# ictnlp/StreamSpeech

Measured on AMD Instinct MI355X. Metric: real-time factor (RTFx = audio seconds / wall seconds) + utterances/sec, offline S2ST fr-en, higher is better.
Workload: dtype f32

## Files before the change

include/streamspeech_hip.h:

```cpp
#ifndef STREAMSPEECH_HIP_H
#define STREAMSPEECH_HIP_H

#include <stddef.h>
#include <stdint.h>

#ifdef __cplusplus
extern "C" {
#endif

#define SS_ABI_VERSION 2

typedef struct ss_model ss_model;
typedef struct ss_vocoder ss_vocoder;
typedef struct ss_scratch ss_scratch;
typedef struct ss_stream_pool ss_stream_pool;

typedef struct ss_config {
  int32_t input_feat, conv_channels, conv_kernel;
  int32_t enc_dim, enc_ffn, enc_heads, enc_layers, dw_kernel;
  int32_t src_vocab, tgt_vocab;
  int32_t mt_layers, dec_dim, dec_ffn, dec_heads;
  int32_t t2u_layers, unit_layers, unit_vocab, ctc_upsample;
  int32_t pad, eos, unk;
  int32_t max_rel_pos;
// ... 214 lines not shown
  float* powers;
  int64_t hist_first;
  int64_t n_hist;
  int64_t first_frame;
  int32_t n_frames;
  int32_t H, W;
  float p_abs, p_min, snr, rise;
  int32_t min_speech, end_silence, post_roll, max_frames;
  int32_t reserved;
} ss_vad_seg;

typedef struct ss_vad_result {
  int64_t consumed;
  int64_t start_frame;
  int64_t cut_sample;
  int64_t last_speech;
  int32_t events;
  int32_t mode;
} ss_vad_result;

int ss_vad_scan(void* stream, const ss_vad_seg* h_segs, int n_segs, ss_vad_result* d_results);
int ss_vad_scan_host(const ss_vad_seg* h_segs, int n_segs, ss_vad_result* h_results);

int ss_row_max_logprob(void* stream, const float* d_logits, int rows, int vocab, int mask0, int mask1, int mask2,
                       float* d_out);

int ss_log_softmax(void* stream, const float* d_logits, int rows, int vocab, int mask0, int mask1, int as_probs,
                   float* d_out);

int ss_encoder_out_len(int T);
int ss_encoder_forward(ss_model* m, void* stream, const float* d_fbank, int T, int attn_chunk,
                       int conv_chunk, float* d_enc_out);

int ss_encoder_stream_reset(ss_model* m);
int ss_encoder_stream_set_tail(ss_model* m, int unsettled_fbank_frames);
int ss_encoder_stream_forward(ss_model* m, void* stream, const float* d_fbank, int T, int attn_chunk,
                              int conv_chunk, float* d_enc_out, int32_t* n_final, int32_t* n_computed);
int ss_encoder_stream_set_deferred(ss_model* m, int on);
int ss_encoder_stream_status(ss_model* m, void* stream, int32_t* repeat);

int ss_stream_pool_create(ss_model* m, int max_sessions, int max_rows, ss_stream_pool** out);
void ss_stream_pool_destroy(ss_stream_pool* p);
int ss_stream_pool_reset(ss_stream_pool* p, int slot);
int ss_stream_pool_set_tail(ss_stream_pool* p, int slot, int unsettled_fbank_frames);
int ss_encoder_stream_forward_batch(ss_model* m, void* stream, ss_stream_pool* p, int n, const int32_t* h_slots,
                                    const float* const* h_fbank, const int32_t* h_T, const int32_t* h_attn_chunk,
                                    const int32_t* h_conv_chunk, float* d_enc_packed, int32_t* h_n_final, int32_t* h_n_computed);
int ss_stream_pool_ctc(ss_model* m, void* stream, ss_stream_pool* p, int head, int n, const int32_t* h_slots,
                       const float* d_enc_packed, int32_t* d_raw, int32_t* d_tokens, int32_t* d_index, int32_t* d_counts);
int ss_stream_pool_set_scores(ss_stream_pool* p, int on);
int ss_stream_pool_ctc_scored(ss_model* m, void* stream, ss_stream_pool* p, int head, int n, const int32_t* h_slots,
                              const float* d_enc_packed, int32_t* d_raw, int32_t* d_tokens, int32_t* d_index, int32_t* d_counts,
                              float* d_lprob, int32_t* d_last, float* d_tok_lprob);
int ss_stream_pool_stats(ss_stream_pool* p, int64_t* launches, int64_t* head_rows);

int ss_ctc_greedy(ss_model* m, void* stream, int head, const float* d_enc_out, int Tp,
                  int32_t* d_raw, int32_t* d_tokens, int32_t* d_index, int32_t* d_count,
                  float* d_logits);

int ss_ctc_greedy_scored(ss_model* m, void* stream, int head, const float* d_enc_out, int Tp,
                         int32_t* d_raw, int32_t* d_tokens, int32_t* d_index, int32_t* d_count,
                         float* d_logits, float* d_lprob, int32_t* d_last, float* d_tok_lprob);

int ss_mt_set_persistent(ss_model* m, int workgroups);
int ss_mt_get_persistent(ss_model* m);

int ss_mt_begin(ss_model* m, void* stream, const float* d_enc_out, int Tp);
int ss_mt_append(ss_model* m, void* stream, const int32_t* d_tokens, int n, int pos0, int ban_eos,
                 int force_eos, float* d_feats, int32_t* d_next, int n_tail_pad);
int ss_mt_greedy(ss_model* m, void* stream, const float* d_enc_out, int Tp, const int32_t* h_prefix,
                 int n_prefix, int max_len, int min_len, int32_t* h_out_tokens, int* h_n_out,
                 float* d_feats, int* h_n_feats);
int ss_mt_truncate(ss_model* m, int len);

int ss_t2u_units(ss_model* m, void* stream, const float* d_mt_feats, int n, int t2u_causal,
                 int mask_eos, int32_t* d_raw, int32_t* d_tokens, int32_t* d_count, float* d_logits,
                 int n_tail_pad);

int ss_vocoder_create(const ss_vocoder_config* cfg, const float* d_blob, size_t blob_floats,
                      const char* const* names, const int64_t* offsets, const int64_t* numels,
                      int n_slots, ss_vocoder** out);
void ss_vocoder_destroy(ss_vocoder* v);
int ss_vocoder_set_bf16x3(ss_vocoder* v, int on);
int ss_vocoder_set_f16(ss_vocoder* v, int on);
int ss_vocoder_forward(ss_vocoder* v, void* stream, const int32_t* d_codes, int K, int dur_prediction,
                       const int32_t* d_forced_dur, float* d_wav, int64_t wav_capacity,
                       int32_t* d_dur, int64_t* h_n_samples);
int ss_vocoder_num_speakers(const ss_vocoder* v);
int ss_vocoder_forward_spkr(ss_vocoder* v, void* stream, const int32_t* d_codes, int K, int dur_prediction,
                            const int32_t* d_forced_dur, float* d_wav, int64_t wav_capacity,
                            int32_t* d_dur, int64_t* h_n_samples, int32_t spkr);

int ss_batch_fbank_cmvn(ss_model* m, void* stream, int B, const float* d_pcm, const int64_t* h_pcm_start,
                        const int32_t* h_n_samples, float pcm_scale, float* d_feat, int32_t* h_T);
int ss_batch_cmvn(ss_model* m, void* stream, const float* d_in, int64_t rows, float* d_out);
int ss_batch_encoder_forward(ss_model* m, void* stream, int B, const float* d_fbank, const int32_t* h_T,
                             int attn_chunk, int conv_chunk, float* d_enc_out, int32_t* h_Tp);
int ss_batch_ctc_greedy(ss_model* m, void* stream, int head, int B, const float* d_enc_out,
                        const int32_t* h_Tp, int32_t* d_raw, int32_t* d_tokens, int32_t* d_index,
                        int32_t* d_counts);
int ss_batch_ctc_greedy_scored(ss_model* m, void* stream, int head, int B, const float* d_enc_out,
                               const int32_t* h_Tp, int32_t* d_raw, int32_t* d_tokens, int32_t* d_index,
                               int32_t* d_counts, float* d_lprob, int32_t* d_last, float* d_tok_lprob);
typedef struct ss_ctc_align_result {
  double score;
  double viterbi;
  int32_t status;
  int32_t n_tokens;
} ss_ctc_align_result;
#define SS_CTC_ALIGN_MAX_FRAMES 1500
#define SS_CTC_ALIGN_MAX_LABELS 1500
int ss_batch_ctc_align(ss_model* m, void* stream, int head, int B, const float* d_enc_out, const int32_t* h_Tp,
                       const int32_t* h_targets, const int32_t* h_n_targets, ss_ctc_align_result* d_results, int32_t* d_path,
                       int32_t* d_first, int32_t* d_last, float* d_tok_lprob);
int ss_ctc_align_host(const float* h_logits, int ld, int V, int pad, int B, const int32_t* h_T, const int32_t* h_targets,
                      const int32_t* h_n_targets, ss_ctc_align_result* h_results, int32_t* h_path, int32_t* h_first, int32_t* h_last,
                      float* h_tok_lprob, float* h_frame_lprob);
int ss_batch_mt_greedy(ss_model* m, void* stream, int B, const float* d_enc_out, const int32_t* h_Tp,
                       const int32_t* h_max_len, int min_len, int32_t* h_out_tokens, int out_stride,
                       int32_t* h_n_out, float* d_feats, int feat_rows);
int ss_batch_mt_beam(ss_model* m, void* stream, int B, int beam, const float* d_enc_out, const int32_t* h_Tp,
                     const int32_t* h_max_len, int min_len, float unk_penalty, int normalize, int32_t* h_out_tokens,
                     int out_stride, int32_t* h_n_out, float* h_scores, float* h_pos_scores, float* d_feats, int feat_rows);
int ss_batch_mt_continue(ss_model* m, void* stream, int B, const float* d_enc_out, const int32_t* h_Tp, const int32_t* h_prefix,
                         const int32_t* h_n_prefix, const int32_t* h_max_len, int min_len, int32_t* h_out_tokens, int out_stride,
                         int32_t* h_n_out, float* d_feats, int feat_rows, int32_t* h_n_feats);
int ss_batch_mt_continue_plan(int B, const int32_t* h_Tp, const int32_t* h_prefix, const int32_t* h_n_prefix, const int32_t* h_max_len,
                              int min_len, int out_stride, int feat_rows, int max_tgt_pos, int vocab, int eos, int32_t* h_dims,
                              int32_t* h_tables, int64_t tables_cap, int64_t* h_n_tables);
int ss_batch_mt_beam_continue(ss_model* m, void* stream, int B, int beam, const float* d_enc_out, const int32_t* h_Tp,
                              const int32_t* h_prefix, const int32_t* h_n_prefix, const int32_t* h_max_len, int min_len,
                              float unk_penalty, int normalize, int32_t* h_out_tokens, int out_stride, int32_t* h_n_out,
                              float* h_scores, float* h_pos_scores, float* d_feats, int feat_rows);
int ss_batch_mt_beam_continue_plan(int B, int beam, const int32_t* h_Tp, const int32_t* h_prefix, const int32_t* h_n_prefix,
                                   const int32_t* h_max_len, int min_len, int out_stride, int feat_rows, int max_tgt_pos, int vocab,
                                   int eos, int pad, int32_t* h_dims, int32_t* h_tables, int64_t tables_cap, int64_t* h_n_tables);
typedef struct ss_mt_search_opts {
  int32_t size;
  int32_t no_repeat_ngram;
  float len_penalty;
  float temperature;
} ss_mt_search_opts;
int ss_batch_mt_beam_opts(ss_model* m, void* stream, int B, int beam, const float* d_enc_out, const int32_t* h_Tp,
                          const int32_t* h_max_len, int min_len, float unk_penalty, int normalize, int32_t* h_out_tokens,
                          int out_stride, int32_t* h_n_out, float* h_scores, float* h_pos_scores, float* d_feats, int feat_rows,
                          const ss_mt_search_opts* opts);
int ss_batch_mt_beam_continue_opts(ss_model* m, void* stream, int B, int beam, const float* d_enc_out, const int32_t* h_Tp,
                                   const int32_t* h_prefix, const int32_t* h_n_prefix, const int32_t* h_max_len, int min_len,
                                   float unk_penalty, int normalize, int32_t* h_out_tokens, int out_stride, int32_t* h_n_out,
                                   float* h_scores, float* h_pos_scores, float* d_feats, int feat_rows,
                                   const ss_mt_search_opts* opts);
int ss_batch_mt_beam_continue_plan_opts(int B, int beam, const int32_t* h_Tp, const int32_t* h_prefix, const int32_t* h_n_prefix,
                                        const int32_t* h_max_len, int min_len, int out_stride, int feat_rows, int max_tgt_pos,
                                        int vocab, int eos, int pad, int32_t* h_dims, int32_t* h_tables, int64_t tables_cap,
                                        int64_t* h_n_tables, const ss_mt_search_opts* opts);
int ss_batch_fbank_frames(ss_model* m, void* stream, int B, const float* const* h_pcm, const int32_t* h_first, const int32_t* h_n,
                          float pcm_scale, float* const* h_feat);
int ss_batch_fbank_frames_sr(ss_model* m, void* stream, int B, const float* const* h_pcm, const int32_t* h_n_in, const int32_t* h_up,
                             const int32_t* h_down, const float* const* h_taps, const int32_t* h_half_len, const int32_t* h_first,
                             const int32_t* h_n, float pcm_scale, float* const* h_feat);
int ss_fbank_sr_rows(int64_t n_in, int up, int down, int half_len, int32_t* h_n_rows, int32_t* h_n_final);
int ss_batch_t2u_units(ss_model* m, void* stream, int B, const float* d_feats, int feat_rows,
                       const int32_t* h_n, int t2u_causal, int mask_eos, int32_t* d_raw, int32_t* d_tokens,
                       int32_t* d_counts);
int ss_batch_vocoder_forward(ss_vocoder* v, void* stream, int B, const int32_t* d_codes, const int32_t* h_K,
                             int dur_prediction, const int32_t* d_forced_dur, float* d_wav,
// ... 10 lines not shown
                         const int32_t* h_n_tokens, const int32_t* h_n_tail_pad, float* d_feats, int feat_rows);
int ss_batch_mt_attention(ss_model* m, void* stream, int B, const float* d_enc_out, const int32_t* h_Tp, const int32_t* h_tokens,
                          const int32_t* h_n_tokens, const int32_t* h_first, float* d_feats, int feat_rows, float* d_attn,
                          int64_t* h_attn_off, int64_t attn_capacity, int32_t* d_peak, float* d_stat);
int ss_batch_mt_score(ss_model* m, void* stream, int U, const float* d_enc_out, const int32_t* h_Tp, int B, const int32_t* h_src,
                      const int32_t* h_tokens, const int32_t* h_n_tokens, float* d_feats, int feat_rows, float* d_stat,
                      int32_t* d_idx);
int ss_batch_vocoder_tail(ss_vocoder* v, void* stream, int B, const int32_t* d_codes, const int32_t* h_K, const int32_t* h_n_new,
                          const int32_t* h_ctx, const int32_t* h_rf, int dur_prediction, float* d_out, int64_t out_capacity,
                          int32_t* h_win_first, int32_t* h_dur, int64_t* h_out_start, int64_t* h_n_out);
int ss_batch_vocoder_tail_spkr(ss_vocoder* v, void* stream, int B, const int32_t* d_codes, const int32_t* h_K, const int32_t* h_n_new,
                               const int32_t* h_ctx, const int32_t* h_rf, int dur_prediction, float* d_out, int64_t out_capacity,
                               int32_t* h_win_first, int32_t* h_dur, int64_t* h_out_start, int64_t* h_n_out,
                               const int32_t* h_spkr );

int ss_batch_unit_spans(ss_model* m, void* stream, int B, const int32_t* d_raw, const int32_t* h_n, const int32_t* h_K,
                        const int32_t* h_dur_first, const int32_t* h_unit0, const int32_t* d_dur, const int32_t* h_dur,
                        int32_t* h_spans, int32_t* h_K_out);
int ss_unit_spans_host(int B, const int32_t* h_raw, const int32_t* h_n, const int32_t* h_K, const int32_t* h_dur_first,
                       const int32_t* h_unit0, const int32_t* h_dur, int up, int blank, int pad, int bos, int eos, int32_t* h_spans,
                       int32_t* h_K_out);

int ss_prof_enable(int cls_mask);
int ss_prof_enable_hi(int cls_mask);
int ss_prof_reset(void);
int ss_prof_read(int cls, double* h_ms_total, double* h_flops_total, int64_t* h_launches,
                 double* h_bytes_total);
int ss_prof_totals(int cls, double* h_flops_total, double* h_bytes_total, int64_t* h_launches);
int ss_prof_read_issued(int cls, double* h_issued_flops_total);
int ss_prof_shape_log(int on);
int ss_prof_shape_dump(char* buf, int cap);
int ss_prof_num_classes(void);
const char* ss_prof_class_name(int cls);

int ss_model_set_pack_invariant(ss_model* m, int on);
int ss_model_get_pack_invariant(ss_model* m);
int ss_debug_canon(int mode);

int ss_debug_last_logits(ss_model* m, void* stream, float* d_out, int64_t cap_floats, int* h_rows, int* h_cols);

int ss_op_ffn_fused(void* stream, const float* dX, int ldx, float* dY, int ldy, const float* ln_g, const float* ln_b,
                    const float* dW1, const float* db1, const float* dW2, const float* db2, float alpha,
                    const float* ln2_g, const float* ln2_b, int M, int D, int F);
int ss_debug_ffn(int grid, int row_tiles_per_wave, int enable);
int ss_debug_rtlin(int grid, int enable);
int ss_debug_rtlin_kb(int uw, int order);
int ss_debug_rtlin_kb_last(int32_t out[4]);
int ss_debug_conv_c64(int enable);
int ss_debug_conv_c256_rows(int rows);
int ss_debug_conv_c32(int enable);
int ss_debug_conv_c16(int enable);
int64_t ss_debug_enc_step_launches(void);
int ss_op_ln_linear(void* stream, const float* dX, int ldx, const float* ln_g, const float* ln_b, const float* dW,
                    const float* dbias, const float* dR, int ldr, float* dC, int ldc, int M, int N, int K, int act, float alpha,
                    int glu);
int ss_op_ln_linear_ex(void* stream, const float* dX, int ldx, const float* ln_g, const float* ln_b, float* ln_out, const float* dW,
                       const float* dbias, const float* dR, int ldr, float* dC, int ldc, int M, int N, int K, int act, float alpha,
                       int glu, int canon);

int ss_debug_force_tile(int bm, int bn, int ks);
int ss_debug_sk_errors(void);
int ss_debug_attention_split(int v);
int ss_debug_attention_q16(int v);
int ss_debug_enc_step_inject_timeout(ss_model* m);
int ss_debug_scratch_audit(ss_scratch* sc, size_t* booked, size_t* held);
int ss_debug_mt_inject_timeout(ss_model* m);

int ss_op_conv_gemm(void* stream, const float* dA, int lda, const float* dW, const float* dbias,
                    const float* dR, int ldr, const float* dR2, int ldr2, float* dC, int ldc,
                    int M, int N, int Cin, int taps, int dil, int stride, int pad, int in_len,
                    int chunk, int in_act, float in_slope, int act, float alpha, float div, int glu);
typedef struct ss_op_conv_args {
  const float* A; const float* W; const float* bias; const float* R; const float* R2; float* C; float* C2;
  int32_t lda, ldc, ldr, ldr2, ldc2;
  int32_t M, N, Cin, taps, dil, stride, pad, in_len, chunk;
  int32_t in_act; float in_slope;
  int32_t act; float act_slope, alpha, div, c2_slope;
  int32_t glu;
  const int32_t* segs; int32_t nseg, max_seg_out;
  int32_t same_rows;
} ss_op_conv_args;
int ss_op_conv_gemm_ex(void* stream, const ss_op_conv_args* a);
int ss_op_conv_gemm_rows(void* stream, const ss_op_conv_args* a, int m_begin, const int32_t* seg_mb, const float* const* seg_A, int canon);
int ss_op_conv_pair(void* stream, const float* dA, int lda, const float* dW1, const float* db1, const float* dW2, const float* db2,
                    float* dC, int ldc, const float* dR2, int ldr2, float div, float* dC2, int ldc2, float c2_slope, int C, int taps,
                    int dil, int M, int in_len, float slope, const int32_t* d_segs, int nseg);
int ss_op_resblock_fused(void* stream, const float* dX, int ldx, const float* const* dW1, const float* const* dB1,
                         const float* const* dW2, const float* const* dB2, const int32_t* dil, float* dY, int ldy, const float* dR2,
                         int ldr2, float div, int C, int taps, int M, float slope, const int32_t* d_segs, int nseg);
int ss_debug_slab(int grid, long long min_rows);
int ss_op_conv_f16(void* stream, const float* dA, const float* dW, const float* dbias, const float* dR, const float* dR2,
                   float* dC, float* dC2, int M, int C, int taps, int dil, int in_act, float in_slope, int act, float div,
                   const int32_t* d_segs, int nseg);
int ss_op_layernorm(void* stream, const float* dx, int ldx, float* dy, int ldy, const float* dg,
                    const float* db, int M, int D, float eps);
int ss_op_attention(void* stream, const float* dQ, int ldq, const float* dK, int ldk, const float* dV,
                    int ldv, float* dO, int ldo, int Tq, int Tk, int H, float scale, int causal,
                    int chunk, const float* dP, int ldp, const float* du, const float* dv);
typedef struct ss_op_attn_args {
  const float* Q; const float* K; const float* V; float* O;
  int32_t ldq, ldk, ldv, ldo;
  int32_t Tq, Tk, H;
  float scale;
  int32_t causal, chunk, q0, k_mask_tail;
  const float* P; int32_t ldp;
  const float* bias_u; const float* bias_v;
  const int32_t* segs; int32_t nseg, max_q, p_tmax;
  const int32_t* seg_tail;
  int32_t no_decode_kernel;
  const int32_t* anc; int32_t anc_ld, anc_slots;
  int32_t use_split;
} ss_op_attn_args;
int ss_op_attention_ex(void* stream, const ss_op_attn_args* a);
typedef struct ss_op_attn_probs_args {
  const float* Q; const float* K;
  int32_t ldq, ldk, H;
  float scale;
  const int32_t* segs; int32_t nseg;
  const int32_t* q_first; const int32_t* row_off; const int64_t* p_off;
  float* P; int32_t* peak; float* stat;
  int32_t max_rows;
} ss_op_attn_probs_args;
int ss_op_attention_probs(void* stream, const ss_op_attn_probs_args* a);
typedef struct ss_op_pool_attn_args {
  const float* Qs; float* cache; float* O;
  int32_t ld, ldo, slot_rows;
  const float* P; int32_t ldp, p_tmax;
  const float* bias_u; const float* bias_v;
  const int32_t* sess; const int32_t* qt_pre;
  int32_t nsess, qtiles, H;
  float scale;
} ss_op_pool_attn_args;
int ss_op_attention_pool(void* stream, const ss_op_pool_attn_args* a);
int ss_debug_attention_no_mfma(int v);
int ss_op_dwconv_bn_silu(void* stream, const float* dx, int ldx, float* dy, int ldy, const float* dwt,
                         int K, const float* mean, const float* var, const float* gamma,
                         const float* beta, float eps, int T, int C, int chunk);
int ss_op_dwconv_bn_silu_ex(void* stream, const float* dx, int ldx, float* dy, int ldy, const float* dwt, int K, const float* mean,
                            const float* var, const float* gamma, const float* beta, float eps, int T, int C, int chunk,
                            const int32_t* segs, int nseg, int t_begin);
int ss_op_pool_dwconv(void* stream, const float* gs, float* cache, int slot_rows, float* y, const float* wt, int K, const float* bn_mean,
                      const float* bn_var, const float* bn_gamma, const float* bn_beta, float bn_eps, int C, const int32_t* sess,
                      int nsess, int max_n);
int ss_op_pool_gather_rows(void* stream, float* out, const float* stk, float* cache, int slot_rows, int W, const int32_t* tab,
                           const int32_t* pre, int nsess, int total);
int ss_op_pool_gather_ids(void* stream, int32_t* out, const int32_t* stk, int32_t* cache, int slot_rows, const int32_t* tab,
                          const int32_t* pre, int nsess, int total);
int ss_op_pool_stack_rows(void* stream, float* out, const float* enc, int W, const int32_t* src, const int32_t* pre, int nsess,
                          int total);

int ss_op_masked_argmax(void* stream, const float* logits, int ld, int M, int N, int mask0, int mask1, int mask2, int force,
                        int32_t* ids, const int32_t* row_max_len, int step, int force_id, const int32_t* row_min_len, int ban_id);
int ss_op_ctc_collapse(void* stream, const int32_t* raw, int T, int blank, int pad, int32_t* tokens, int32_t* index, int32_t* count,
                       const int32_t* segs, int nseg);
int ss_op_masked_argmax_lprob(void* stream, const float* logits, int ld, int M, int N, int mask0, int mask1, int mask2, int32_t* ids,
                              float* lprob);
int ss_op_ctc_collapse_spans(void* stream, const int32_t* raw, const float* lprob, int T, int blank, int pad, int32_t* tokens,
                             int32_t* index, int32_t* last, float* tok_lprob, int32_t* count, const int32_t* segs, int nseg);
int ss_op_mt_token_scores(void* stream, const float* d_logits, int ld, int rows, int V, const int32_t* d_target, float* d_stat,
                          int32_t* d_idx);
int ss_debug_mt_score_form(int force_strided);
int ss_op_ctc_align(void* stream, const float* d_logits, int ld, int V, int pad, int B, const int32_t* h_T, const int32_t* h_targets,
                    const int32_t* h_n_targets, ss_ctc_align_result* d_results, int32_t* d_path, int32_t* d_first, int32_t* d_last,
                    float* d_tok_lprob, float* d_frame_lprob);
int ss_op_unit_spans(void* stream, int B, const int32_t* d_raw, const int32_t* h_n, const int32_t* h_K, const int32_t* h_dur_first,
                     const int32_t* h_unit0, const int32_t* d_dur, int up, int blank, int pad, int bos, int eos, int32_t* d_spans,
// ... 49 lines not shown
```

streamspeech_amd/csrc/conv_c64.hip:

```cpp
#include "slab_common.hpp"

#ifndef C64_FENCE
#define C64_FENCE 1
#endif
#if C64_FENCE
#define C64_STEP_FENCE __builtin_amdgcn_sched_barrier(0)
#else
#define C64_STEP_FENCE do { } while (0)
#endif

namespace ss {

using u32x4 = __attribute__((ext_vector_type(4))) unsigned;

namespace {
constexpr int C6_C = 64;
constexpr int C6_BM_MAX = 256;
constexpr int C6_LDA = C6_C + 4;
constexpr int C6_MAXHALO = 64;
constexpr int C6_MAXSEG = 256;
[[maybe_unused]] constexpr int C6_RING = 8;
[[maybe_unused]] constexpr int C6_NUM_RECORDS = 0x7ffffff0;
[[maybe_unused]] constexpr int C6_NP = ((C6_BM_MAX + C6_MAXHALO) * (C6_C / 4) + 255) / 256;
}

template <bool LRELU, int WM>
__global__ __launch_bounds__(256, 2) void conv_c64_kernel(const GemmArgs p, const int slab_rows) {
#if __HIP_DEVICE_COMPILE__
  constexpr int C = C6_C, BM = 64 * WM, LDA = C6_LDA, NP = C6_NP;
  extern __shared__ __attribute__((aligned(16))) float smem[];
  float* sA = smem;
  int* s_blk = reinterpret_cast<int*>(smem + ((slab_rows * LDA + 3) & ~3));

  const int t = threadIdx.x, lane = t & 63;
  const int wave = __builtin_amdgcn_readfirstlane(t >> 6);
  const int r = lane & 15, g = lane >> 4;
  const int K = p.taps * C;

  SlabWalk<GemmArgs> w(p, s_blk, BM);
  __syncthreads();
  const int nblocks = w.nblocks();
  const float slope = p.in_slope;

  const __amdgpu_buffer_rsrc_t rsW = __builtin_amdgcn_make_buffer_rsrc((void*)p.W, 0, C6_NUM_RECORDS, 0x00020000);
  const int vo = (r * K + 4 * g) * 4;
  auto wload = [&](int tap, int f) -> f32x4 {
    const int so = __builtin_amdgcn_readfirstlane((((f & 3) * 16) * K + tap * C + (f >> 2) * 16) * 4);
    const u32x4 v = __builtin_amdgcn_raw_buffer_load_b128(rsW, vo, so, 0);
    return f32x4{__uint_as_float(v[0]), __uint_as_float(v[1]), __uint_as_float(v[2]), __uint_as_float(v[3])};
  };

  int blk = blockIdx.x;
  if (blk >= nblocks) return;
  f32x4 ring[C6_RING];
#pragma unroll
  for (int f = 0; f < C6_RING; ++f) ring[f] = wload(0, f);

  for (; blk < nblocks; blk += gridDim.x) {
    w.locate(blk, p.in_len);
    const int m0 = w.m0, seg_lo = w.seg_lo, seg_hi = w.seg_hi;
    const int m_hi = p.nseg > 0 ? seg_hi : min(seg_hi, p.M);
    const bool edge = (m0 - p.pad < seg_lo) || (m0 - p.pad + slab_rows > seg_hi);
    __syncthreads();
    {
      f32x4 pre[NP];
#pragma unroll
      for (int u = 0; u < NP; ++u) {
        const int rho = (t >> 4) + 16 * u;
        const int gc = min(max(m0 - p.pad + rho, seg_lo), seg_hi - 1);
        pre[u] = *reinterpret_cast<const f32x4*>(p.A + (size_t)gc * p.lda + (t & 15) * 4);
      }
      float* dst = sA + (t >> 4) * LDA + (t & 15) * 4;
#pragma unroll
      for (int u = 0; u < NP; ++u) {
        const int rho = (t >> 4) + 16 * u;
        f32x4 v = pre[u];
        if (edge) {
          const int gin = m0 - p.pad + rho;
          const bool ok = gin >= seg_lo && gin < seg_hi;
#pragma unroll
          for (int e = 0; e < 4; ++e) v[e] = ok ? v[e] : 0.f;
        }
        if (LRELU) {
#pragma unroll
          for (int e = 0; e < 4; ++e) v[e] = fmaxf(v[e], v[e] * slope);
        }
        if (rho < slab_rows) *reinterpret_cast<f32x4*>(dst + u * 16 * LDA) = v;
      }
    }
    __syncthreads();

    f32x4 acc[WM][4];
#pragma unroll
    for (int i = 0; i < WM; ++i)
#pragma unroll
      for (int j = 0; j < 4; ++j) acc[i][j] = f32x4{0.f, 0.f, 0.f, 0.f};

    const float* pa = sA + (wave * 16 * WM + r) * LDA + 4 * g;
    const int a_step = p.dil * LDA;
    f32x4 xa[WM];
#pragma unroll
    for (int i = 0; i < WM; ++i) xa[i] = *reinterpret_cast<const f32x4*>(pa + i * 16 * LDA);
#pragma unroll 1
    for (int tap = 0; tap < p.taps; ++tap) {
      const int tap_next = tap + 1 < p.taps ? tap + 1 : 0;
      const float* pa_next = tap + 1 < p.taps ? pa + a_step : pa;
#pragma unroll
      for (int cc = 0; cc < 4; ++cc) {
        f32x4 xb[WM];
#pragma unroll
        for (int i = 0; i < WM; ++i)
          xb[i] = *reinterpret_cast<const f32x4*>((cc < 3 ? pa : pa_next) + i * 16 * LDA + (cc < 3 ? (cc + 1) * 16 : 0));
        f32x4 wf[4];
#pragma unroll
        for (int j = 0; j < 4; ++j) {
          const int f = cc * 4 + j;
          wf[j] = ring[f % C6_RING];
          ring[f % C6_RING] = wload(f + C6_RING < 16 ? tap : tap_next, (f + C6_RING) & 15);
        }
#pragma unroll
        for (int e = 0; e < 4; ++e)
#pragma unroll
          for (int i = 0; i < WM; ++i)
#pragma unroll
            for (int j = 0; j < 4; ++j)
              acc[i][j] = __builtin_amdgcn_mfma_f32_16x16x4f32(wf[j][e], xa[i][e], acc[i][j], 0, 0, 0);
#pragma unroll
        for (int i = 0; i < WM; ++i) xa[i] = xb[i];
        C64_STEP_FENCE;
      }
      pa = pa_next;
    }

    int le = lane;
    asm volatile("" : "+v"(le));
    const int r_e = le & 15, g_e = le >> 4;
    f32x4 bb[4];
#pragma unroll
    for (int j = 0; j < 4; ++j) bb[j] = f32x4{0.f, 0.f, 0.f, 0.f};
    if (p.bias) {
#pragma unroll
      for (int j = 0; j < 4; ++j) bb[j] = *reinterpret_cast<const f32x4*>(p.bias + j * 16 + g_e * 4);
    }
    f32x4 y[WM * 4];
#pragma unroll
    for (int i = 0; i < WM; ++i)
#pragma unroll
      for (int j = 0; j < 4; ++j) y[i * 4 + j] = acc[i][j];
    const int mw = m0 + wave * 16 * WM + r_e;
    slab_epi_batch(p, y, bb, [&](int q, int n) -> size_t {
      return (size_t)min(mw + (n / 4) * 16, m_hi - 1) * (q == 0 ? p.ldr : p.ldr2) + (n % 4) * 16 + g_e * 4;
    });
#pragma unroll
    for (int i = 0; i < WM; ++i) {
      if (mw + i * 16 < m_hi) {
#pragma unroll
        for (int j = 0; j < 4; ++j) slab_epi_store(p, mw + i * 16, j * 16 + g_e * 4, y[i * 4 + j]);
      }
    }
  }
#endif
}

void conv_c64_debug(int enable) { if (enable >= 0) dispatch_edit([enable](Dispatch& d) { d.c64_off = enable ? 0 : 1; }); }
bool conv_c64_enabled() { return !disp().c64_off; }

bool conv_c64_eligible(const GemmArgs& a) {
  return !disp().c64_off && slab_conv_ok(a, C6_C) && a.taps >= 1 && a.dil >= 1 && (a.taps - 1) * a.dil <= C6_MAXHALO && a.pad >= 0 &&
         a.pad <= (a.taps - 1) * a.dil && a.nseg <= C6_MAXSEG && a.M >= disp().c64_min_rows && slab_rows_ok(a.M) &&
         (size_t)a.taps * C6_C * C6_C * 4 < 0x7ff00000ull;
}

static size_t c64_lds(int bm, const GemmArgs& a) { return slab_lds_bytes(bm + (a.taps - 1) * a.dil, C6_LDA, C6_MAXSEG); }
template <bool LRELU, int WM>
static int launch_c64_t(const GemmArgs& a, hipStream_t stream) {
  constexpr int BM = 64 * WM;
  const int slab_rows = BM + (a.taps - 1) * a.dil;
  const size_t lds = c64_lds(BM, a);
  SS_MAX_LDS_ONCE((&conv_c64_kernel<LRELU, WM>), 96 * 1024);
  SkWorkspace* st = nullptr;
  int rc = sk_workspace_acquire(stream, &st);
  if (rc != SS_OK) return rc;
  const int occ = lds * 2 <= 158 * 1024 ? 2 : 1;
  const int grid = slab_grid(occ, st->cus, a.M, BM, a.nseg);
  ProfRec rec{}; bool prof = false;
  rc = prof_begin(a, stream, PROF_CONV_C64, rec, prof);
  if (rc != SS_OK) return rc;
  hipLaunchKernelGGL((conv_c64_kernel<LRELU, WM>), dim3(grid), dim3(256), lds, stream, a, slab_rows);
  SS_LAUNCH_CHECK();
  return prof_end(stream, rec, prof);
}

int launch_conv_c64(const GemmArgs& a, hipStream_t stream) {
  if (!conv_c64_eligible(a)) return SS_ERR_ARG;
  const bool wm4 = 2 * c64_lds(256, a) <= 158 * 1024;
  if (a.in_act == ACT_LRELU) return wm4 ? launch_c64_t<true, 4>(a, stream) : launch_c64_t<true, 3>(a, stream);
  return wm4 ? launch_c64_t<false, 4>(a, stream) : launch_c64_t<false, 3>(a, stream);
}

}
```

streamspeech_amd/csrc/conv_sk2.hip:

```cpp
#include "gemm.hpp"

#include <cstdlib>

namespace ss {

using f32x4 = __attribute__((ext_vector_type(4))) float;
using u32x4 = __attribute__((ext_vector_type(4))) unsigned;
using f32x2 = __attribute__((ext_vector_type(2))) float;
using s16x4 = __attribute__((ext_vector_type(4))) short;
typedef __bf16 bf16x2_t __attribute__((ext_vector_type(2)));
typedef __attribute__((address_space(3))) void* lds_ptr_t;

constexpr int K2_BM = 256, K2_BK = 32;
[[maybe_unused]] constexpr int K2_SC1 = 16;
constexpr int K2_MAXG = 512;
[[maybe_unused]] constexpr int K2_WORD0 = 16;
[[maybe_unused]] constexpr unsigned K2_SPIN_LIMIT = 1u << 22;
[[maybe_unused]] constexpr int K2_NUM_RECORDS = 0x7ffffff0;
[[maybe_unused]] constexpr unsigned K2_OOB = 0x80000000u;
constexpr int k2_stage_floats(int BN) { return (K2_BM + BN) * K2_BK; }
constexpr size_t k2_lds_bytes(int BN) { return 3 * (size_t)k2_stage_floats(BN) * sizeof(float) + (2 * K2_BM + 4) * sizeof(int); }

struct Sk2Args {
  float* ws;
  unsigned* sync;
  unsigned base;
  unsigned epoch;
  int G;
  unsigned long long* dbg;
};

#define K2_WAIT_VMCNT(n) asm volatile("s_waitcnt vmcnt(" #n ")" ::: "memory")
#ifdef K2_DIAGNOSTIC_BUILD
#include "../../tools/src/conv_sk2_diag.hpp"
#else
#define K2D_SKIP_DMA(in_loop) false
#define K2D_SKIP_A_PIECE(in_loop, j) false
#define K2D_SKIP_WAIT_BARRIER 0
#define K2D_SKIP_DS_READ(in_loop) false
#define K2D_SKIP_TAIL false
#define K2D_SKIP_MFMA false
#define K2D_SKIP_HANDOFF false
#define K2D_SKIP_STORES false
#define K2D_SKIP_R_LOADS false
#define K2D_ONE_A_PIECE 0
#define K2D_TIMING 0
#define K2D_TIMING_DECL
#define K2_STAMP(slot) do { } while (0)
#define K2D_COUNT_STEPS(n) do { } while (0)
#define K2D_TIMING_FLUSH do { } while (0)
#endif
#ifndef K2_RPREF
#define K2_RPREF 1
#endif

__device__ __attribute__((noinline)) float k2_act_slow(float v, int act) {
  if (act == ACT_SILU) return v / (1.0f + expf(-v));
  if (act == ACT_TANH) return tanhf(v);
  return v;
}

__device__ __forceinline__ f32x4 k2_split_bf16(f32x4 x) {
  const bf16x2_t h01 = __builtin_convertvector((f32x2){x[0], x[1]}, bf16x2_t);
  const bf16x2_t h23 = __builtin_convertvector((f32x2){x[2], x[3]}, bf16x2_t);
  const unsigned u01 = __builtin_bit_cast(unsigned, h01), u23 = __builtin_bit_cast(unsigned, h23);
  const bf16x2_t l01 = __builtin_convertvector((f32x2){x[0] - __uint_as_float(u01 << 16), x[1] - __uint_as_float(u01 & 0xffff0000u)}, bf16x2_t);
  const bf16x2_t l23 = __builtin_convertvector((f32x2){x[2] - __uint_as_float(u23 << 16), x[3] - __uint_as_float(u23 & 0xffff0000u)}, bf16x2_t);
  return f32x4{__uint_as_float(u01), __uint_as_float(u23), __uint_as_float(__builtin_bit_cast(unsigned, l01)),
               __uint_as_float(__builtin_bit_cast(unsigned, l23))};
}
__device__ __forceinline__ s16x4 k2_half(f32x4 v, int lo) {
  const unsigned long long w = (unsigned long long)__float_as_uint(v[2 * lo]) | ((unsigned long long)__float_as_uint(v[2 * lo + 1]) << 32);
  return __builtin_bit_cast(s16x4, w);
}

template <int BN, bool LRELU, bool X3>
__global__ __launch_bounds__(256, 1) void conv_sk2_kernel(const GemmArgs p, const Sk2Args q) {
#if __HIP_DEVICE_COMPILE__
  constexpr int BM = K2_BM, BK = K2_BK, STAGE = k2_stage_floats(BN);
  constexpr int TN = 4, TM = BN == 128 ? 8 : 4;
  constexpr int NWP = BN / 32;
  constexpr int PIECES = 8 + NWP;
  constexpr int NFR = TM + TN;
  constexpr int HG = TM / 2;
  static_assert(BN == 128 || BN == 64, "tile widths");
  extern __shared__ __attribute__((aligned(16))) float smem[];
  int* s_lo = reinterpret_cast<int*>(smem + 3 * STAGE);
  int* s_hi = s_lo + BM;
  int* s_misc = s_hi + BM;

  const int t = threadIdx.x, lane = t & 63;
  const int wave = __builtin_amdgcn_readfirstlane(t >> 6);
  const int wrow = BN == 128 ? (wave >> 1) * 128 : wave * 64;
  const int wcol = BN == 128 ? (wave & 1) * 64 : 0;
  const int r = lane & 15, g = lane >> 4;
  if (t == 0) s_misc[0] = (int)(atomicAdd(q.sync, 1u) - q.base);
  __syncthreads();
  const int w = __builtin_amdgcn_readfirstlane(s_misc[0]);
  if ((unsigned)w >= (unsigned)q.G) { if (t == 0) atomicAdd(q.sync + 8, 1u); return; }
  K2D_TIMING_DECL

  const int kpt = p.Cin / BK;
  const int nk = p.taps * kpt;
  const int Ktot = p.taps * p.Cin;
  const int tiles_n = p.N / BN;
  const int tiles_m = (p.M + BM - 1) / BM;
  const long long U = (long long)tiles_m * tiles_n * nk;
  const long long u0 = (long long)w * U / q.G, u1 = (long long)(w + 1) * U / q.G;
  if (u1 <= u0) return;
  const int t_first = (int)(u0 / nk), t_last = (int)((u1 - 1) / nk);

  const float slope = p.in_slope;
  const __amdgpu_buffer_rsrc_t rsA = __builtin_amdgcn_make_buffer_rsrc(
      (void*)(reinterpret_cast<uintptr_t>(p.A) - (uintptr_t)p.pad * p.lda * sizeof(float)), 0, K2_NUM_RECORDS, 0x00020000);
  const __amdgpu_buffer_rsrc_t rsW = __builtin_amdgcn_make_buffer_rsrc((void*)p.W, 0, K2_NUM_RECORDS, 0x00020000);

  const int swz = (r >> 1) & 7;
  const int rdA0 = (wrow + r) * BK + ((g ^ swz) << 2);
  const int rdA1 = (wrow + r) * BK + (((4 + g) ^ swz) << 2);
  const int rdW0 = BM * BK + (wcol + r) * BK + ((g ^ swz) << 2);
  const int rdW1 = BM * BK + (wcol + r) * BK + (((4 + g) ^ swz) << 2);
  const int st_row = lane >> 3, st_pos = lane & 7;

  struct Part { int ka, kb, n, m0, n0, tm; };
  const int nparts = t_last - t_first + 1;
  auto part_of = [&](int ip) {
    const int tile = t_last - ip;
    const long long ut0 = (long long)tile * nk;
    Part P;
    P.ka = (int)(max(u0, ut0) - ut0);
    P.kb = (int)(min(u1, ut0 + nk) - ut0);
    P.n = P.kb - P.ka;
    P.tm = tile / tiles_n;
    P.m0 = P.tm * BM;
    P.n0 = (tile - P.tm * tiles_n) * BN;
    return P;
  };
  int a_base[8], a_len[8];
  unsigned a_off[8], w_off[NWP];
  int nci = 0, ntap = 0;
  int soffA = 0, soffW = 0, shift = 0;
  int cur_tm = -1;
  auto lds_barrier = [&]() {
    asm volatile("s_waitcnt lgkmcnt(0)" ::: "memory");
    __builtin_amdgcn_s_barrier();
  };
  auto stage_setup = [&](const Part& P) {
    lds_barrier();
    if (P.tm != cur_tm) {
      cur_tm = P.tm;
      const int m = P.m0 + t;
      int lo = 0, hi = 0;
      if (m < p.M) {
        if (p.nseg > 0) {
          int a = 0, bsz = p.nseg;
          while (bsz > 1) {
            const int half = bsz >> 1;
            if (p.segs[4 * (a + half)] <= m) a += half;
            bsz -= half;
          }
          const int sst = p.segs[4 * a], ln = p.segs[4 * a + 1];
          if (m >= sst && m < sst + ln) { lo = sst; hi = sst + ln; }
        } else {
          hi = p.in_len;
        }
      }
      s_lo[t] = lo; s_hi[t] = hi;
      lds_barrier();
    }
#pragma unroll
    for (int j = 0; j < 8; ++j) {
      const int row = wave * 64 + j * 8 + st_row;
      a_base[j] = P.m0 + row - p.pad - s_lo[row];
      a_len[j] = s_hi[row] - s_lo[row];
      a_off[j] = (unsigned)(((P.m0 + row) * p.lda + ((st_pos ^ ((row >> 1) & 7)) << 2)) * 4);
    }
#pragma unroll
    for (int j = 0; j < NWP; ++j) {
      const int nrow = wave * (BN / 4) + j * 8 + st_row;
      w_off[j] = (unsigned)(((P.n0 + nrow) * Ktot + ((st_pos ^ ((nrow >> 1) & 7)) << 2)) * 4);
    }
    nci = (P.ka / p.taps) * BK;
    ntap = P.ka - (P.ka / p.taps) * p.taps;
  };
  int shift_l = 0;
  auto step_begin = [&](bool live) {
    const int tapv = __builtin_amdgcn_readfirstlane(ntap);
    const int nciv = __builtin_amdgcn_readfirstlane(nci);
    shift = tapv * p.dil;
    shift_l = live ? shift : 0x40000000;
    soffA = (shift * p.lda + nciv) * 4;
    soffW = (tapv * p.Cin + nciv) * 4;
  };
  auto step_advance = [&](bool adv = true) {
    const int nt = ntap + (adv ? 1 : 0);
    const bool wrap = nt >= p.taps;
    ntap = wrap ? 0 : nt;
    nci += wrap ? BK : 0;
  };
  [[maybe_unused]] bool in_loop = false;
  auto issueA = [&](int stage, int j, bool live) {
    if (K2D_SKIP_DMA(in_loop) || K2D_SKIP_A_PIECE(in_loop, j)) return;
    float* sA = smem + stage * STAGE + (wave * 64) * BK;
    const bool ok = (unsigned)(a_base[j] + shift_l) < (unsigned)a_len[j];
    __builtin_amdgcn_raw_ptr_buffer_load_lds(rsA, (lds_ptr_t)(sA + j * 8 * BK), 16, ok ? a_off[j] : K2_OOB,
                                             __builtin_amdgcn_readfirstlane(soffA), 0, 0);
  };
  auto issueW = [&](int stage, int j, bool live) {
    if (K2D_SKIP_DMA(in_loop)) return;
    float* sW = smem + stage * STAGE + BM * BK + (wave * (BN / 4)) * BK;
    __builtin_amdgcn_raw_ptr_buffer_load_lds(rsW, (lds_ptr_t)(sW + j * 8 * BK), 16, live ? w_off[j] : K2_OOB,
                                             __builtin_amdgcn_readfirstlane(soffW), 0, 0);
  };
  auto issue_step = [&](int stage, bool live) {
    step_begin(live);
#pragma unroll
    for (int j = 0; j < 8; ++j) issueA(stage, j, live);
#pragma unroll
    for (int j = 0; j < NWP; ++j) issueW(stage, j, live);
    step_advance(live);
  };
  auto wait_newest_step_only = [&]() {
    if constexpr (K2D_ONE_A_PIECE != 0) { if constexpr (BN == 128) K2_WAIT_VMCNT(5); else K2_WAIT_VMCNT(3); }
    else if constexpr (BN == 128) K2_WAIT_VMCNT(12); else K2_WAIT_VMCNT(10);
  };
  int stage_ip = 0, stage_left = 0;
  auto stager_next_part = [&]() {
    const Part P = part_of(stage_ip);
    stage_setup(P);
    stage_left = P.n;
  };
  auto stager_advance = [&]() {
    if (stage_left == 0 && stage_ip + 1 < nparts) { ++stage_ip; stager_next_part(); }
  };

  int st = 0;
  stager_next_part();
  issue_step(0, true);
  --stage_left;
  stager_advance();
  issue_step(1, stage_left > 0);
  stage_left -= stage_left > 0 ? 1 : 0;
  wait_newest_step_only();
  __builtin_amdgcn_s_barrier();
  K2_STAMP(0);
  for (int ip = 0; ip < nparts; ++ip) {
    const Part cur = part_of(ip);
    const int n = cur.n, m0 = cur.m0, n0 = cur.n0;
    K2D_COUNT_STEPS(n);
    f32x4 acc[TM][TN];
#pragma unroll
    for (int i = 0; i < TM; ++i)
#pragma unroll
      for (int j = 0; j < TN; ++j) acc[i][j] = f32x4{0.f, 0.f, 0.f, 0.f};

    auto load_frag = [&](const float* S, int half, int u, f32x4 (&af)[TM], f32x4 (&bf)[TN]) {
      if (K2D_SKIP_DS_READ(in_loop)) return;
      if (u < TN) {
        bf[u] = *reinterpret_cast<const f32x4*>(S + (half ? rdW1 : rdW0) + u * 16 * BK);
        if (X3) bf[u] = k2_split_bf16(bf[u]);
      } else {
        const int i = u - TN;
        af[i] = *reinterpret_cast<const f32x4*>(S + (half ? rdA1 : rdA0) + i * 16 * BK);
        if (LRELU) {
#pragma unroll
          for (int e = 0; e < 4; ++e) af[i][e] = fmaxf(af[i][e], af[i][e] * slope);
        }
        if (X3) af[i] = k2_split_bf16(af[i]);
      }
    };
    auto mma8 = [&](const f32x4 (&af)[TM], const f32x4 (&bf)[TN], int e, int qd) {
      if (K2D_SKIP_MFMA) return;
      if (X3 && e == 3) return;
#pragma unroll
      for (int i = 2 * qd; i < 2 * qd + 2; ++i)
#pragma unroll
        for (int j = 0; j < TN; ++j) {
          if constexpr (X3)
            acc[i][j] = __builtin_amdgcn_mfma_f32_16x16x16bf16_1k(k2_half(bf[j], e == 2), k2_half(af[i], e == 1), acc[i][j], 0, 0, 0);
          else
            acc[i][j] = __builtin_amdgcn_mfma_f32_16x16x4f32(bf[j][e], af[i][e], acc[i][j], 0, 0, 0);
        }
    };

    f32x4 ax[TM], bx[TN], ay[TM], by[TN];
#pragma unroll
    for (int u = 0; u < NFR; ++u) load_frag(smem + st * STAGE, 0, u, ax, bx);
#if K2_RPREF
    constexpr int PT = BN == 128 ? 2 : TM;
    f32x4 rall[PT][TN];
    const bool want_r = p.R != nullptr && cur.kb == nk;
#endif
    in_loop = true;
    K2_STAMP(1);
    for (int i = 0; i < n; ++i) {
#if K2_RPREF
      if (i == n - 1 && want_r) {
        int lp = lane;
        asm volatile("" : "+v"(lp));
#pragma unroll
        for (int ii = 0; ii < PT; ++ii) {
          const int m = min(m0 + wrow + ii * 16 + (lp & 15), p.M - 1);
#pragma unroll
          for (int j = 0; j < TN; ++j)
            rall[ii][j] = *reinterpret_cast<const f32x4*>(p.R + (size_t)m * p.ldr + n0 + wcol + j * 16 + (lp >> 4) * 4);
        }
      }
#endif
      stager_advance();
      const float* S = smem + st * STAGE;
      const int st1 = st == 2 ? 0 : st + 1, st2 = st1 == 2 ? 0 : st1 + 1;
      const bool live = stage_left > 0;
      stage_left -= live ? 1 : 0;
      const float* S1 = smem + st1 * STAGE;
      step_begin(live);
#pragma unroll
      for (int u = 0; u < (NFR > PIECES ? NFR : PIECES); ++u) {
        if (u < NFR) load_frag(S, 1, u, ay, by);
        if (u < 8) issueA(st2, u, live); else if (u < PIECES) issueW(st2, u - 8, live);
      }
      step_advance(live);
#pragma unroll
      for (int sl = 0; sl < 4 * HG; ++sl) mma8(ax, bx, sl / HG, sl % HG);
#pragma unroll
      for (int sl = 0; sl < 2 * HG; ++sl) mma8(ay, by, sl / HG, sl % HG);
#if !K2D_SKIP_WAIT_BARRIER
      wait_newest_step_only();
      __builtin_amdgcn_s_barrier();
#endif
#pragma unroll
      for (int u = 0; u < NFR; ++u) load_frag(S1, 0, u, ax, bx);
#pragma unroll
      for (int sl = 0; sl < 2 * HG; ++sl) mma8(ay, by, 2 + sl / HG, sl % HG);
      st = st1;
    }
    in_loop = false;
    K2_STAMP(2);
    const bool has_begin = cur.ka == 0, has_end = cur.kb == nk;
    if (K2D_SKIP_TAIL && acc[0][0][0] != 12345.f) continue;

    int le = lane;
    asm volatile("" : "+v"(le));
    const int r_e = le & 15, g_e = le >> 4;
    if (!K2D_SKIP_HANDOFF && !has_end) {
      const __amdgpu_buffer_rsrc_t rsP = __builtin_amdgcn_make_buffer_rsrc((void*)(q.ws + (size_t)w * (BM * BN)), 0, BM * BN * 4, 0x00020000);
#pragma unroll
      for (int i = 0; i < TM; ++i)
#pragma unroll
        for (int j = 0; j < TN; ++j) {
          u32x4 v;
#pragma unroll
          for (int e = 0; e < 4; ++e) v[e] = __float_as_uint(acc[i][j][e]);
          __builtin_amdgcn_raw_buffer_store_b128(v, rsP, (((wave * TM + i) * TN + j) * 64 + le) * 16, 0, K2_SC1);
        }
      K2_WAIT_VMCNT(0);
      __syncthreads();
      if (t == 0) __hip_atomic_store(q.sync + K2_WORD0 + w, q.epoch, __ATOMIC_RELAXED, __HIP_MEMORY_SCOPE_AGENT);
      K2_STAMP(3);
      continue;
    }
    if (!K2D_SKIP_HANDOFF && !has_begin) {
      const long long ut0 = (long long)(t_last - ip) * nk;
      const int wf = (int)(((ut0 + 1) * q.G - 1) / U);
      if (t == 0) {
        for (int ww = wf; ww < w; ++ww) {
          unsigned spins = 0;
          while (__hip_atomic_load(q.sync + K2_WORD0 + ww, __ATOMIC_RELAXED, __HIP_MEMORY_SCOPE_AGENT) != q.epoch) {
            __builtin_amdgcn_s_sleep(8);
            if (++spins > K2_SPIN_LIMIT) { atomicAdd(q.sync + 8, 1u); break; }
          }
        }
      }
      __syncthreads();
      for (int ww = wf; ww < w; ++ww) {
        const __amdgpu_buffer_rsrc_t rsP = __builtin_amdgcn_make_buffer_rsrc((void*)(q.ws + (size_t)ww * (BM * BN)), 0, BM * BN * 4, 0x00020000);
#pragma unroll
        for (int qq = 0; qq < HG; ++qq) {
          __builtin_amdgcn_sched_barrier(0);
          u32x4 o[2][TN];
#pragma unroll
          for (int i = 0; i < 2; ++i)
#pragma unroll
            for (int j = 0; j < TN; ++j)
              o[i][j] = __builtin_amdgcn_raw_buffer_load_b128(rsP, (((wave * TM + qq * 2 + i) * TN + j) * 64 + le) * 16, 0, K2_SC1);
          __builtin_amdgcn_sched_barrier(0);
#pragma unroll
          for (int i = 0; i < 2; ++i)
#pragma unroll
            for (int j = 0; j < TN; ++j)
#pragma unroll
              for (int e = 0; e < 4; ++e) acc[qq * 2 + i][j][e] += __uint_as_float(o[i][j][e]);
        }
        __builtin_amdgcn_sched_barrier(0);
      }
    }

    K2_STAMP(3);
    if (m0 + wrow >= p.M) continue;
    f32x4 bb[TN];
#pragma unroll
    for (int j = 0; j < TN; ++j) {
      bb[j] = f32x4{0.f, 0.f, 0.f, 0.f};
      if (p.bias) bb[j] = *reinterpret_cast<const f32x4*>(p.bias + n0 + wcol + j * 16 + g_e * 4);
    }
#pragma unroll
    for (int qq = 0; qq < HG; ++qq) {
      __builtin_amdgcn_sched_barrier(0);
      f32x4 rr[2][TN], rr2[2][TN];
#pragma unroll
      for (int i = 0; i < 2; ++i) {
        const int m = min(m0 + wrow + (qq * 2 + i) * 16 + r_e, p.M - 1);
#pragma unroll
        for (int j = 0; j < TN; ++j) {
          const int nn = n0 + wcol + j * 16 + g_e * 4;
#if K2_RPREF
          if (p.R && !K2D_SKIP_R_LOADS) {
            if (qq * 2 + i < PT) rr[i][j] = rall[qq * 2 + i < PT ? qq * 2 + i : 0][j];
            else rr[i][j] = *reinterpret_cast<const f32x4*>(p.R + (size_t)m * p.ldr + nn);
          }
#else
          if (p.R && !K2D_SKIP_R_LOADS) rr[i][j] = *reinterpret_cast<const f32x4*>(p.R + (size_t)m * p.ldr + nn);
#endif
          if (p.R2 && !K2D_SKIP_R_LOADS) rr2[i][j] = *reinterpret_cast<const f32x4*>(p.R2 + (size_t)m * p.ldr2 + nn);
        }
      }
      __builtin_amdgcn_sched_barrier(0);
      f32x4 v[2][TN];
#pragma unroll
      for (int i = 0; i < 2; ++i)
#pragma unroll
        for (int j = 0; j < TN; ++j) {
          v[i][j] = acc[qq * 2 + i][j];
#pragma unroll
          for (int e = 0; e < 4; ++e) v[i][j][e] += bb[j][e];
        }
      if (p.act == ACT_LRELU) {
#pragma unroll
        for (int i = 0; i < 2; ++i)
#pragma unroll
          for (int j = 0; j < TN; ++j)
#pragma unroll
            for (int e = 0; e < 4; ++e) v[i][j][e] = v[i][j][e] > 0.f ? v[i][j][e] : v[i][j][e] * p.act_slope;
      } else if (p.act == ACT_RELU) {
#pragma unroll
        for (int i = 0; i < 2; ++i)
// ... 3 lines not shown
            for (int e = 0; e < 4; ++e) v[i][j][e] = fmaxf(v[i][j][e], 0.f);
      } else if (p.act != ACT_NONE) {
#pragma unroll
        for (int i = 0; i < 2; ++i)
#pragma unroll
          for (int j = 0; j < TN; ++j)
#pragma unroll
            for (int e = 0; e < 4; ++e) v[i][j][e] = k2_act_slow(v[i][j][e], p.act);
      }
#pragma unroll
      for (int i = 0; i < 2; ++i)
#pragma unroll
        for (int j = 0; j < TN; ++j)
#pragma unroll
          for (int e = 0; e < 4; ++e) v[i][j][e] *= p.alpha;
      if (p.R && !K2D_SKIP_R_LOADS) {
#pragma unroll
        for (int i = 0; i < 2; ++i)
#pragma unroll
          for (int j = 0; j < TN; ++j)
#pragma unroll
            for (int e = 0; e < 4; ++e) v[i][j][e] += rr[i][j][e];
      }
      if (p.R2 && !K2D_SKIP_R_LOADS) {
#pragma unroll
        for (int i = 0; i < 2; ++i)
#pragma unroll
          for (int j = 0; j < TN; ++j)
#pragma unroll
            for (int e = 0; e < 4; ++e) v[i][j][e] = rr2[i][j][e] + v[i][j][e];
      }
      if (p.div > 0.f) {
#pragma unroll
        for (int i = 0; i < 2; ++i)
#pragma unroll
          for (int j = 0; j < TN; ++j)
#pragma unroll
            for (int e = 0; e < 4; ++e) v[i][j][e] = v[i][j][e] / p.div;
      }
#pragma unroll
      for (int i = 0; i < 2; ++i) {
        const int m = m0 + wrow + (qq * 2 + i) * 16 + r_e;
        if (m >= p.M) continue;
#pragma unroll
        for (int j = 0; j < TN; ++j) {
          const int nn = n0 + wcol + j * 16 + g_e * 4;
          if (!K2D_SKIP_STORES || v[i][j][0] == 12345.f) *reinterpret_cast<f32x4*>(p.C + (size_t)m * p.ldc + nn) = v[i][j];
          if (p.C2 && !K2D_SKIP_STORES) {
            f32x4 w2;
#pragma unroll
            for (int e = 0; e < 4; ++e) w2[e] = v[i][j][e] > 0.f ? v[i][j][e] : v[i][j][e] * p.c2_slope;
            *reinterpret_cast<f32x4*>(p.C2 + (size_t)m * p.ldc2 + nn) = w2;
          }
        }
      }
    }
    __builtin_amdgcn_sched_barrier(0);
    K2_STAMP(4);
  }
  K2D_TIMING_FLUSH;
#endif
}

#if K2D_TIMING
static unsigned long long* g_k2_last_dbg = nullptr;
static int g_k2_last_G = 0;
extern "C" int ss_debug_sk2_timing(unsigned long long* h_out, int cap_wgs) {
  if (!g_k2_last_dbg || cap_wgs < g_k2_last_G) return -1;
  if (hipMemcpy(h_out, g_k2_last_dbg, (size_t)g_k2_last_G * 8 * sizeof(unsigned long long), hipMemcpyDeviceToHost) != hipSuccess) return -1;
  return g_k2_last_G;
}
#endif

bool conv_sk2_eligible(const GemmArgs& a) {
  return a.canon != CANON_SEQ && a.same_rows && a.stride == 1 && a.chunk == 0 && !a.glu && !a.ln_g && a.Cin % K2_BK == 0 && (a.lda & 3) == 0 &&
         a.N % 64 == 0 && a.M > 0 && (a.ldc & 3) == 0 && (!a.R || (a.ldr & 3) == 0) && (!a.R2 || (a.ldr2 & 3) == 0) &&
         (!a.C2 || (a.ldc2 & 3) == 0) && ((size_t)(a.M + a.pad + 256) * a.lda + a.Cin) * 4 < 0x7ff00000ull &&
         (size_t)a.N * a.taps * a.Cin * 4 < 0x7ff00000ull &&
         (a.in_act == ACT_NONE || (a.in_act == ACT_LRELU && a.in_slope > 0.f && a.in_slope < 1.f));
}

int conv_sk2_error_count() { return 0; }

template <int BN, bool LRELU, bool X3>
static int launch_sk2(const GemmArgs& a, hipStream_t stream, int g_force) {
  constexpr size_t kLds = k2_lds_bytes(BN);
  SS_MAX_LDS_ONCE((&conv_sk2_kernel<BN, LRELU, X3>), kLds);
  SkWorkspace* st = nullptr;
  int rc = sk_workspace_acquire(stream, &st);
  if (rc != SS_OK) return rc;
  int cus = st->cus > K2_MAXG ? K2_MAXG : st->cus;
  if (const int spare = disp().sk2_spare_cus; spare > 0 && spare < cus) cus -= spare;
  const long long nk = (long long)a.taps * (a.Cin / K2_BK);
  const long long U = (long long)cdiv(a.M, K2_BM) * (a.N / BN) * nk;
  long long G = g_force > 0 ? g_force : cus;
  if (G > cus) G = cus;
  if (G > U / 4) G = U / 4;
  if (G < 1) G = 1;
  Sk2Args q;
  q.ws = st->ws; q.sync = st->sync2; q.G = (int)G; q.dbg = nullptr;
#if K2D_TIMING
  if (!st->dbg) SS_HIP_CHECK(hipMalloc(&st->dbg, (size_t)K2_MAXG * 8 * sizeof(unsigned long long)));
  SS_HIP_CHECK(hipMemsetAsync(st->dbg, 0, (size_t)K2_MAXG * 8 * sizeof(unsigned long long), stream));
  q.dbg = st->dbg;
  g_k2_last_dbg = st->dbg; g_k2_last_G = (int)G;
#endif
  unsigned epoch = st->epoch2 + 1;
  if (epoch == 0) epoch = 1;
  q.base = st->base2;
  q.epoch = epoch;
  ProfRec rec{}; bool prof = false;
  rc = prof_begin(a, stream, X3 ? PROF_CONV_SK2_BF16X3 : PROF_CONV_SK2, rec, prof);
  if (rc != SS_OK) return rc;
  hipLaunchKernelGGL((conv_sk2_kernel<BN, LRELU, X3>), dim3((unsigned)G), dim3(256), kLds, stream, a, q);
  SS_LAUNCH_CHECK();
  st->base2 += (unsigned)G;
  st->epoch2 = epoch;
  return prof_end(stream, rec, prof);
}

int launch_conv_sk2(const GemmArgs& a, hipStream_t stream, int g_force) {
  if (!conv_sk2_eligible(a)) return SS_ERR_ARG;
  const bool lr = a.in_act == ACT_LRELU;
  if (a.x3) {
    if (a.N % 128 == 0) return lr ? launch_sk2<128, true, true>(a, stream, g_force) : launch_sk2<128, false, true>(a, stream, g_force);
    return lr ? launch_sk2<64, true, true>(a, stream, g_force) : launch_sk2<64, false, true>(a, stream, g_force);
  }
  if (a.N % 128 == 0) return lr ? launch_sk2<128, true, false>(a, stream, g_force) : launch_sk2<128, false, false>(a, stream, g_force);
  return lr ? launch_sk2<64, true, false>(a, stream, g_force) : launch_sk2<64, false, false>(a, stream, g_force);
}

}
```

streamspeech_amd/csrc/debug_ops.hip:

```cpp
#include "model_internal.hpp"
#include "ctc_align.hpp"

static int op_bind_wino(GemmArgs& a, void* stream) {
  static thread_local std::map<hipStream_t, DevBuf> wino_tmps;
  DevBuf& wino_tmp = wino_tmps[(hipStream_t)stream];
  const int N = a.N, Cin = a.Cin, taps = a.taps;
  if ((conv_c64w_enabled() && N == 64 && Cin == 64 && taps >= 3 && conv_c64_eligible(a)) ||
      (conv_c128w_enabled() && N == 128 && Cin == 128 && taps >= 3 && a.same_rows && !a.glu) ||
      (conv_c256w_enabled() && N == 256 && Cin == 256 && taps >= 3 && a.same_rows && !a.glu) ||
      (conv_c32w_enabled() && N == 32 && Cin == 32 && taps >= 3 && conv_c32_eligible(a))) {
    RET(wino_tmp.ensure((size_t)N * ((taps + 2) / 3) * 4 * N * sizeof(float)));
    RET(launch_wino_pack(a.W, wino_tmp.f(), N, taps, (hipStream_t)stream));
    a.Wwino = wino_tmp.f();
  }
  return SS_OK;
}

extern "C" int ss_op_conv_gemm(void* stream, const float* dA, int lda, const float* dW, const float* dbias,
                               const float* dR, int ldr, const float* dR2, int ldr2, float* dC, int ldc, int M,
                               int N, int Cin, int taps, int dil, int stride, int pad, int in_len, int chunk,
                               int in_act, float in_slope, int act, float alpha, float div, int glu) {
  GemmArgs a;
  a.A = dA; a.lda = lda; a.W = dW; a.bias = dbias; a.R = dR; a.ldr = ldr; a.R2 = dR2; a.ldr2 = ldr2; a.C = dC; a.ldc = ldc;
  a.M = M; a.N = N; a.Cin = Cin; a.taps = taps; a.dil = dil; a.stride = stride; a.pad = pad; a.in_len = in_len;
  a.chunk = chunk; a.in_act = in_act; a.in_slope = in_slope; a.act = act; a.alpha = alpha; a.div = div; a.glu = glu;
  a.same_rows = (stride == 1 && M == in_len) ? 1 : 0;
  RET(op_bind_wino(a, stream));
  return launch_conv_gemm(a, (hipStream_t)stream);
}

static void op_fill_conv(GemmArgs& a, const ss_op_conv_args* x) {
  a.A = x->A; a.W = x->W; a.bias = x->bias; a.R = x->R; a.R2 = x->R2; a.C = x->C; a.C2 = x->C2;
  a.lda = x->lda; a.ldc = x->ldc; a.ldr = x->ldr; a.ldr2 = x->ldr2; a.ldc2 = x->ldc2;
  a.M = x->M; a.N = x->N; a.Cin = x->Cin; a.taps = x->taps; a.dil = x->dil; a.stride = x->stride; a.pad = x->pad;
  a.in_len = x->in_len; a.chunk = x->chunk;
  a.in_act = x->in_act; a.in_slope = x->in_slope; a.act = x->act; a.act_slope = x->act_slope; a.alpha = x->alpha; a.div = x->div;
  a.c2_slope = x->c2_slope; a.glu = x->glu;
  a.segs = x->segs; a.nseg = x->nseg; a.max_seg_out = x->max_seg_out; a.same_rows = x->same_rows;
}
extern "C" int ss_op_conv_gemm_ex(void* stream, const ss_op_conv_args* x) {
  if (!x) return SS_ERR_ARG;
  GemmArgs a;
  op_fill_conv(a, x);
  if (a.W && a.N > 0 && a.taps > 0) RET(op_bind_wino(a, stream));
  return launch_conv_gemm(a, (hipStream_t)stream);
}
extern "C" int ss_op_conv_gemm_rows(void* stream, const ss_op_conv_args* x, int m_begin, const int32_t* seg_mb,
                                    const float* const* seg_A, int canon) {
  if (!x || canon < 0 || canon > 2) return SS_ERR_ARG;
  GemmArgs a;
  op_fill_conv(a, x);
  a.m_begin = m_begin; a.seg_mb = seg_mb; a.seg_A = seg_A; a.canon = canon;
  if (a.W && a.N > 0 && a.taps > 0) RET(op_bind_wino(a, stream));
  return launch_conv_gemm(a, (hipStream_t)stream);
}
extern "C" int ss_op_conv_pair(void* stream, const float* dA, int lda, const float* dW1, const float* db1, const float* dW2,
                               const float* db2, float* dC, int ldc, const float* dR2, int ldr2, float div, float* dC2, int ldc2,
                               float c2_slope, int Cch, int taps, int dil, int M, int in_len, float slope, const int32_t* d_segs,
                               int nseg) {
  return launch_conv_pair(dA, lda, dW1, db1, dW2, db2, dC, ldc, dR2, ldr2, div, dC2, ldc2, c2_slope, Cch, taps, dil, M, in_len, slope,
                          d_segs, nseg, (hipStream_t)stream);
}
extern "C" int ss_op_resblock_fused(void* stream, const float* dX, int ldx, const float* const* dW1, const float* const* dB1,
                                    const float* const* dW2, const float* const* dB2, const int32_t* dil, float* dY, int ldy,
                                    const float* dR2, int ldr2, float div, int Cch, int taps, int M, float slope,
                                    const int32_t* d_segs, int nseg) {
  if (!dW1 || !dB1 || !dW2 || !dB2 || !dil) return SS_ERR_ARG;
  return launch_resblock_fused(dX, ldx, dW1, dB1, dW2, dB2, dil, dY, ldy, dR2, ldr2, div, Cch, taps, M, slope, d_segs, nseg,
                               (hipStream_t)stream);
}
extern "C" int ss_debug_slab(int grid, long long min_rows) {
  if (grid < 0) return SS_ERR_ARG;
  slab_debug(grid, min_rows);
  return SS_OK;
}

extern "C" int ss_op_conv_f16(void* stream, const float* dA, const float* dW, const float* dbias, const float* dR, const float* dR2,
                              float* dC, float* dC2, int M, int Cch, int taps, int dil, int in_act, float in_slope, int act, float div,
                              const int32_t* d_segs, int nseg) {
  if (!dA || !dW || !dC || M <= 0 || taps < 1 || dil < 1 || nseg < 0 || (nseg > 0 && !d_segs)) return SS_ERR_ARG;
  if (!(Cch == 64 || Cch == 128 || Cch == 256)) return SS_ERR_ARG;
  static thread_local std::map<hipStream_t, DevBuf> f16_tmps;
  DevBuf& wh = f16_tmps[(hipStream_t)stream];
  RET(wh.ensure(f16_pack_halves(Cch, taps) * sizeof(uint16_t)));
  RET(launch_f16_pack(dW, wh.p, Cch, taps, (hipStream_t)stream));
  GemmArgs a;
  a.A = dA; a.lda = Cch; a.W = dW; a.Wf16 = wh.p; a.bias = dbias; a.R = dR; a.ldr = Cch; a.R2 = dR2; a.ldr2 = Cch;
  a.C = dC; a.ldc = Cch; a.C2 = dC2; a.ldc2 = Cch; a.c2_slope = 0.1f;
  a.M = M; a.N = Cch; a.Cin = Cch; a.taps = taps; a.dil = dil; a.stride = 1; a.pad = dil * (taps - 1) / 2; a.in_len = M;
  a.same_rows = 1; a.in_act = in_act; a.in_slope = in_slope; a.act = act; a.act_slope = 0.1f; a.div = div;
  a.segs = d_segs; a.nseg = nseg;
  return launch_conv_f16(a, (hipStream_t)stream);
}

extern "C" int ss_debug_last_logits(ss_model* m, void* stream, float* d_out, int64_t cap_floats, int* h_rows, int* h_cols) {
  if (!m || !h_rows || !h_cols) return SS_ERR_ARG;
  *h_rows = m->sc->dbg_rows; *h_cols = m->sc->dbg_cols;
  if (!d_out) return SS_OK;
  if (!m->sc->dbg_logits || cap_floats < (int64_t)m->sc->dbg_rows * m->sc->dbg_cols) return SS_ERR_CAPACITY;
  SS_HIP_CHECK(hipMemcpyAsync(d_out, m->sc->dbg_logits, (size_t)m->sc->dbg_rows * m->sc->dbg_cols * sizeof(float), hipMemcpyDeviceToDevice,
                              (hipStream_t)stream));
  return SS_OK;
}

extern "C" int ss_op_ffn_fused(void* stream, const float* dX, int ldx, float* dY, int ldy, const float* ln_g, const float* ln_b,
                               const float* dW1, const float* db1, const float* dW2, const float* db2, float alpha,
                               const float* ln2_g, const float* ln2_b, int M, int D, int F) {
  return launch_ffn_fused(dX, ldx, dY, ldy, ln_g, ln_b, dW1, db1, dW2, db2, alpha, ln2_g, ln2_b, M, D, F, (hipStream_t)stream,
                          canon_mode() == CANON_SEQ);
}
extern "C" int ss_debug_canon(int mode) {
  if (mode < 0 || mode > 2) return SS_ERR_ARG;
  canon_debug_set(mode);
  return SS_OK;
}
extern "C" int ss_op_ln_linear(void* stream, const float* dX, int ldx, const float* ln_g, const float* ln_b, const float* dW,
                               const float* dbias, const float* dR, int ldr, float* dC, int ldc, int M, int N, int K, int act,
                               float alpha, int glu) {
  GemmArgs a;
  a.A = dX; a.lda = ldx; a.W = dW; a.bias = dbias; a.R = dR; a.ldr = ldr; a.C = dC; a.ldc = ldc;
  a.M = M; a.N = N; a.Cin = K; a.in_len = M; a.act = act; a.alpha = alpha; a.glu = glu; a.same_rows = 1;
  a.ln_g = ln_g; a.ln_b = ln_b;
  return launch_conv_gemm(a, (hipStream_t)stream);
}
extern "C" int ss_op_ln_linear_ex(void* stream, const float* dX, int ldx, const float* ln_g, const float* ln_b, float* ln_out,
                                  const float* dW, const float* dbias, const float* dR, int ldr, float* dC, int ldc, int M, int N, int K,
                                  int act, float alpha, int glu, int canon) {
  if (canon < 0 || canon > 2 || (ln_g == nullptr) != (ln_b == nullptr) || (ln_out && !ln_g)) return SS_ERR_ARG;
  GemmArgs a;
  a.A = dX; a.lda = ldx; a.W = dW; a.bias = dbias; a.R = dR; a.ldr = ldr; a.C = dC; a.ldc = ldc;
  a.M = M; a.N = N; a.Cin = K; a.in_len = M; a.act = act; a.alpha = alpha; a.glu = glu; a.same_rows = 1;
  a.ln_g = ln_g; a.ln_b = ln_b; a.ln_out = ln_out; a.canon = canon;
  return launch_conv_gemm(a, (hipStream_t)stream);
}
extern "C" int ss_debug_conv_c64(int enable) {
  if (enable == 4 || enable == 5) { conv_c64w_debug(enable == 5); return SS_OK; }
  if (enable == 6 || enable == 7) { conv_c128w_debug(enable == 7); return SS_OK; }
  if (enable == 8 || enable == 9) { conv_c256w_debug(enable == 9); return SS_OK; }
// ... 238 lines not shown
```

streamspeech_amd/csrc/dispatch.hip:

```cpp
#include "gemm.hpp"

#include <atomic>
#include <cstdlib>
#include <map>
#include <mutex>
#include <utility>
#include <vector>

namespace ss {

namespace {
std::mutex g_disp_mu;
std::atomic<unsigned> g_disp_gen{1};
Dispatch env_defaults() {
  Dispatch d;
  auto I = [](const char* k, int dflt) { const char* e = getenv(k); return e ? atoi(e) : dflt; };
  auto L = [](const char* k, long long dflt) { const char* e = getenv(k); return e ? atoll(e) : dflt; };
  d.attn_split = I("SS_ATTN_NO_SPLIT", 0) ? -1 : 0; d.attn_q16 = I("SS_ATTN_Q16", d.attn_q16);
  d.c16_off = I("SS_NO_CONV_C16", 0) ? 1 : 0; d.c32_off = I("SS_NO_CONV_C32", 0) ? 1 : 0; d.c64_off = I("SS_NO_CONV_C64", 0) ? 1 : 0;
  d.c16_min_rows = L("SS_CONV_C16_MIN_ROWS", d.c16_min_rows); d.c32_min_rows = L("SS_CONV_C32_MIN_ROWS", d.c32_min_rows);
  d.c64_min_rows = L("SS_CONV_C64_MIN_ROWS", d.c64_min_rows);
  d.c64w_on = I("SS_CONV_C64_WINOGRAD", 1); d.c128w_on = I("SS_CONV_C128_WINOGRAD", 1); d.c256w_on = I("SS_CONV_C256_WINOGRAD", 1);
  d.c32w_on = I("SS_CONV_C32_WINOGRAD", 1); d.c64w_min_k = I("SS_CONV_C64_WINOGRAD_MIN_K", 3);
  d.c128w_min_rows = L("SS_CONV_C128_MIN_ROWS", d.c128w_min_rows); d.c256w_min_rows = L("SS_CONV_C256_MIN_ROWS", d.c256w_min_rows);
  if (const int r = I("SS_CONV_C256_ROWS", d.c256w_rows); r == 128 || r == 256) d.c256w_rows = r;
  if (getenv("SS_FFN_WM")) { d.ffn_wm = I("SS_FFN_WM", 3); d.ffn_wm_forced = 1; d.ffn_wm_env = d.ffn_wm; }
  d.ffn_fusion = I("SS_NO_FFN_FUSION", 0) ? 0 : 1; d.ffn_min_rows = I("SS_FFN_MIN_ROWS", d.ffn_min_rows);
  if (getenv("SS_SK_MIN_GFLOP")) d.sk_min_flops = 1e9 * atof(getenv("SS_SK_MIN_GFLOP"));
  d.no_resblock_fusion = I("SS_NO_RESBLOCK_FUSION", 0); d.no_pair_fusion = I("SS_NO_PAIR_FUSION", 0);
  d.rt_off = I("SS_NO_RTLIN", 0) ? 1 : 0; d.rt_min_rows = I("SS_RTLIN_MIN_ROWS", d.rt_min_rows); d.rt_min_units = L("SS_RTLIN_MIN_UNITS", d.rt_min_units);
  d.rt_kb_min_units = L("SS_RTLIN_KB_MIN_UNITS", d.rt_kb_min_units); d.rt_kb_uw = I("SS_RTLIN_KB_UW", d.rt_kb_uw); d.rt_kb_xmap = I("SS_RTLIN_KB_XMAP", d.rt_kb_xmap);
  d.smallm_max_rows = I("SS_SMALLM_MAX_ROWS", d.smallm_max_rows); d.sk_min_units = L("SS_SK_MIN_UNITS", d.sk_min_units);
  d.no_sk2 = I("SS_NO_SK2", 0) ? 1 : 0; d.sk2_min_k64 = I("SS_SK2_MINK64", d.sk2_min_k64); d.sk2_spare_cus = I("SS_SK2_SPARE_CUS", 0);
  d.rt_wg_per_cu = I("SS_RTLIN_WG_PER_CU", 0); d.c32_min_k = I("SS_CONV_C32_MIN_K", d.c32_min_k); d.c16_min_k = I("SS_CONV_C16_MIN_K", d.c16_min_k);
  return d;
}
Dispatch& process_settings() { static Dispatch d = env_defaults(); return d; }
thread_local const Dispatch* t_disp = nullptr;
thread_local CtxDispatch t_disp_own;
}
void dispatch_edit(const std::function<void(Dispatch&)>& fn) {
  std::lock_guard<std::mutex> lk(g_disp_mu);
  fn(process_settings());
  g_disp_gen.fetch_add(1, std::memory_order_release);
}
void slab_debug(int grid, long long min_rows) {
  const Dispatch dflt = env_defaults();
  dispatch_edit([=](Dispatch& d) {
    d.slab_grid_cap = grid > 0 ? grid : 0;
    const bool set = min_rows >= 0;
    d.c16_min_rows = set ? min_rows : dflt.c16_min_rows; d.c32_min_rows = set ? min_rows : dflt.c32_min_rows;
    d.c64_min_rows = set ? min_rows : dflt.c64_min_rows;
    d.c128w_min_rows = set ? min_rows : dflt.c128w_min_rows; d.c256w_min_rows = set ? min_rows : dflt.c256w_min_rows;
  });
}
int conv_c256w_rows_debug(int rows) {
  if (rows != 0 && rows != 128 && rows != 256) return SS_ERR_ARG;
  const int dflt = env_defaults().c256w_rows;
  dispatch_edit([=](Dispatch& d) { d.c256w_rows = rows ? rows : dflt; });
  return SS_OK;
}
const Dispatch* CtxDispatch::refresh() {
  const unsigned now = g_disp_gen.load(std::memory_order_acquire);
  if (gen != now) {
    std::lock_guard<std::mutex> lk(g_disp_mu);
    d = process_settings();
    gen = g_disp_gen.load(std::memory_order_relaxed);
  }
  return &d;
}
const Dispatch& disp() { return t_disp ? *t_disp : *t_disp_own.refresh(); }
DispatchScope::DispatchScope(const Dispatch* d) : prev(t_disp) { t_disp = d; }
DispatchScope::~DispatchScope() { t_disp = prev; }

void debug_force_tile(int bm, int bn, int ks) {
  dispatch_edit([=](Dispatch& d) { d.force_bm = bm; d.force_bn = bn; d.force_ks = ks; d.sk_groups = (bm == 1 && bn == 8); });
}
bool debug_tile_forced() { return disp().force_bm != 0; }

static thread_local int t_canon = CANON_NONE;
CanonScope::CanonScope(int mode) : prev(t_canon) { t_canon = mode; }
CanonScope::~CanonScope() { t_canon = prev; }
int canon_mode() { return t_canon; }
void canon_debug_set(int mode) { t_canon = mode; }

constexpr size_t SKW_SYNC_BYTES = (16 + 1024) * sizeof(unsigned) + 256;
static std::mutex g_skw_mu;
static std::vector<SkWorkspace*> g_skw_live;
static std::map<std::pair<int, hipStream_t>, SkWorkspace*> g_skw_fallback;
static thread_local SkWorkspace* t_skw = nullptr;

SkWorkspace* sk_workspace_new() {
  SkWorkspace* w = new SkWorkspace();
  std::lock_guard<std::mutex> lk(g_skw_mu);
  g_skw_live.push_back(w);
  return w;
}
void sk_workspace_free(SkWorkspace* w) {
  if (!w) return;
  {
    std::lock_guard<std::mutex> lk(g_skw_mu);
    for (size_t i = 0; i < g_skw_live.size(); ++i)
      if (g_skw_live[i] == w) { g_skw_live.erase(g_skw_live.begin() + i); break; }
  }
  if (w->ws) (void)hipFree(w->ws);
  if (w->sync1) (void)hipFree(w->sync1);
  if (w->sync2) (void)hipFree(w->sync2);
  if (w->sync3) (void)hipFree(w->sync3);
  if (w->dbg) (void)hipFree(w->dbg);
  delete w;
}
SkScope::SkScope(SkWorkspace* w) : prev(t_skw), prev_disp(t_disp) { t_skw = w; t_disp = w ? w->disp.refresh() : nullptr; }
SkScope::~SkScope() { t_skw = prev; t_disp = prev_disp; }

int sk_workspace_acquire(hipStream_t stream, SkWorkspace** out) {
  *out = nullptr;
// ... 59 lines not shown
```

streamspeech_amd/csrc/dispatch.hpp:

```cpp
#pragma once
#include <functional>

namespace ss {

struct Dispatch {
  int attn_no_mfma = 0;
  int attn_q16 = 1;
  int attn_split = 0;
  int c16_off = 0, c32_off = 0, c64_off = 0;
  long long c16_min_rows = 131072, c32_min_rows = 65536, c64_min_rows = 32768;
  int c64w_on = 1, c128w_on = 1, c256w_on = 1, c32w_on = 1;
  int c64w_min_k = 3;
  long long c128w_min_rows = 65536, c256w_min_rows = 32768;
  int c256w_rows = 128;
  int c32_min_k = 7, c16_min_k = 11;
  int slab_grid_cap = 0;
  int sk_groups = 0;
  int sk2_spare_cus = 0;
  int ffn_force_g = 0;
  int ffn_wm = 3, ffn_wm_forced = 0;
  int ffn_wm_env = 0;
  int ffn_fusion = 1;
  int ffn_min_rows = 1000;
  int force_bm = 0, force_bn = 0, force_ks = 0;
  double sk_min_flops = 4e9;
  int smallm_max_rows = 192;
  long long sk_min_units = 12 * 512;
  int no_sk2 = 0;
  int sk2_min_k64 = 192;
  int no_resblock_fusion = 0, no_pair_fusion = 0;
  int rt_off = 0, rt_min_rows = 193, rt_force_g = 0;
  long long rt_min_units = 4000;
  int rt_wg_per_cu = 0;
  long long rt_kb_min_units = 256;
  int rt_kb_xmap = 1;
  int rt_kb_uw = 0;
  int rt_kb_order = 1;
};

const Dispatch& disp();
void dispatch_edit(const std::function<void(Dispatch&)>& fn);

struct CtxDispatch {
  Dispatch d;
  unsigned gen = 0xffffffffu;
  const Dispatch* refresh();
};
struct DispatchScope {
  explicit DispatchScope(const Dispatch* d);
  ~DispatchScope();
  const Dispatch* prev;
};

}
```

streamspeech_amd/csrc/gemm.hpp:

```cpp
#pragma once
#include "common.hpp"
#include "dispatch.hpp"
#include "prof.hpp"

namespace ss {

struct GemmArgs {
  const float* A = nullptr;
  const float* W = nullptr;
  const float* Wwino = nullptr;
  const void* Wf16 = nullptr;
  const float* bias = nullptr;
  const float* R = nullptr;
  const float* R2 = nullptr;
  float* C = nullptr;
  int lda = 0, ldc = 0, ldr = 0, ldr2 = 0;
  int M = 0, N = 0, Cin = 0;
  int taps = 1, dil = 1, stride = 1, pad = 0;
  int in_len = 0;
  int chunk = 0;
  int m_begin = 0;
  int in_act = ACT_NONE;
  float in_slope = 0.1f;
  int act = ACT_NONE;
  float alpha = 1.0f;
  float div = 0.0f;
  float act_slope = 0.1f;
  float* C2 = nullptr;
  int ldc2 = 0;
  float c2_slope = 0.1f;
  int glu = 0;
  const int* segs = nullptr;
  int nseg = 0;
  int max_seg_out = 0;
  const int* seg_mb = nullptr;
  const float* const* seg_A = nullptr;
  double algo_flops = 0.0;
  double algo_bytes = 0.0;
  const float* ln_g = nullptr;
  const float* ln_b = nullptr;
  float* ln_out = nullptr;
  int same_rows = 0;
  int x3 = 0;
  int canon = 0;
};
constexpr int CANON_NONE = 0, CANON_SEQ = 1, CANON_SMALLM = 2;
constexpr int CANON_KBLOCK = 64;
struct CanonScope {
  explicit CanonScope(int mode);
  ~CanonScope();
  int prev;
};
int canon_mode();
void canon_debug_set(int mode);

struct SkWorkspace {
  int dev = -1, cus = 0;
  float* ws = nullptr;
  unsigned* sync1 = nullptr;
  unsigned* sync2 = nullptr;
  unsigned* sync3 = nullptr;
  unsigned base1[8] = {0, 0, 0, 0, 0, 0, 0, 0}, epoch1 = 0;
  unsigned base2 = 0, epoch2 = 0;
  unsigned long long* dbg = nullptr;
  CtxDispatch disp;
};
SkWorkspace* sk_workspace_new();
void sk_workspace_free(SkWorkspace* w);
struct SkScope {
  explicit SkScope(SkWorkspace* w);
  ~SkScope();
  SkWorkspace* prev;
  const Dispatch* prev_disp;
};
int sk_workspace_acquire(hipStream_t stream, SkWorkspace** out);
int sk_workspace_error_count();

bool conv_sk_eligible(const GemmArgs& a);
int launch_conv_sk(const GemmArgs& a, hipStream_t stream, int g_force = 0);
int conv_sk_error_count();
void conv_sk_set_groups(int on);

bool conv_sk2_eligible(const GemmArgs& a);
int launch_conv_sk2(const GemmArgs& a, hipStream_t stream, int g_force = 0);
int conv_sk2_error_count();

inline bool slab_rows_ok(long long rows) { return rows > 0 && rows < (1ll << 30); }

inline size_t slab_lds_bytes(int slab_rows, int lda, int maxseg) {
  return (size_t)((slab_rows * lda + 3) & ~3) * sizeof(float) + (maxseg + 2) * sizeof(int);
}
inline long long slab_max_blocks(int M, int bm, int nseg) { return (long long)cdiv(M, bm) + (nseg > 0 ? nseg : 1); }
inline int slab_grid(int occ, int cus, int M, int bm, int nseg) {
  const long long g = std::min<long long>((long long)occ * cus, std::max<long long>(1, slab_max_blocks(M, bm, nseg)));
  const int cap = disp().slab_grid_cap;
  return (int)(cap > 0 ? std::min<long long>(g, cap) : g);
}
void slab_debug(int grid, long long min_rows);
bool slab_layout_ok(const GemmArgs& a);
bool slab_conv_ok(const GemmArgs& a, int c);
int device_cus(int& cus);

bool conv_slab_eligible(const GemmArgs& a);
int launch_conv_slab(const GemmArgs& a, hipStream_t stream);

bool conv_pair_eligible(int C, int taps, int dil, int lda, int ldc, int nseg, long long M);
int launch_conv_pair(const float* A, int lda, const float* W1, const float* b1, const float* W2, const float* b2, float* C,
                     int ldc, const float* R2, int ldr2, float div, float* C2, int ldc2, float c2_slope, int Cch, int taps,
                     int dil, int M, int in_len, float slope, const int* segs, int nseg, hipStream_t stream);

bool resblock_fused_eligible(int C, int taps, const int* dil, int ldx, int ldy, int nseg, long long M);
int launch_resblock_fused(const float* X, int ldx, const float* const* W1, const float* const* B1, const float* const* W2,
                          const float* const* B2, const int* dil, float* Y, int ldy, const float* R2, int ldr2, float div, int C,
                          int taps, int M, float slope, const int* segs, int nseg, hipStream_t stream);

bool conv_c64_eligible(const GemmArgs& a);
bool conv_c64_enabled();
int launch_conv_c64(const GemmArgs& a, hipStream_t stream);
bool conv_c64w_eligible(const GemmArgs& a);
int launch_conv_c64w(const GemmArgs& a, hipStream_t stream);
int launch_wino_pack(const float* W, float* WW, int C, int taps, hipStream_t stream);
void conv_c64w_debug(int enable);
bool conv_c64w_enabled();
bool conv_wide_winograd_eligible(const GemmArgs& a, int ch);
int launch_conv_c128w(const GemmArgs& a, hipStream_t stream);
void conv_c128w_debug(int enable);
bool conv_c128w_enabled();
int launch_conv_c256w(const GemmArgs& a, hipStream_t stream);
void conv_c256w_debug(int enable);
int conv_c256w_rows_debug(int rows);
bool conv_c256w_enabled();
bool conv_c32w_eligible(const GemmArgs& a);
int launch_conv_c32w(const GemmArgs& a, hipStream_t stream);
void conv_c32w_debug(int enable);
bool conv_c32w_enabled();
void conv_c64_debug(int enable);

bool conv_c32_eligible(const GemmArgs& a);
bool conv_c32_enabled();
int launch_conv_c32(const GemmArgs& a, hipStream_t stream);
void conv_c32_debug(int enable);

bool conv_c16_eligible(const GemmArgs& a);
bool conv_c16_enabled();
int launch_conv_c16(const GemmArgs& a, hipStream_t stream);
void conv_c16_debug(int enable);

bool conv_f16_eligible(const GemmArgs& a);
bool conv_f16_geometry_ok(int C, int taps, int dil);
int launch_conv_f16(const GemmArgs& a, hipStream_t stream);
size_t f16_pack_halves(int C, int taps);
int launch_f16_pack(const float* W, void* Wf, int C, int taps, hipStream_t stream);

bool rtlin_eligible(const GemmArgs& a);
bool rtlin_shape_ok(const GemmArgs& a);
int launch_rtlin(const GemmArgs& a, hipStream_t stream);
void rtlin_debug(int grid, int enable);
bool rtlin_kb_shape_ok(const GemmArgs& a);
bool rtlin_kb_eligible(const GemmArgs& a);
int launch_rtlin_kb(const GemmArgs& a, hipStream_t stream);
void rtlin_kb_debug(int uw, int order);
void rtlin_kb_last(int out[4]);

bool ffn_fused_eligible(int D, int F, int act, int M, int ldx, int ldy, bool canon = false);
int launch_ffn_fused(const float* X, int ldx, float* Y, int ldy, const float* ln_g, const float* ln_b, const float* W1,
                     const float* b1, const float* W2, const float* b2, float alpha, const float* ln2_g, const float* ln2_b,
                     int M, int D, int F, hipStream_t stream, int canon = 0);
void ffn_fused_debug_grid(int g);
void ffn_fused_debug_rows(int wm);

bool gemv_eligible(const GemmArgs& a);
bool smallm_eligible(const GemmArgs& a);

void debug_force_tile(int bm, int bn, int ks);
bool debug_tile_forced();

int launch_conv_gemm(const GemmArgs& a, hipStream_t stream);

}
```

streamspeech_amd/csrc/model_internal.hpp:

```cpp
#pragma once
#include <algorithm>
#include <atomic>
#include <map>
#include <mutex>
#include <string>
#include <tuple>
#include <unordered_map>
#include <vector>

#include "../../include/streamspeech_hip.h"
#include "attention.hpp"
#include "attn_probs.hpp"
#include "common.hpp"
#include "elementwise.hpp"
#include "fbank.hpp"
#include "gemm.hpp"
#include "mt_step.hpp"
#include "enc_step.hpp"

using namespace ss;

namespace {

struct Slot { const float* p = nullptr; int64_t n = 0; };
// ... 314 lines not shown
}

[[maybe_unused]] static void subsampler_args(const ss_model* m, const float* fbank, float* h1, float* out, GemmArgs& a, GemmArgs& b) {
  const ss_config& c = m->cfg;
  const int k = c.conv_kernel, C1 = c.conv_channels / 2;
  a.A = fbank; a.lda = c.input_feat; a.W = m->sub0.w; a.bias = m->sub0.b; a.C = h1; a.ldc = C1;
  a.N = c.conv_channels; a.Cin = c.input_feat; a.taps = k; a.stride = 2; a.pad = k / 2; a.glu = 1;
  b.A = h1; b.lda = C1; b.W = m->sub1.w; b.bias = m->sub1.b; b.C = out; b.ldc = c.enc_dim;
  b.N = 2 * c.enc_dim; b.Cin = C1; b.taps = k; b.stride = 2; b.pad = k / 2; b.glu = 1;
}

[[maybe_unused]] static int enc_ffn_half(hipStream_t s, const ss_config& c, float* x, int n, const LN& ln, const Lin& w1, const Lin& w2,
                                         const LN* fin, bool fused, bool canon, float* h, float* ff) {
  const int d = c.enc_dim, f = c.enc_ffn;
  if (fused)
    return launch_ffn_fused(x, d, x, d, ln.g, ln.b, w1.w, w1.b, w2.w, w2.b, 0.5f, fin ? fin->g : nullptr, fin ? fin->b : nullptr,
                            n, d, f, s, canon);
  RET(ln_linear(s, x, n, ln, w1, f, d, ff, f, h, ACT_SILU));
  RET(linear(s, ff, f, n, w2, d, f, x, d, ACT_NONE, 0.5f, x, d));
  return fin ? layernorm(s, x, x, *fin, n, d) : SS_OK;
}

template <typename Attention, typename DwConv>
static int enc_layer_ex(hipStream_t s, const ss_config& c, const EncLayer& e, float* x, int n, float* h, float* ff, float* qkv_rows,
                        float* glu_rows, const float* dw_rows, bool ffn_fused, bool canon, Attention&& attention, DwConv&& dwconv) {
  const int d = c.enc_dim;
  RET(enc_ffn_half(s, c, x, n, e.ffn1_ln, e.ffn1_w1, e.ffn1_w2, nullptr, ffn_fused, canon, h, ff));
  RET(ln_linear(s, x, n, e.attn_ln, e.qkv, 3 * d, d, qkv_rows, 3 * d, h));
  RET(attention());
  RET(linear(s, h, d, n, e.out, d, d, x, d, ACT_NONE, 1.f, x, d));
  RET(ln_linear(s, x, n, e.conv_ln, e.pw1, 2 * d, d, glu_rows, d, h, ACT_NONE, 1.f, 1));
  RET(dwconv());
  RET(linear(s, dw_rows, d, n, e.pw2, d, d, x, d, ACT_NONE, 1.f, x, d));
  return enc_ffn_half(s, c, x, n, e.ffn2_ln, e.ffn2_w1, e.ffn2_w2, &e.final_ln, ffn_fused, canon, h, ff);
}

int mt_prefix_pass(ss_model* m, hipStream_t s, int B, int Np, int np_max, int n_enc, const int* d_ptok, const int* d_ppos,
                   const int* d_pself, const int* d_pcross, const int* d_ptail, const int* d_pcache, int cache_rows, const float** out);

int mt_cross_kv(ss_model* m, hipStream_t s, const float* d_enc_out, int n_rows);

struct MtRowsWs {
  float *x, *h, *q2, *ff, *logits;
  static size_t floats(int rows, int D, int F, int V, size_t gap = 0) { return (size_t)rows * (3 * D + F + V) + gap; }
  MtRowsWs(float* base, int rows, int D, int F, size_t gap = 0)
      : x(base), h(x + (size_t)rows * D), q2(h + (size_t)rows * D), ff(q2 + (size_t)rows * D), logits(ff + (size_t)rows * F + gap) {}
};

struct MtRowsStep {
  int rows = 0;
  int cache_ld = 0, ci = 0;
  const int* tok = nullptr;
  const int* row_pos = nullptr;
  int row_pad = -1;
  const int* self_segs = nullptr;
  const int* cross_segs = nullptr;
  int n_enc = 0;
  const int* anc = nullptr; int anc_ld = 0, anc_slots = 0;
  float* states = nullptr; int states_ld = 0;
};
int mt_decode_rows(ss_model* m, hipStream_t s, const MtRowsWs& w, const MtRowsStep& a);

extern std::atomic<int> g_mt_timeouts;

struct ConvW { const float* w = nullptr; const float* b = nullptr; const float* ww = nullptr;
               const void* wh = nullptr; };
struct ss_vocoder {
  ss_vocoder_config cfg;
  WeightTable wt;
  ss_scratch* sc = nullptr;
  const float* dict = nullptr;
  ConvW dur_c1, dur_c2, dur_proj, pre, post;
  LN dur_ln1, dur_ln2;
  std::vector<ConvW> ups;
  std::vector<ConvW> rb_c1, rb_c2;
  float* wino = nullptr;
  const float* wino_key = nullptr;
  int x3 = 0;
  int f16 = 0;
  const float* blob = nullptr;
  void* f16w = nullptr;
  const float* spk_table = nullptr;
  int n_spk = 0;
};

namespace {

[[maybe_unused]] int upload(hipStream_t s, int* dst, const std::vector<int>& v) {
  SS_HIP_CHECK(hipMemcpyAsync(dst, v.data(), v.size() * sizeof(int), hipMemcpyHostToDevice, s));
  return SS_OK;
}

struct Offsets { std::vector<int> off; int total = 0, mx = 0; };
[[maybe_unused]] Offsets prefix(const int* len, int B) {
  Offsets o; o.off.resize(B + 1); o.off[0] = 0;
  for (int b = 0; b < B; ++b) { o.off[b + 1] = o.off[b] + len[b]; o.mx = std::max(o.mx, len[b]); }
  o.total = o.off[B];
  return o;
}

}
```

streamspeech_amd/csrc/vocoder.hip:

```cpp
#include "model_internal.hpp"

#include <cstdint>
#include <tuple>


namespace {
struct WinoShared { DevBuf buf; size_t floats = 0; int refs = 0; };
struct WinoKey {
  int dev; const float* blob; uint64_t sig;
  bool operator<(const WinoKey& o) const { return std::tie(dev, blob, sig) < std::tie(o.dev, o.blob, o.sig); }
};
std::mutex g_wino_mu;
std::map<WinoKey, WinoShared> g_wino;
inline uint64_t fnv(uint64_t h, uint64_t v) { for (int i = 0; i < 8; ++i) { h ^= (v >> (8 * i)) & 0xff; h *= 1099511628211ull; } return h; }
uint64_t blob_sig(const ss_vocoder* v, const float* d_blob) {
  const ss_vocoder_config* cfg = &v->cfg;
  uint64_t sig = fnv(fnv(fnv(14695981039346656037ull, (uint64_t)cfg->upsample_initial_channel), (uint64_t)cfg->n_up), (uint64_t)cfg->n_res);
  for (int j = 0; j < cfg->n_res; ++j) sig = fnv(sig, (uint64_t)cfg->resblock_kernel_sizes[j]);
  for (size_t i = 0; i < v->rb_c1.size(); ++i) sig = fnv(fnv(sig, (uint64_t)(v->rb_c1[i].w - d_blob)), (uint64_t)(v->rb_c2[i].w - d_blob));
  return sig;
}
std::mutex g_f16_mu;
std::map<WinoKey, WinoShared> g_f16;
bool f16_stage(int ch) { return ch == 64 || ch == 128 || ch == 256; }
// ... 23 lines not shown
  for (int i = 0; i < cfg->n_up; ++i) {
    const int Co = C / 2, st = cfg->upsample_rates[i];
    v->ups.push_back({w.get("voc.up" + std::to_string(i) + ".w", (int64_t)st * Co * 3 * C),
                      w.get("voc.up" + std::to_string(i) + ".b", (int64_t)st * Co)});
    for (int j = 0; j < cfg->n_res; ++j) {
      const int kr = cfg->resblock_kernel_sizes[j];
      for (int dd = 0; dd < 3; ++dd) {
        const std::string p = "voc.rb" + std::to_string(i * cfg->n_res + j);
        v->rb_c1.push_back({w.get(p + ".c1." + std::to_string(dd) + ".w", (int64_t)Co * kr * Co),
                            w.get(p + ".c1." + std::to_string(dd) + ".b", Co)});
        v->rb_c2.push_back({w.get(p + ".c2." + std::to_string(dd) + ".w", (int64_t)Co * kr * Co),
                            w.get(p + ".c2." + std::to_string(dd) + ".b", Co)});
      }
    }
    C = Co;
  }
  v->post = {w.get("voc.post.w", (int64_t)7 * C), w.get("voc.post.b", 1)};
  {
    auto it = w.map.find("voc.spkr.table");
    if (it != w.map.end()) {
      const int64_t per = (int64_t)16 * C0;
      if (it->second.n <= 0 || it->second.n % per || it->second.n / per > INT32_MAX || (C0 & 3)) { scratch_unref(v->sc); delete v; return SS_ERR_ARG; }
      v->spk_table = it->second.p;
      v->n_spk = (int)(it->second.n / per);
    }
  }
  if (!w.missing.empty()) { scratch_unref(v->sc); delete v; return SS_ERR_MISSING_WEIGHT; }
  {
    auto wino_stage = [](int ch) { return ch == 32 || ch == 64 || ch == 128 || ch == 256; };
    size_t need = 0;
    int Cs = C0;
    for (int i = 0; i < cfg->n_up; ++i) {
      Cs /= 2;
      if (wino_stage(Cs)) for (int j = 0; j < cfg->n_res; ++j) need += 6 * (size_t)Cs * ((cfg->resblock_kernel_sizes[j] + 2) / 3) * 4 * Cs;
    }
    if (need) {
      int dev = 0;
      if (hipGetDevice(&dev) != hipSuccess) { scratch_unref(v->sc); delete v; return SS_ERR_HIP; }
      std::lock_guard<std::mutex> lk(g_wino_mu);
      const WinoKey key{dev, d_blob, blob_sig(v, d_blob)};
      WinoShared& sh = g_wino[key];
      const bool fresh = sh.refs == 0;
      if (!fresh && sh.floats != need) { scratch_unref(v->sc); delete v; return SS_ERR_ARG; }
      if (fresh) {
        rc = sh.buf.ensure(need * sizeof(float));
        if (rc != SS_OK) { g_wino.erase(key); scratch_unref(v->sc); delete v; return rc; }
        sh.floats = need;
      }
      float* dst = sh.buf.f();
      Cs = C0;
      for (int i = 0; i < cfg->n_up && rc == SS_OK; ++i) {
        Cs /= 2;
        if (!wino_stage(Cs)) continue;
        for (int j = 0; j < cfg->n_res && rc == SS_OK; ++j) {
          const int kr = cfg->resblock_kernel_sizes[j];
          const size_t n = (size_t)Cs * ((kr + 2) / 3) * 4 * Cs;
          for (int dd = 0; dd < 3 && rc == SS_OK; ++dd) {
            const int idx = (i * cfg->n_res + j) * 3 + dd;
            if (fresh) rc = launch_wino_pack(v->rb_c1[idx].w, dst, Cs, kr, nullptr);
            v->rb_c1[idx].ww = dst; dst += n;
            if (fresh && rc == SS_OK) rc = launch_wino_pack(v->rb_c2[idx].w, dst, Cs, kr, nullptr);
            v->rb_c2[idx].ww = dst; dst += n;
          }
        }
      }
      if (fresh && rc == SS_OK && hipDeviceSynchronize() != hipSuccess) rc = SS_ERR_HIP;
      if (rc != SS_OK) {
        if (fresh) { sh.buf.release(); g_wino.erase(key); }
        scratch_unref(v->sc); delete v; return rc;
      }
      ++sh.refs;
      v->wino = sh.buf.f(); v->wino_key = d_blob;
    }
  }
  *out = v;
  return SS_OK;
}

extern "C" int ss_vocoder_num_speakers(const ss_vocoder* v) { return v ? v->n_spk : 0; }

extern "C" int ss_vocoder_set_bf16x3(ss_vocoder* v, int on) {
  if (!v) return SS_ERR_ARG;
  v->x3 = on ? 1 : 0;
  return SS_OK;
}

static int f16_take(ss_vocoder* v) {
  const ss_vocoder_config& c = v->cfg;
  size_t need = 0;
  for (int i = 0, Cs = c.upsample_initial_channel; i < c.n_up; ++i) {
    Cs /= 2;
    if (f16_stage(Cs)) for (int j = 0; j < c.n_res; ++j) need += 6 * f16_pack_halves(Cs, c.resblock_kernel_sizes[j]);
  }
  if (!need) return SS_OK;
  for (int i = 0, Cs = c.upsample_initial_channel; i < c.n_up; ++i) {
    Cs /= 2;
    if (!f16_stage(Cs)) continue;
    for (int j = 0; j < c.n_res; ++j)
      for (int dd = 0; dd < 3; ++dd)
        if (!conv_f16_geometry_ok(Cs, c.resblock_kernel_sizes[j], c.resblock_dilations[j][dd]) ||
            !conv_f16_geometry_ok(Cs, c.resblock_kernel_sizes[j], 1))
          return SS_ERR_ARG;
  }
  int dev = 0;
  if (hipGetDevice(&dev) != hipSuccess) return SS_ERR_HIP;
  std::lock_guard<std::mutex> lk(g_f16_mu);
  const WinoKey key{dev, v->blob, blob_sig(v, v->blob)};
  WinoShared& sh = g_f16[key];
  const bool fresh = sh.refs == 0;
  if (!fresh && sh.floats != need) return SS_ERR_ARG;
  int rc = SS_OK;
  if (fresh) {
    rc = sh.buf.ensure(need * sizeof(uint16_t));
    if (rc != SS_OK) { g_f16.erase(key); return rc; }
    sh.floats = need;
  }
  char* dst = static_cast<char*>(sh.buf.p);
  std::vector<ConvW> rb1 = v->rb_c1, rb2 = v->rb_c2;
  for (int i = 0, Cs = c.upsample_initial_channel; i < c.n_up && rc == SS_OK; ++i) {
    Cs /= 2;
    if (!f16_stage(Cs)) continue;
    for (int j = 0; j < c.n_res && rc == SS_OK; ++j) {
      const int kr = c.resblock_kernel_sizes[j];
      const size_t n = f16_pack_halves(Cs, kr) * sizeof(uint16_t);
      for (int dd = 0; dd < 3 && rc == SS_OK; ++dd) {
        const int idx = (i * c.n_res + j) * 3 + dd;
        if (fresh) rc = launch_f16_pack(rb1[idx].w, dst, Cs, kr, nullptr);
        rb1[idx].wh = dst; dst += n;
        if (fresh && rc == SS_OK) rc = launch_f16_pack(rb2[idx].w, dst, Cs, kr, nullptr);
        rb2[idx].wh = dst; dst += n;
      }
    }
  }
  if (fresh && rc == SS_OK && hipDeviceSynchronize() != hipSuccess) rc = SS_ERR_HIP;
  if (rc != SS_OK) {
    if (fresh) { sh.buf.release(); g_f16.erase(key); }
    return rc;
  }
  ++sh.refs;
  v->rb_c1.swap(rb1); v->rb_c2.swap(rb2);
  v->f16w = sh.buf.p;
  return SS_OK;
}

extern "C" int ss_vocoder_set_f16(ss_vocoder* v, int on) {
  if (!v) return SS_ERR_ARG;
  if (on && !v->f16w) RET(f16_take(v));
  v->f16 = on ? 1 : 0;
  return SS_OK;
}

extern "C" void ss_vocoder_destroy(ss_vocoder* v) {
  if (!v) return;
  if (v->f16w) {
    std::lock_guard<std::mutex> lk(g_f16_mu);
    for (auto it = g_f16.begin(); it != g_f16.end(); ++it)
      if (it->first.blob == v->blob && it->second.buf.p == v->f16w) {
        if (--it->second.refs == 0) { it->second.buf.release(); g_f16.erase(it); }
        break;
      }
  }
  if (v->wino_key) {
    std::lock_guard<std::mutex> lk(g_wino_mu);
    for (auto it = g_wino.begin(); it != g_wino.end(); ++it)
      if (it->first.blob == v->wino_key && it->second.buf.f() == v->wino) {
        if (--it->second.refs == 0) { it->second.buf.release(); g_wino.erase(it); }
// ... 11 lines not shown
    scratch_unref(v->sc);
    v->sc = sc;
  }
  return SS_OK;
}

struct GenBufs { float *bx, *bt, *br, *bs, *bxa, *bra, *bsa, *br2; };
struct SpkSel { const int* seg = nullptr; int one = 0; int max_frames = 0; };

template <class ConvFn, class StageFn, class GeomFn>
static int hifigan_stack(const ss_vocoder* v, hipStream_t s, ConvFn&& conv, StageFn&& on_stage, GeomFn&& geom,
                         const float* frames, int Ft, const GenBufs& b, int* out_scale, int* out_C, const SpkSel* spk = nullptr) {
  const ss_vocoder_config& c = v->cfg;
  const bool f16 = v->f16 && v->f16w;
  const bool x3 = v->x3 && !f16;
  auto slab_stage = [&](int channels) {
    if (x3 || !(channels == 64 ? conv_c64_enabled() : channels == 32 ? conv_c32_enabled() : channels == 16 ? conv_c16_enabled() : false)) return false;
    long long rows = Ft; int ch = c.upsample_initial_channel; bool found = false;
    for (int i = 0; i < c.n_up && !found; ++i) { rows *= c.upsample_rates[i]; ch /= 2; found = ch == channels; }
    if (!found || rows >= (1ll << 30)) return false;
    GemmArgs probe;
    probe.same_rows = 1; probe.Cin = probe.N = probe.lda = probe.ldc = channels; probe.taps = 3; probe.dil = 1; probe.pad = 1;
    probe.M = probe.in_len = (int)rows; probe.in_act = ACT_LRELU;
    return channels == 64 ? conv_c64_eligible(probe) : channels == 32 ? conv_c32_eligible(probe) : conv_c16_eligible(probe);
  };
  const bool c64 = slab_stage(64), c32 = slab_stage(32), c16 = slab_stage(16);
  auto wino_slab_stage = [&](int channels) {
    if (f16 || x3 || !(channels == 128 ? conv_c128w_enabled() : conv_c256w_enabled())) return false;
    long long rows = Ft; int ch = c.upsample_initial_channel, stage = -1;
    for (int i = 0; i < c.n_up && stage < 0; ++i) { rows *= c.upsample_rates[i]; ch /= 2; if (ch == channels) stage = i; }
    if (stage < 0 || rows >= (1ll << 30)) return false;
    int sc = 1, gM = 0, gnseg = 0; const int* gsegs = nullptr;
    for (int i = 0; i <= stage; ++i) sc *= c.upsample_rates[i];
    geom(sc, gM, gsegs, gnseg);
    for (int j = 0; j < c.n_res; ++j)
      for (int dd = 0; dd < 3; ++dd)
        for (int which = 0; which < 2; ++which) {
          const int idx = (stage * c.n_res + j) * 3 + dd;
          GemmArgs probe;
          probe.same_rows = 1; probe.Cin = probe.N = probe.lda = probe.ldc = probe.ldr = probe.ldr2 = probe.ldc2 = channels;
          probe.taps = c.resblock_kernel_sizes[j]; probe.dil = which ? 1 : c.resblock_dilations[j][dd];
          probe.pad = probe.dil * (probe.taps - 1) / 2; probe.M = probe.in_len = gM; probe.nseg = gnseg; probe.in_act = ACT_LRELU;
          probe.Wwino = which ? v->rb_c2[idx].ww : v->rb_c1[idx].ww;
          if (!conv_wide_winograd_eligible(probe, channels)) return false;
        }
    return true;
  };
  const bool c128 = wino_slab_stage(128), c256 = wino_slab_stage(256);
  auto preact = [c64, c128, c256, f16](int channels) {
    return channels >= 64 && !(c64 && channels == 64) && !(c128 && channels == 128) && !(c256 && channels == 256) && !(f16 && f16_stage(channels));
  };
  auto up_preact = [c64](int channels) { return channels >= 64 && !(c64 && channels == 64); };
  auto mk = [x3, f16](const float* A, int Cin, const ConvW& cw, int Cout, int k, int dil, float* Cc, int ldc) {
    GemmArgs a;
    a.A = A; a.lda = Cin; a.W = cw.w; a.Wwino = cw.ww; a.bias = cw.b; a.C = Cc; a.ldc = ldc; a.ldr = ldc; a.ldr2 = ldc; a.ldc2 = ldc;
    a.N = Cout; a.Cin = Cin; a.taps = k; a.dil = dil; a.stride = 1; a.pad = dil * (k - 1) / 2; a.same_rows = 1;
    a.x3 = x3;
    if (f16) a.Wf16 = cw.wh;
    return a;
  };
  int scale = 1, C = c.upsample_initial_channel;
  RET(on_stage(scale));
  {
    GemmArgs a = mk(frames, c.model_in_dim, v->pre, C, 7, 1, b.bx, C);
    if (up_preact(C) && !spk) a.C2 = b.bxa;
    if (f16) a.canon = CANON_SEQ;
    RET(conv(a, scale));
    if (spk) {
      int gM = 0, gnseg = 0; const int* gsegs = nullptr;
      geom(scale, gM, gsegs, gnseg);
      const bool pa0 = up_preact(C);
      RET(launch_spkr_pre_add(b.bx, pa0 ? b.bxa : b.bx, C, C, v->spk_table, spk->seg, spk->one, gsegs, gnseg, spk->max_frames, gM, pa0 ? 1 : 0,
                              0.1f, s));
    }
  }
  for (int i = 0; i < c.n_up; ++i) {
    const int st = c.upsample_rates[i], Co = C / 2;
    const bool pa_in = up_preact(C), pa = preact(Co);
    {
      GemmArgs a = mk(pa_in ? b.bxa : b.bx, C, v->ups[i], st * Co, 3, 1, b.bs, st * Co);
      if (!pa_in) { a.in_act = ACT_LRELU; a.in_slope = 0.1f; }
      if (pa) a.C2 = b.bsa;
      a.algo_flops = 2.0 * Ft * scale * C * Co * c.upsample_kernel_sizes[i];
      if (f16 && Co >= 64) a.canon = CANON_SEQ;
      RET(conv(a, scale));
    }
    scale *= st; C = Co;
    RET(on_stage(scale));
    const bool pa_next = (i + 1 < c.n_up) && up_preact(C);
    for (int j = 0; j < c.n_res; ++j) {
      const int kr = c.resblock_kernel_sizes[j];
      int gM = 0, gnseg = 0; const int* gsegs = nullptr;
      geom(scale, gM, gsegs, gnseg);
      const bool per_conv = (c32 && C == 32 && kr >= disp().c32_min_k) || (c16 && C == 16 && kr >= disp().c16_min_k);
      if (!pa && !per_conv && !disp().no_resblock_fusion && resblock_fused_eligible(C, kr, c.resblock_dilations[j], C, C, gnseg, gM)) {
        const float *W1[3], *B1[3], *W2[3], *B2[3];
        for (int dd = 0; dd < 3; ++dd) {
          const int idx = (i * c.n_res + j) * 3 + dd;
          W1[dd] = v->rb_c1[idx].w; B1[dd] = v->rb_c1[idx].b; W2[dd] = v->rb_c2[idx].w; B2[dd] = v->rb_c2[idx].b;
        }
        RET(launch_resblock_fused(b.bs, C, W1, B1, W2, B2, c.resblock_dilations[j], b.bx, C, j > 0 ? b.bx : nullptr, C,
                                  j == c.n_res - 1 ? (float)c.n_res : 0.f, C, kr, gM, 0.1f, gsegs, gnseg, s));
        continue;
      }
      const bool fuse = !pa && !per_conv && !disp().no_pair_fusion && kr == 3 &&
                        conv_pair_eligible(C, kr, c.resblock_dilations[j][2], C, C, gnseg, gM);
      const float* cur = b.bs;
      for (int dd = 0; dd < 3; ++dd) {
        const int idx = (i * c.n_res + j) * 3 + dd;
        if (fuse) {
          float* out = dd == 0 ? b.br : dd == 1 ? b.br2 : b.bx;
          const float* R2 = (dd == 2 && j > 0) ? b.bx : nullptr;
          const float div = (dd == 2 && j == c.n_res - 1) ? (float)c.n_res : 0.f;
          RET(launch_conv_pair(cur, C, v->rb_c1[idx].w, v->rb_c1[idx].b, v->rb_c2[idx].w, v->rb_c2[idx].b, out, C, R2, C, div,
                               nullptr, C, 0.1f, C, kr, c.resblock_dilations[j][dd], gM, gM, 0.1f, gsegs, gnseg, s));
          cur = out;
          continue;
        }
        const float* rin = dd == 0 ? b.bs : b.br;
        const float* rin_act = dd == 0 ? b.bsa : b.bra;
        GemmArgs a1 = mk(pa ? rin_act : rin, C, v->rb_c1[idx], C, kr, c.resblock_dilations[j][dd], b.bt, C);
        if (pa) { a1.act = ACT_LRELU; a1.act_slope = 0.1f; }
        else { a1.in_act = ACT_LRELU; a1.in_slope = 0.1f; }
        RET(conv(a1, scale));
        GemmArgs a2 = mk(b.bt, C, v->rb_c2[idx], C, kr, 1, dd < 2 ? b.br : b.bx, C);
        if (!pa) { a2.in_act = ACT_LRELU; a2.in_slope = 0.1f; }
        a2.R = rin;
        if (dd < 2) {
          if (pa) a2.C2 = b.bra;
        } else {
          a2.R2 = j == 0 ? nullptr : b.bx;
          a2.div = (j == c.n_res - 1) ? (float)c.n_res : 0.f;
          if (pa_next && j == c.n_res - 1) a2.C2 = b.bxa;
        }
        RET(conv(a2, scale));
      }
    }
  }
  *out_scale = scale; *out_C = C;
  return SS_OK;
}

static int conv1d(hipStream_t s, const float* A, int T, int Cin, const ConvW& cw, int Cout, int k, int dil,
                  float* C, int in_act, float slope, int act, const float* R, const float* R2, float div) {
  GemmArgs a;
  a.A = A; a.lda = Cin; a.W = cw.w; a.bias = cw.b; a.C = C; a.ldc = Cout; a.R = R; a.ldr = Cout; a.R2 = R2; a.ldr2 = Cout;
  a.M = T; a.N = Cout; a.Cin = Cin; a.taps = k; a.dil = dil; a.stride = 1; a.pad = dil * (k - 1) / 2; a.in_len = T;
  a.in_act = in_act; a.in_slope = slope; a.act = act; a.div = div; a.same_rows = 1;
  return launch_conv_gemm(a, s);
}

static bool spkr_args_ok(const ss_vocoder* v, bool have, const int32_t* h_spkr, int B) {
  if (!have) return v->n_spk == 0;
  if (v->n_spk == 0 || !h_spkr) return false;
  for (int b = 0; b < B; ++b)
    if (h_spkr[b] < 0 || h_spkr[b] >= v->n_spk) return false;
  return true;
}

static int vocoder_forward(ss_vocoder* v, void* stream, const int32_t* d_codes, int K, int dur_prediction,
                           const int32_t* d_forced_dur, float* d_wav, int64_t wav_capacity,
                           int32_t* d_dur, int64_t* h_n_samples, const int32_t* h_spkr) {
  if (!v || K <= 0 || !d_codes || !d_wav || !d_dur) return SS_ERR_ARG;
  if (!spkr_args_ok(v, h_spkr != nullptr, h_spkr, 1)) return SS_ERR_ARG;
  SkScope sk_scope(v->sc->skws);
  hipStream_t s = (hipStream_t)stream;
// ... 402 lines not shown
```

streamspeech_amd/engine.py:

```python
import ctypes as C
import os
from typing import List, NamedTuple, Optional, Tuple

import numpy as np
import torch

from . import lib as L
from .config import ModelConfig, VocoderConfig
from .weights import pack_model, pack_vocoder


def _ptr(t: Optional[torch.Tensor]):
    return None if t is None else C.c_void_p(t.data_ptr())


def _stream():
    return C.c_void_p(torch.cuda.current_stream().cuda_stream)


def _require_gpu(device):
    if not torch.cuda.is_available():
        raise L.StreamSpeechHipError(
            "streamspeech_amd needs an AMD GPU (torch.cuda.is_available() is False); "
            "there is no CPU fallback for the product path")
    return torch.device(device)


def _slots(names, offsets, numels):
    n = len(names)
    c_names = (C.c_char_p * n)(*[s.encode() for s in names])
    c_off = (C.c_int64 * n)(*offsets)
    c_num = (C.c_int64 * n)(*numels)
    return c_names, c_off, c_num, n


def _i32(vals):
    return (C.c_int32 * len(vals))(*[int(v) for v in vals])


def _unpack_scored(host, T: List[int], return_raw: bool = False):
    tot, fl = sum(T), host.view(np.float32)
    out, off = [], 0
    for b, t in enumerate(T):
        n = int(host[6 * tot + b])
        rec = (host[tot + off: tot + off + n].tolist(), host[2 * tot + off: 2 * tot + off + n].tolist(),
               host[3 * tot + off: 3 * tot + off + n].tolist(), fl[5 * tot + off: 5 * tot + off + n].copy(),
               fl[4 * tot + off: 4 * tot + off + t].copy())
        out.append(rec + (host[off: off + t].tolist(),) if return_raw else rec)
        off += t
    return out


class CtcAlignment(NamedTuple):
    score: float
    viterbi_score: float
    status: int
    path: Optional[List[int]]
    first: List[int]
    last: List[int]
    tok_lprob: np.ndarray


def resample_ratio(sr_in: int, sr_out: int = 16000) -> Tuple[int, int, int]:
    import math
    from .frontend import filter_half_len
    g = math.gcd(int(sr_in), int(sr_out))
    up, down = int(sr_out) // g, int(sr_in) // g
    return up, down, (0 if up == down else filter_half_len(up, down))


def fbank_sr_rows(n_in: int, up: int, down: int, half_len: int, lib=None) -> Optional[Tuple[int, int]]:
    lib = lib or L.load()
    rows, fin = C.c_int32(0), C.c_int32(0)
    rc = lib.ss_fbank_sr_rows(int(n_in), int(up), int(down), int(half_len), C.byref(rows), C.byref(fin))
    if rc == L.SS_ERR_ARG:
        return None
    L.check(rc, "ss_fbank_sr_rows")
    return rows.value, fin.value


MT_BEAM_MAX_ROWS = 256
MT_BEAM_MAX = 32


def check_search_options(len_penalty: float = 1.0, temperature: float = 1.0, no_repeat_ngram_size: int = 0):
    n, p, t = int(no_repeat_ngram_size), float(len_penalty), float(temperature)
    if n != no_repeat_ngram_size or (n != 0 and not 2 <= n <= 32):
        raise ValueError(f"no_repeat_ngram_size {no_repeat_ngram_size} outside {{0, 2..32}}")
    if not np.isfinite(p):
        raise ValueError(f"len_penalty {len_penalty} is not finite")
    if not (np.isfinite(t) and t > 0):
        raise ValueError(f"temperature {temperature} is not a finite positive number")
# ... 904 lines not shown
            _i32([min(int(a), 1 << 30) for a in attn_chunks]), _i32([min(int(c), 1 << 30) for c in conv_chunks]),
            _ptr(out), nf, nc), "ss_encoder_stream_forward_batch")
        views = [out[o:o + t2] for o, t2 in zip(plan["off"], plan["T2"])]
        self._last = (list(int(s) for s in slots), plan["T2"], out)
        return out, views, list(nf), list(nc)

    def ctc(self, head: int, slots: Optional[List[int]] = None, enc_packed: Optional[torch.Tensor] = None, return_raw: bool = False):
        if self._last is None:
            raise ValueError("ctc() before any forward()")
        lslots, T2, lout = self._last
        if slots is not None and [int(s) for s in slots] != lslots:
            raise ValueError("ctc() takes the slots of the last forward(), in its order")
        enc = lout if enc_packed is None else enc_packed
        if enc.shape[0] != sum(T2):
            raise ValueError("packed output of another step")
        n, tot = len(lslots), sum(T2)
        if self.scores:
            ibuf = torch.empty((6 * tot + n,), dtype=torch.int32, device=self.device)
            self._ctc_scored(head, n, lslots, enc, ibuf, tot)
            return _unpack_scored(ibuf.cpu().numpy(), T2, return_raw)
        ibuf = torch.empty((3 * tot + n,), dtype=torch.int32, device=self.device)
        raw, toks, idx, cnt = ibuf[:tot], ibuf[tot:2 * tot], ibuf[2 * tot:3 * tot], ibuf[3 * tot:]
        L.check(self.lib.ss_stream_pool_ctc(self.model.h, _stream(), self.h, int(head), n, _i32(lslots), _ptr(enc), _ptr(raw),
                                            _ptr(toks), _ptr(idx), _ptr(cnt)), "ss_stream_pool_ctc")
        host = ibuf.cpu().numpy()
        res, off = [], 0
        for b in range(n):
            k = int(host[3 * tot + b])
            rec = (host[tot + off: tot + off + k].tolist(), host[2 * tot + off: 2 * tot + off + k].tolist())
            res.append(rec + (host[off: off + T2[b]].tolist(),) if return_raw else rec)
            off += T2[b]
        return res

    def ctc_both(self):
        if self._last is None:
            raise ValueError("ctc_both() before any forward()")
        lslots, T2, enc = self._last
        n, tot = len(lslots), sum(T2)
        if self.scores:
            per = 6 * tot + n
            ibuf = torch.empty((2 * per,), dtype=torch.int32, device=self.device)
            for hd in (0, 1):
                self._ctc_scored(hd, n, lslots, enc, ibuf[hd * per:(hd + 1) * per], tot)
            host = ibuf.cpu().numpy()
            return _unpack_scored(host[:per], T2), _unpack_scored(host[per:], T2)
        per = 3 * tot + n
        ibuf = torch.empty((2 * per,), dtype=torch.int32, device=self.device)
        for hd in (0, 1):
            b = ibuf[hd * per:(hd + 1) * per]
            L.check(self.lib.ss_stream_pool_ctc(self.model.h, _stream(), self.h, hd, n, _i32(lslots), _ptr(enc), _ptr(b[:tot]),
                                                _ptr(b[tot:2 * tot]), _ptr(b[2 * tot:3 * tot]), _ptr(b[3 * tot:])), "ss_stream_pool_ctc")
        host = ibuf.cpu().numpy()
        res = []
        for hd in (0, 1):
            h = host[hd * per:(hd + 1) * per]
            out, off = [], 0
            for b in range(n):
                k = int(h[3 * tot + b])
                out.append((h[tot + off: tot + off + k].tolist(), h[2 * tot + off: 2 * tot + off + k].tolist()))
                off += T2[b]
            res.append(out)
        return res[0], res[1]

    def stats(self) -> Tuple[int, int]:
        a, b = C.c_int64(0), C.c_int64(0)
        L.check(self.lib.ss_stream_pool_stats(self.h, C.byref(a), C.byref(b)), "ss_stream_pool_stats")
        return int(a.value), int(b.value)

    def __del__(self):
        try:
            if getattr(self, "h", None):
                self.lib.ss_stream_pool_destroy(self.h)
                self.h = None
        except Exception:
            pass


class HipVocoder:

    def __init__(self, generator_state_dict, cfg: VocoderConfig = None, device="cuda:0", _share=None, scratch: "Scratch" = None):
        self.lib = L.load()
        self.cfg = cfg or VocoderConfig()
        self.device = _require_gpu(device)
        if _share is not None:
            names, offsets, numels, self.blob = _share
        else:
            names, offsets, numels, blob = pack_vocoder(generator_state_dict, self.cfg)
            self.blob = blob.to(self.device)
        self._packed = (names, offsets, numels, self.blob)
        c = self.cfg
        cc = L.SSVocoderConfig()
        c.validate()
        cc.num_embeddings, cc.embedding_dim, cc.model_in_dim = c.num_embeddings, c.embedding_dim, c.embedding_dim
        cc.upsample_initial_channel = c.upsample_initial_channel
        cc.n_up = len(c.upsample_rates)
        for i, (u, k) in enumerate(zip(c.upsample_rates, c.upsample_kernel_sizes)):
            cc.upsample_rates[i] = u
            cc.upsample_kernel_sizes[i] = k
        cc.n_res = len(c.resblock_kernel_sizes)
        for j, (k, dil) in enumerate(zip(c.resblock_kernel_sizes, c.resblock_dilation_sizes)):
            cc.resblock_kernel_sizes[j] = k
            for t, dv in enumerate(dil):
                cc.resblock_dilations[j][t] = dv
        cc.dur_hidden, cc.dur_kernel = c.dur_hidden, c.dur_kernel
        self.c_cfg = cc
        cn, co, cm, n = _slots(names, offsets, numels)
        h = C.c_void_p()
        with torch.cuda.device(self.device):
            L.check(self.lib.ss_vocoder_create(C.byref(cc), _ptr(self.blob), self.blob.numel(), cn, co, cm, n,
                                               C.byref(h)), "ss_vocoder_create")
        self.h = h
        self.num_speakers = int(self.lib.ss_vocoder_num_speakers(self.h))
        self.scratch = None
        if scratch is not None:
            self.bind_scratch(scratch)
        self.hop = int(np.prod(c.upsample_rates))
        self.max_dur = 64

    def bind_scratch(self, scratch: "Scratch"):
        L.check(self.lib.ss_vocoder_bind_scratch(self.h, scratch.h), "ss_vocoder_bind_scratch")
        self.scratch = scratch

    def new_context(self, scratch: "Scratch" = None) -> "HipVocoder":
        v = HipVocoder(None, self.cfg, device=str(self.device), _share=self._packed, scratch=scratch)
        if getattr(self, "bf16x3", False):
            v.set_bf16x3(True)
        if getattr(self, "fp16", False):
            v.set_fp16(True)
        return v

    def set_fp16(self, on: bool):
        with torch.cuda.device(self.device):
            L.check(self.lib.ss_vocoder_set_f16(self.h, int(bool(on))), "ss_vocoder_set_f16")
        self.fp16 = bool(on)

    def set_bf16x3(self, on: bool):
        L.check(self.lib.ss_vocoder_set_bf16x3(self.h, int(bool(on))), "ss_vocoder_set_bf16x3")
        self.bf16x3 = bool(on)

    def _check_units(self, ids: torch.Tensor):
        if ids.numel() and (int(ids.min()) < 0 or int(ids.max()) >= self.cfg.num_embeddings):
            raise IndexError(f"unit id outside the vocoder's {self.cfg.num_embeddings} codes")

    def _check_speakers(self, speakers, n: int) -> Optional[List[int]]:
        if not self.num_speakers:
            if speakers is not None:
                raise ValueError("this vocoder is single-speaker: it takes no speaker")
            return None
        if speakers is None:
            raise ValueError('require a speaker for a multi-speaker vocoder (the reference: require "spkr" input)')
        ids = [int(x) for x in speakers]
        if len(ids) != n:
            raise ValueError(f"{len(ids)} speakers for {n} rows")
        if any(x < 0 or x >= self.num_speakers for x in ids):
            raise IndexError(f"speaker id outside the vocoder's {self.num_speakers} speakers")
        return ids

    def batch_forward(self, codes: List[List[int]], dur_prediction=True, forced_dur: Optional[List[List[int]]] = None,
                      speakers: Optional[List[int]] = None):
        B = len(codes)
        spk = self._check_speakers(speakers, B)
        K = [len(c) for c in codes]
        flat = torch.tensor([u for c in codes for u in c], dtype=torch.int32)
        self._check_units(flat)
        flat = flat.to(self.device)
        fd = None
        if forced_dur is not None:
            fd = torch.tensor([d for ds in forced_dur for d in ds], dtype=torch.int32).to(self.device)
            cap = int(sum(sum(ds) for ds in forced_dur)) * self.hop
        else:
            cap = sum(K) * (self.max_dur if dur_prediction else 1) * self.hop
        wav = torch.empty((cap,), dtype=torch.float32, device=self.device)
        dur = torch.empty((sum(K),), dtype=torch.int32, device=self.device)
        st, ns = (C.c_int64 * B)(), (C.c_int64 * B)()
        if spk is None:
            L.check(self.lib.ss_batch_vocoder_forward(self.h, _stream(), B, _ptr(flat), _i32(K), int(dur_prediction), _ptr(fd),
                                                      _ptr(wav), cap, _ptr(dur), st, ns), "ss_batch_vocoder_forward")
        else:
            L.check(self.lib.ss_batch_vocoder_forward_spkr(self.h, _stream(), B, _ptr(flat), _i32(K), int(dur_prediction), _ptr(fd),
                                                           _ptr(wav), cap, _ptr(dur), st, ns, _i32(spk)),
                    "ss_batch_vocoder_forward_spkr")
        wavs = [wav[st[b]: st[b] + ns[b]] for b in range(B)]
        return wavs, dur, K

    def batch_tail(self, codes: List[List[int]], n_new: List[int], ctx: List[int], rf: List[int], dur_prediction: bool = True,
                   speakers: Optional[List[int]] = None):
        B = len(codes)
        if not (len(n_new) == len(ctx) == len(rf) == B) or B == 0:
            raise ValueError("one unit list, n_new, ctx and rf per row")
        spk = self._check_speakers(speakers, B)
        K = [len(c) for c in codes]
        flat = torch.tensor([u for c in codes for u in c], dtype=torch.int32)
        self._check_units(flat)
        flat = flat.to(self.device)
        cap = sum(int(n) for n in n_new) * (self.max_dur if dur_prediction else 1) * self.hop
        out = torch.empty((max(cap, 1),), dtype=torch.float32, device=self.device)
        first = (C.c_int32 * B)()
        dur = (C.c_int32 * max(sum(K), 1))()
        st, ns = (C.c_int64 * B)(), (C.c_int64 * B)()
        rfs = _i32([-1 if r is None else r for r in rf])
        if spk is None:
            L.check(self.lib.ss_batch_vocoder_tail(self.h, _stream(), B, _ptr(flat), _i32(K), _i32(n_new), _i32(ctx), rfs,
                                                   int(dur_prediction), _ptr(out), cap, first, dur, st, ns), "ss_batch_vocoder_tail")
        else:
            L.check(self.lib.ss_batch_vocoder_tail_spkr(self.h, _stream(), B, _ptr(flat), _i32(K), _i32(n_new), _i32(ctx), rfs,
                                                        int(dur_prediction), _ptr(out), cap, first, dur, st, ns, _i32(spk)),
                    "ss_batch_vocoder_tail_spkr")
# ... 37 lines not shown
```

streamspeech_amd/lib.py:

```python
import ctypes as C
import os

_HERE = os.path.dirname(os.path.abspath(__file__))
LIB_PATH = os.environ.get("SS_HIP_LIB") or os.path.join(_HERE, "libstreamspeech_hip.so")


class SSConfig(C.Structure):
    _fields_ = [(n, C.c_int32) for n in (
        "input_feat", "conv_channels", "conv_kernel", "enc_dim", "enc_ffn", "enc_heads", "enc_layers",
        "dw_kernel", "src_vocab", "tgt_vocab", "mt_layers", "dec_dim", "dec_ffn", "dec_heads",
        "t2u_layers", "unit_layers", "unit_vocab", "ctc_upsample", "pad", "eos", "unk",
        "max_rel_pos", "max_tgt_pos")]


class SSVocoderConfig(C.Structure):
    _fields_ = [
        ("num_embeddings", C.c_int32), ("embedding_dim", C.c_int32), ("model_in_dim", C.c_int32),
        ("upsample_initial_channel", C.c_int32),
        ("n_up", C.c_int32), ("upsample_rates", C.c_int32 * 8), ("upsample_kernel_sizes", C.c_int32 * 8),
        ("n_res", C.c_int32), ("resblock_kernel_sizes", C.c_int32 * 4), ("resblock_dilations", (C.c_int32 * 3) * 4),
        ("dur_hidden", C.c_int32), ("dur_kernel", C.c_int32)]


_vp, _i, _f, _i64 = C.c_void_p, C.c_int, C.c_float, C.c_int64
# ... 106 lines not shown

SIGNATURES = {
    "ss_abi_version": (_i, []),
    "ss_error_string": (C.c_char_p, [_i]),
    "ss_model_create": (_i, [C.POINTER(SSConfig), _vp, C.c_size_t, C.POINTER(C.c_char_p), C.POINTER(_i64),
                             C.POINTER(_i64), _i, C.POINTER(_vp)]),
    "ss_model_destroy": (None, [_vp]),
    "ss_scratch_create": (_i, [C.POINTER(_vp)]),
    "ss_scratch_destroy": (None, [_vp]),
    "ss_scratch_set_cap": (_i, [_vp, C.c_size_t]),
    "ss_scratch_trim": (_i, [_vp, C.c_size_t]),
    "ss_scratch_bytes": (C.c_size_t, [_vp]),
    "ss_model_bind_scratch": (_i, [_vp, _vp]),
    "ss_vocoder_bind_scratch": (_i, [_vp, _vp]),
    "ss_fbank_num_frames": (_i, [_i]),
    "ss_fbank_cmvn": (_i, [_vp, _vp, _vp, _i, _f, _vp, C.POINTER(_i)]),
    "ss_encoder_out_len": (_i, [_i]),
    "ss_resample": (_i, [_vp, _vp, _i64, _i, _i, _vp, _i, _vp, _i64]),
    "ss_mp3_probe": (_i, [_vp, C.c_size_t, _vp]),
    "ss_mp3_unpack": (_i, [_vp, C.c_size_t, _i64, _vp, _vp, _vp]),
    "ss_mp3_synthesize": (_i, [_vp, _vp, _vp, _i64, _vp, _i, _i, _vp, _i64, _vp, C.POINTER(C.c_size_t)]),
    "ss_mp3_stream_create": (_i, [_i, C.POINTER(_vp)]),
    "ss_mp3_stream_destroy": (None, [_vp]),
    "ss_mp3_stream_reset": (_i, [_vp]),
    "ss_mp3_stream_bound": (_i64, [_vp, C.c_size_t]),
    "ss_mp3_stream_push": (_i, [_vp, _vp, C.c_size_t, _i, _i64, _vp, _vp, _vp, C.POINTER(_i64), _vp]),
    "ss_mp3_stream_query": (_i, [_vp, _vp]),
    "ss_mp3_stream_copy": (_i, [_vp, _vp]),
    "ss_mp3_stream_synthesize": (_i, [_vp, _vp, _vp, _i64, _vp, _i, C.POINTER(_vp), C.POINTER(_vp), C.POINTER(_i64), _i, _i, _vp,
                                      C.POINTER(C.c_size_t)]),
    "ss_flac_streaminfo": (_i, [_vp, C.c_size_t, _vp]),
    "ss_flac_probe": (_i, [_vp, C.c_size_t, _vp]),
    "ss_flac_unpack": (_i, [_vp, C.c_size_t, _i64, _vp, _vp, _i64, _vp]),
    "ss_flac_restore_host": (_i, [_vp, _vp, _i64, _vp, _i, _i, _vp, _vp]),
    "ss_flac_restore": (_i, [_vp, _vp, _vp, _i64, _i64, _vp, _i, _i, _vp, _i64, _vp, C.POINTER(C.c_size_t)]),
    "ss_pcm_scatter": (_i, [_vp, _vp, _i64, _vp, _i, C.POINTER(_vp), C.POINTER(_i64), _i]),
    "ss_pcm_pack_s16": (_i, [_vp, _vp, _i64, _vp]),
    "ss_pcm_decode_host": (_i, [_vp, _i, _i, _i64, _vp]),
    "ss_pcm_pack_s16_host": (_i, [_vp, _i64, _vp]),
    "ss_pcm_emit_count": (_i64, [_i64, _i, _i, _i, _i]),
    "ss_pcm_emit": (_i, [_vp, _vp, _i, _vp, _i64]),
    "ss_pcm_emit_host": (_i, [_vp, _i, _vp, _i64]),
    "ss_pcm_encode_host": (_i, [_vp, _i64, _i, _vp]),
    "ss_vad_scan": (_i, [_vp, _vp, _i, _vp]),
    "ss_vad_scan_host": (_i, [_vp, _i, _vp]),
    "ss_row_max_logprob": (_i, [_vp, _vp, _i, _i, _i, _i, _i, _vp]),
    "ss_log_softmax": (_i, [_vp, _vp, _i, _i, _i, _i, _i, _vp]),
    "ss_encoder_forward": (_i, [_vp, _vp, _vp, _i, _i, _i, _vp]),
    "ss_encoder_stream_reset": (_i, [_vp]),
    "ss_encoder_stream_set_tail": (_i, [_vp, _i]),
    "ss_encoder_stream_set_deferred": (_i, [_vp, _i]),
    "ss_encoder_stream_status": (_i, [_vp, _vp, _vp]),
    "ss_debug_enc_step_inject_timeout": (_i, [_vp]),
    "ss_encoder_stream_forward": (_i, [_vp, _vp, _vp, _i, _i, _i, _vp, C.POINTER(C.c_int32), C.POINTER(C.c_int32)]),
    "ss_ctc_greedy_scored": (_i, [_vp, _vp, _i, _vp, _i, _vp, _vp, _vp, _vp, _vp, _vp, _vp, _vp]),
    "ss_ctc_greedy": (_i, [_vp, _vp, _i, _vp, _i, _vp, _vp, _vp, _vp, _vp]),
    "ss_stream_pool_create": (_i, [_vp, _i, _i, C.POINTER(_vp)]),
    "ss_stream_pool_destroy": (None, [_vp]),
    "ss_stream_pool_reset": (_i, [_vp, _i]),
    "ss_stream_pool_set_tail": (_i, [_vp, _i, _i]),
    "ss_encoder_stream_forward_batch": (_i, [_vp, _vp, _vp, _i, C.POINTER(C.c_int32), C.POINTER(_vp), C.POINTER(C.c_int32),
                                             C.POINTER(C.c_int32), C.POINTER(C.c_int32), _vp, C.POINTER(C.c_int32),
                                             C.POINTER(C.c_int32)]),
    "ss_stream_pool_set_scores": (_i, [_vp, _i]),
    "ss_stream_pool_ctc_scored": (_i, [_vp, _vp, _vp, _i, _i, C.POINTER(C.c_int32), _vp, _vp, _vp, _vp, _vp, _vp, _vp, _vp]),
    "ss_stream_pool_ctc": (_i, [_vp, _vp, _vp, _i, _i, C.POINTER(C.c_int32), _vp, _vp, _vp, _vp, _vp]),
    "ss_stream_pool_stats": (_i, [_vp, C.POINTER(_i64), C.POINTER(_i64)]),
    "ss_mt_begin": (_i, [_vp, _vp, _vp, _i]),
    "ss_mt_set_persistent": (_i, [_vp, _i]),
    "ss_model_set_pack_invariant": (_i, [_vp, _i]),
    "ss_model_get_pack_invariant": (_i, [_vp]),
    "ss_debug_canon": (_i, [_i]),
    "ss_mt_get_persistent": (_i, [_vp]),
    "ss_debug_mt_inject_timeout": (_i, [_vp]),
    "ss_mt_append": (_i, [_vp, _vp, _vp, _i, _i, _i, _i, _vp, _vp, _i]),
    "ss_mt_truncate": (_i, [_vp, _i]),
    "ss_mt_greedy": (_i, [_vp, _vp, _vp, _i, C.POINTER(C.c_int32), _i, _i, _i, C.POINTER(C.c_int32), C.POINTER(_i),
                          _vp, C.POINTER(_i)]),
    "ss_t2u_units": (_i, [_vp, _vp, _vp, _i, _i, _i, _vp, _vp, _vp, _vp, _i]),
    "ss_vocoder_create": (_i, [C.POINTER(SSVocoderConfig), _vp, C.c_size_t, C.POINTER(C.c_char_p),
                               C.POINTER(_i64), C.POINTER(_i64), _i, C.POINTER(_vp)]),
    "ss_vocoder_destroy": (None, [_vp]),
    "ss_vocoder_set_bf16x3": (_i, [_vp, _i]),
    "ss_vocoder_set_f16": (_i, [_vp, _i]),
    "ss_vocoder_forward": (_i, [_vp, _vp, _vp, _i, _i, _vp, _vp, _i64, _vp, C.POINTER(_i64)]),
    "ss_vocoder_num_speakers": (_i, [_vp]),
    "ss_vocoder_forward_spkr": (_i, [_vp, _vp, _vp, _i, _i, _vp, _vp, _i64, _vp, C.POINTER(_i64), C.c_int32]),
    "ss_batch_vocoder_forward_spkr": (_i, [_vp, _vp, _i, _vp, C.POINTER(C.c_int32), _i, _vp, _vp, _i64, _vp,
                                           C.POINTER(_i64), C.POINTER(_i64), C.POINTER(C.c_int32)]),
    "ss_batch_vocoder_tail_spkr": (_i, [_vp, _vp, _i, _vp, C.POINTER(C.c_int32), C.POINTER(C.c_int32), C.POINTER(C.c_int32),
                                        C.POINTER(C.c_int32), _i, _vp, _i64, C.POINTER(C.c_int32), C.POINTER(C.c_int32),
                                        C.POINTER(_i64), C.POINTER(_i64), C.POINTER(C.c_int32)]),
    "ss_batch_fbank_cmvn": (_i, [_vp, _vp, _i, _vp, C.POINTER(_i64), C.POINTER(C.c_int32), _f, _vp, C.POINTER(C.c_int32)]),
    "ss_batch_cmvn": (_i, [_vp, _vp, _vp, _i64, _vp]),
    "ss_batch_encoder_forward": (_i, [_vp, _vp, _i, _vp, C.POINTER(C.c_int32), _i, _i, _vp, C.POINTER(C.c_int32)]),
    "ss_batch_ctc_greedy_scored": (_i, [_vp, _vp, _i, _i, _vp, C.POINTER(C.c_int32), _vp, _vp, _vp, _vp, _vp, _vp, _vp]),
    "ss_batch_ctc_greedy": (_i, [_vp, _vp, _i, _i, _vp, C.POINTER(C.c_int32), _vp, _vp, _vp, _vp]),
    "ss_batch_ctc_align": (_i, [_vp, _vp, _i, _i, _vp, C.POINTER(C.c_int32), C.POINTER(C.c_int32), C.POINTER(C.c_int32), _vp, _vp, _vp,
                                _vp, _vp]),
    "ss_ctc_align_host": (_i, [_vp, _i, _i, _i, _i, C.POINTER(C.c_int32), C.POINTER(C.c_int32), C.POINTER(C.c_int32), _vp, _vp, _vp,
                               _vp, _vp, _vp]),
    "ss_batch_mt_greedy": (_i, [_vp, _vp, _i, _vp, C.POINTER(C.c_int32), C.POINTER(C.c_int32), _i,
                                C.POINTER(C.c_int32), _i, C.POINTER(C.c_int32), _vp, _i]),
    "ss_batch_mt_beam": (_i, [_vp, _vp, _i, _i, _vp, C.POINTER(C.c_int32), C.POINTER(C.c_int32), _i, _f, _i,
                              C.POINTER(C.c_int32), _i, C.POINTER(C.c_int32), C.POINTER(_f), C.POINTER(_f), _vp, _i]),
    "ss_batch_mt_continue": (_i, [_vp, _vp, _i, _vp, C.POINTER(C.c_int32), C.POINTER(C.c_int32), C.POINTER(C.c_int32),
                                  C.POINTER(C.c_int32), _i, C.POINTER(C.c_int32), _i, C.POINTER(C.c_int32), _vp, _i,
                                  C.POINTER(C.c_int32)]),
    "ss_batch_mt_continue_plan": (_i, [_i, C.POINTER(C.c_int32), C.POINTER(C.c_int32), C.POINTER(C.c_int32),
                                       C.POINTER(C.c_int32), _i, _i, _i, _i, _i, _i, C.POINTER(C.c_int32), C.POINTER(C.c_int32),
                                       _i64, C.POINTER(_i64)]),
    "ss_batch_mt_beam_continue": (_i, [_vp, _vp, _i, _i, _vp, C.POINTER(C.c_int32), C.POINTER(C.c_int32), C.POINTER(C.c_int32),
                                       C.POINTER(C.c_int32), _i, _f, _i, C.POINTER(C.c_int32), _i, C.POINTER(C.c_int32),
                                       C.POINTER(_f), C.POINTER(_f), _vp, _i]),
    "ss_batch_mt_beam_continue_plan": (_i, [_i, _i, C.POINTER(C.c_int32), C.POINTER(C.c_int32), C.POINTER(C.c_int32),
                                            C.POINTER(C.c_int32), _i, _i, _i, _i, _i, _i, _i, C.POINTER(C.c_int32),
                                            C.POINTER(C.c_int32), _i64, C.POINTER(_i64)]),
    "ss_batch_mt_beam_opts": (_i, [_vp, _vp, _i, _i, _vp, C.POINTER(C.c_int32), C.POINTER(C.c_int32), _i, _f, _i,
                                   C.POINTER(C.c_int32), _i, C.POINTER(C.c_int32), C.POINTER(_f), C.POINTER(_f), _vp, _i,
                                   C.POINTER(SSMtSearchOpts)]),
    "ss_batch_mt_beam_continue_opts": (_i, [_vp, _vp, _i, _i, _vp, C.POINTER(C.c_int32), C.POINTER(C.c_int32), C.POINTER(C.c_int32),
                                            C.POINTER(C.c_int32), _i, _f, _i, C.POINTER(C.c_int32), _i, C.POINTER(C.c_int32),
                                            C.POINTER(_f), C.POINTER(_f), _vp, _i, C.POINTER(SSMtSearchOpts)]),
    "ss_batch_mt_beam_continue_plan_opts": (_i, [_i, _i, C.POINTER(C.c_int32), C.POINTER(C.c_int32), C.POINTER(C.c_int32),
                                                 C.POINTER(C.c_int32), _i, _i, _i, _i, _i, _i, _i, C.POINTER(C.c_int32),
                                                 C.POINTER(C.c_int32), _i64, C.POINTER(_i64), C.POINTER(SSMtSearchOpts)]),
    "ss_batch_fbank_frames": (_i, [_vp, _vp, _i, C.POINTER(_vp), C.POINTER(C.c_int32), C.POINTER(C.c_int32), _f,
                                   C.POINTER(_vp)]),
    "ss_batch_fbank_frames_sr": (_i, [_vp, _vp, _i, C.POINTER(_vp), C.POINTER(C.c_int32), C.POINTER(C.c_int32), C.POINTER(C.c_int32),
                                      C.POINTER(_vp), C.POINTER(C.c_int32), C.POINTER(C.c_int32), C.POINTER(C.c_int32), _f,
                                      C.POINTER(_vp)]),
    "ss_fbank_sr_rows": (_i, [_i64, _i, _i, _i, C.POINTER(C.c_int32), C.POINTER(C.c_int32)]),
    "ss_batch_t2u_units": (_i, [_vp, _vp, _i, _vp, _i, C.POINTER(C.c_int32), _i, _i, _vp, _vp, _vp]),
    "ss_batch_vocoder_forward": (_i, [_vp, _vp, _i, _vp, C.POINTER(C.c_int32), _i, _vp, _vp, _i64, _vp,
                                      C.POINTER(_i64), C.POINTER(_i64)]),
    "ss_batch_t2u_units_pad": (_i, [_vp, _vp, _i, _vp, _i, C.POINTER(C.c_int32), C.POINTER(C.c_int32), _i, _i, _vp, _vp, _vp]),
    "ss_batch_mt_features": (_i, [_vp, _vp, _i, _vp, C.POINTER(C.c_int32), C.POINTER(C.c_int32), C.POINTER(C.c_int32),
                                  C.POINTER(C.c_int32), _vp, _i]),
    "ss_batch_mt_attention": (_i, [_vp, _vp, _i, _vp, C.POINTER(C.c_int32), C.POINTER(C.c_int32), C.POINTER(C.c_int32),
                                   C.POINTER(C.c_int32), _vp, _i, _vp, C.POINTER(_i64), _i64, _vp, _vp]),
    "ss_batch_mt_score": (_i, [_vp, _vp, _i, _vp, C.POINTER(C.c_int32), _i, C.POINTER(C.c_int32), C.POINTER(C.c_int32),
                               C.POINTER(C.c_int32), _vp, _i, _vp, _vp]),
    "ss_batch_vocoder_tail": (_i, [_vp, _vp, _i, _vp, C.POINTER(C.c_int32), C.POINTER(C.c_int32), C.POINTER(C.c_int32),
                                   C.POINTER(C.c_int32), _i, _vp, _i64, C.POINTER(C.c_int32), C.POINTER(C.c_int32),
                                   C.POINTER(_i64), C.POINTER(_i64)]),
    "ss_batch_unit_spans": (_i, [_vp, _vp, _i, _vp, C.POINTER(C.c_int32), C.POINTER(C.c_int32), C.POINTER(C.c_int32),
                                 C.POINTER(C.c_int32), _vp, _vp, _vp, _vp]),
    "ss_unit_spans_host": (_i, [_i, _vp, C.POINTER(C.c_int32), C.POINTER(C.c_int32), C.POINTER(C.c_int32), C.POINTER(C.c_int32), _vp,
                                _i, _i, _i, _i, _i, _vp, _vp]),
    "ss_op_unit_spans": (_i, [_vp, _i, _vp, C.POINTER(C.c_int32), C.POINTER(C.c_int32), C.POINTER(C.c_int32), C.POINTER(C.c_int32),
                              _vp, _i, _i, _i, _i, _i, _vp, _vp]),
    "ss_prof_enable": (_i, [_i]),
    "ss_prof_enable_hi": (_i, [_i]),
    "ss_prof_reset": (_i, []),
    "ss_prof_read": (_i, [_i, C.POINTER(C.c_double), C.POINTER(C.c_double), C.POINTER(_i64), C.POINTER(C.c_double)]),
    "ss_prof_totals": (_i, [_i, C.POINTER(C.c_double), C.POINTER(C.c_double), C.POINTER(_i64)]),
    "ss_prof_read_issued": (_i, [_i, C.POINTER(C.c_double)]),
    "ss_prof_shape_log": (_i, [_i]),
    "ss_prof_shape_dump": (_i, [C.c_char_p, _i]),
    "ss_prof_num_classes": (_i, []),
    "ss_prof_class_name": (C.c_char_p, [_i]),
    "ss_debug_force_tile": (_i, [_i, _i, _i]),
    "ss_op_ffn_fused": (_i, [_vp, _vp, _i, _vp, _i, _vp, _vp, _vp, _vp, _vp, _vp, _f, _vp, _vp, _i, _i, _i]),
    "ss_debug_ffn": (_i, [_i, _i, _i]),
    "ss_debug_rtlin": (_i, [_i, _i]),
    "ss_debug_rtlin_kb": (_i, [_i, _i]),
    "ss_debug_rtlin_kb_last": (_i, [C.POINTER(C.c_int32)]),
    "ss_debug_conv_c64": (_i, [_i]),
    "ss_debug_conv_c256_rows": (_i, [_i]),
    "ss_debug_conv_c32": (_i, [_i]),
    "ss_debug_conv_c16": (_i, [_i]),
    "ss_debug_enc_step_launches": (_i64, []),
    "ss_debug_scratch_audit": (_i, [_vp, C.POINTER(C.c_size_t), C.POINTER(C.c_size_t)]),
    "ss_op_ln_linear": (_i, [_vp, _vp, _i, _vp, _vp, _vp, _vp, _vp, _i, _vp, _i, _i, _i, _i, _i, _f, _i]),
    "ss_op_ln_linear_ex": (_i, [_vp, _vp, _i, _vp, _vp, _vp, _vp, _vp, _vp, _i, _vp, _i, _i, _i, _i, _i, _f, _i, _i]),
    "ss_debug_last_logits": (_i, [_vp, _vp, _vp, _i64, C.POINTER(_i), C.POINTER(_i)]),
    "ss_debug_sk_errors": (_i, []),
    "ss_debug_attention_split": (_i, [_i]),
    "ss_debug_attention_q16": (_i, [_i]),
    "ss_op_conv_gemm": (_i, [_vp, _vp, _i, _vp, _vp, _vp, _i, _vp, _i, _vp, _i, _i, _i, _i, _i, _i, _i, _i, _i, _i,
                             _i, _f, _i, _f, _f, _i]),
    "ss_op_conv_gemm_ex": (_i, [_vp, C.POINTER(SSOpConvArgs)]),
    "ss_op_conv_gemm_rows": (_i, [_vp, C.POINTER(SSOpConvArgs), _i, _vp, _vp, _i]),
    "ss_op_conv_pair": (_i, [_vp, _vp, _i, _vp, _vp, _vp, _vp, _vp, _i, _vp, _i, _f, _vp, _i, _f, _i, _i, _i, _i, _i, _f, _vp, _i]),
    "ss_op_resblock_fused": (_i, [_vp, _vp, _i, _vp, _vp, _vp, _vp, _vp, _vp, _i, _vp, _i, _f, _i, _i, _i, _f, _vp, _i]),
    "ss_debug_slab": (_i, [_i, C.c_longlong]),
    "ss_op_conv_f16": (_i, [_vp, _vp, _vp, _vp, _vp, _vp, _vp, _vp, _i, _i, _i, _i, _i, _f, _i, _f, _vp, _i]),
    "ss_op_layernorm": (_i, [_vp, _vp, _i, _vp, _i, _vp, _vp, _i, _i, _f]),
    "ss_op_attention": (_i, [_vp, _vp, _i, _vp, _i, _vp, _i, _vp, _i, _i, _i, _i, _f, _i, _i, _vp, _i, _vp, _vp]),
    "ss_op_attention_ex": (_i, [_vp, C.POINTER(SSOpAttnArgs)]),
    "ss_op_attention_probs": (_i, [_vp, C.POINTER(SSOpAttnProbsArgs)]),
    "ss_op_attention_pool": (_i, [_vp, C.POINTER(SSOpPoolAttnArgs)]),
    "ss_debug_attention_no_mfma": (_i, [_i]),
    "ss_op_dwconv_bn_silu": (_i, [_vp, _vp, _i, _vp, _i, _vp, _i, _vp, _vp, _vp, _vp, _f, _i, _i, _i]),
    "ss_op_dwconv_bn_silu_ex": (_i, [_vp, _vp, _i, _vp, _i, _vp, _i, _vp, _vp, _vp, _vp, _f, _i, _i, _i, _vp, _i, _i]),
    "ss_op_pool_dwconv": (_i, [_vp, _vp, _vp, _i, _vp, _vp, _i, _vp, _vp, _vp, _vp, _f, _i, _vp, _i, _i]),
    "ss_op_pool_gather_rows": (_i, [_vp, _vp, _vp, _vp, _i, _i, _vp, _vp, _i, _i]),
    "ss_op_pool_gather_ids": (_i, [_vp, _vp, _vp, _vp, _i, _vp, _vp, _i, _i]),
    "ss_op_pool_stack_rows": (_i, [_vp, _vp, _vp, _i, _vp, _vp, _i, _i]),
    "ss_op_masked_argmax": (_i, [_vp, _vp, _i, _i, _i, _i, _i, _i, _i, _vp, _vp, _i, _i, _vp, _i]),
    "ss_op_ctc_collapse": (_i, [_vp, _vp, _i, _i, _i, _vp, _vp, _vp, _vp, _i]),
    "ss_op_masked_argmax_lprob": (_i, [_vp, _vp, _i, _i, _i, _i, _i, _i, _vp, _vp]),
    "ss_op_mt_token_scores": (_i, [_vp, _vp, _i, _i, _i, _vp, _vp, _vp]),
    "ss_debug_mt_score_form": (_i, [_i]),
    "ss_op_ctc_collapse_spans": (_i, [_vp, _vp, _vp, _i, _i, _i, _vp, _vp, _vp, _vp, _vp, _vp, _i]),
    "ss_op_ctc_align": (_i, [_vp, _vp, _i, _i, _i, _i, C.POINTER(C.c_int32), C.POINTER(C.c_int32), C.POINTER(C.c_int32), _vp, _vp, _vp,
                             _vp, _vp, _vp]),
    "ss_op_dur_predict": (_i, [_vp, _vp, _vp, _i, _vp, _vp, _vp, _i]),
    "ss_op_repeat_rows": (_i, [_vp, _vp, _vp, _i, _i, _vp, _i, _vp, _i]),
    "ss_op_embed_tokens": (_i, [_vp, _vp, _vp, _vp, _f, _i, _vp, _i, _i, _i, _i, _i]),
    "ss_op_embed_tokens_rows": (_i, [_vp, _vp, _vp, _vp, _i, _f, _i, _vp, _vp, _i, _i, _i, _i]),
    "ss_op_upsample_add_pos": (_i, [_vp, _vp, _i, _i, _vp, _f, _vp, _i]),
    "ss_op_gather_rows": (_i, [_vp, _vp, _vp, _i, _vp, _i, _i]),
    "ss_op_scatter_rows": (_i, [_vp, _vp, _vp, _i, _vp, _i, _i, _i, _i]),
    "ss_op_conv_post_tanh": (_i, [_vp, _vp, _i, _i, _vp, _vp, _f, _vp, _vp, _i]),
    "ss_op_conv_post_tanh_crop": (_i, [_vp, _vp, _i, _vp, _vp, _f, _vp, _vp, _i, _i]),
    "ss_op_spkr_pre_add": (_i, [_vp, _vp, _vp, _i, _i, _vp, _vp, _i, _vp, _i, _i, _i, _i, _f]),
    "ss_op_beam_topk": (_i, [_vp, _vp, _i, _i, _i, _i, _i, _vp, _vp, _vp, _vp, _i, _i, _i, _f, _vp, _vp]),
    "ss_op_beam_merge": (_i, [_vp, C.POINTER(SSOpBeamState), _i, _i, _i, _i, _i, _i, _i, _i]),
    "ss_op_beam_prefix_score": (_i, [_vp, _vp, _i, _i, _vp, _i, _i, _f, _vp]),
    "ss_op_beam_prefix_chain": (_i, [_vp, _vp, _vp, _vp, _i, _i, _vp, _vp]),
    "ss_op_beam_topk_opts": (_i, [_vp, _vp, _i, _i, _i, _i, _i, _vp, _vp, _vp, _vp, _i, _i, _i, _f, _vp, _vp, _f, _i, _vp, _vp, _i, _i,
                                  _vp, _vp, _vp]),
    "ss_op_beam_merge_opts": (_i, [_vp, C.POINTER(SSOpBeamState), _i, _i, _i, _i, _i, _i, _i, _i, _f]),
    "ss_op_beam_prefix_score_opts": (_i, [_vp, _vp, _i, _i, _vp, _i, _i, _f, _vp, _f]),
}

_lib = None


SS_ERR_ARG = 2
SS_ERR_CAPACITY = 4
SS_ERR_SCRATCH_CAP = 5
SS_ERR_STREAM_REPEAT = 8


class StreamSpeechHipError(RuntimeError):

    def __init__(self, msg, code=None):
        super().__init__(msg)
        self.code = code


def load():
    global _lib
    if _lib is not None:
        return _lib
    if not os.path.exists(LIB_PATH):
        raise StreamSpeechHipError(
            f"{LIB_PATH} not found: build it with streamspeech_amd/csrc/build.sh "
            "(or __graft_entry__.build()).  There is no CPU fallback for the product path.")
    import torch
    lib = C.CDLL(LIB_PATH)
    for name, (res, args) in SIGNATURES.items():
        try:
            fn = getattr(lib, name)
        except AttributeError as e:
            raise StreamSpeechHipError(f"{LIB_PATH} does not export {name}") from e
        fn.restype = res
        fn.argtypes = args
    if lib.ss_abi_version() != 2:
        raise StreamSpeechHipError("ABI version mismatch")
    _lib = lib
    return lib


# ... 5 lines not shown
```

streamspeech_amd/weights.py:

```python
import math
from typing import Dict, List, Tuple

import numpy as np
import torch

from .config import ModelConfig, VocoderConfig


def _t(x) -> torch.Tensor:
    if isinstance(x, torch.Tensor):
        return x.detach().float().cpu()
    return torch.from_numpy(np.ascontiguousarray(x)).float()


def glu_interleave(w: torch.Tensor) -> torch.Tensor:
    H = w.shape[0] // 2
    assert H % 16 == 0
    val = w[:H].reshape(H // 16, 16, *w.shape[1:])
    gate = w[H:].reshape(H // 16, 16, *w.shape[1:])
    return torch.cat([val, gate], dim=1).reshape(w.shape)


def conv_tap_major(w: torch.Tensor) -> torch.Tensor:
    return w.permute(0, 2, 1).contiguous().reshape(w.shape[0], -1)


def convT_polyphase(w: torch.Tensor, b: torch.Tensor, stride: int) -> Tuple[torch.Tensor, torch.Tensor]:
    cin, cout, k = w.shape
    assert (k - stride) % 2 == 0
    p = (k - stride) // 2
    out = torch.zeros(stride, cout, 3, cin)
    for r in range(stride):
        for jj in range(3):
            j = (1 - jj) * stride + r + p
            if 0 <= j < k:
                out[r, :, jj, :] = w[:, :, j].t()
    return out.reshape(stride * cout, 3 * cin).contiguous(), b.repeat(stride).contiguous()


def rel_pos_table(tmax: int, d: int) -> torch.Tensor:
    pe_positive = torch.zeros(tmax, d)
    pe_negative = torch.zeros(tmax, d)
    position = torch.arange(0, tmax, dtype=torch.float32).unsqueeze(1)
    div_term = torch.exp(torch.arange(0, d, 2, dtype=torch.float32) * -(math.log(10000.0) / d))
    pe_positive[:, 0::2] = torch.sin(position * div_term)
    pe_positive[:, 1::2] = torch.cos(position * div_term)
    pe_negative[:, 0::2] = torch.sin(-1 * position * div_term)
    pe_negative[:, 1::2] = torch.cos(-1 * position * div_term)
    return torch.cat([torch.flip(pe_positive, [0]), pe_negative[1:]], dim=0)


def sinusoid_table(n: int, dim: int, padding_idx: int) -> torch.Tensor:
    half = dim // 2
    e = math.log(10000) / (half - 1)
    e = torch.exp(torch.arange(half, dtype=torch.float) * -e)
    e = torch.arange(n, dtype=torch.float).unsqueeze(1) * e.unsqueeze(0)
    e = torch.cat([torch.sin(e), torch.cos(e)], dim=1).view(n, -1)
    e[padding_idx, :] = 0
    return e


def povey_window() -> torch.Tensor:
    i = np.arange(400, dtype=np.float64)
    return torch.from_numpy(((0.5 - 0.5 * np.cos(2 * math.pi * i / 399)) ** 0.85).astype(np.float32))


def mel_banks() -> torch.Tensor:
    mel = lambda f: 1127.0 * np.log(1.0 + f / 700.0)
    mlow, mhigh = mel(20.0), mel(8000.0)
    delta = (mhigh - mlow) / 81
    b = np.arange(80, dtype=np.float64)[:, None]
    left = mlow + b * delta
    center, right = left + delta, left + 2 * delta
    m = mel(31.25 * np.arange(256, dtype=np.float64))[None, :]
    w = np.maximum(0.0, np.minimum((m - left) / (center - left), (right - m) / (right - center)))
    return torch.from_numpy(np.pad(w, ((0, 0), (0, 1))).astype(np.float32))


class Packer:
    def __init__(self):
        self.names: List[str] = []
        self.tensors: List[torch.Tensor] = []

    def add(self, name: str, t: torch.Tensor):
        assert name not in self.names, name
        self.names.append(name)
        self.tensors.append(t.contiguous().float().reshape(-1))

    def finish(self):
        offsets, numels, off = [], [], 0
        for t in self.tensors:
            offsets.append(off)
            numels.append(t.numel())
            off += (t.numel() + 63) // 64 * 64
        blob = torch.zeros(off, dtype=torch.float32)
        for o, t in zip(offsets, self.tensors):
            blob[o:o + t.numel()] = t
        return self.names, offsets, numels, blob


def _ln(pk, name, sd, key):
    pk.add(name + ".g", _t(sd[key + ".weight"]))
    pk.add(name + ".b", _t(sd[key + ".bias"]))


def _lin(pk, name, sd, key, bias=True, scale=1.0):
    pk.add(name + ".w", _t(sd[key + ".weight"]) * scale)
    if bias:
        pk.add(name + ".b", _t(sd[key + ".bias"]) * scale)


def _fairseq_layers(pk: Packer, sd, src: str, dst: str, n: int, cross: bool):
    for l in range(n):
        p, q = f"{src}.layers.{l}", f"{dst}.L{l}"
        _ln(pk, q + ".self.ln", sd, p + ".self_attn_layer_norm")
        w = torch.cat([_t(sd[p + ".self_attn.q_proj.weight"]) * 0.125, _t(sd[p + ".self_attn.k_proj.weight"]),
                       _t(sd[p + ".self_attn.v_proj.weight"])], 0)
        b = torch.cat([_t(sd[p + ".self_attn.q_proj.bias"]) * 0.125, _t(sd[p + ".self_attn.k_proj.bias"]),
                       _t(sd[p + ".self_attn.v_proj.bias"])], 0)
        pk.add(q + ".self.qkv.w", w)
# ... 135 lines not shown
```

Before: 6453.

## Skip structurally-zero polyphase taps in vocoder transposed-conv GEMMs

Transposed convolutions in the vocoder are lowered to a 3-tap polyphase GEMM in which, per output phase, some tap slots are always zero. The change works out which tap range is live for each output-column tile. The stream-K GEMM then only walks those taps, and the c64 kernel gets a specialised 2-tap variant that pairs phase halves with shifted inputs. The host checks at load time that the dead slots really are zero before turning this on. The cost is added indexing complexity and extra tile-lookup loops in the sk2 kernel, in exchange for cutting MFMA and weight-load work on the upsampling layers.

```diff
diff --git a/include/streamspeech_hip.h b/include/streamspeech_hip.h
--- a/include/streamspeech_hip.h
+++ b/include/streamspeech_hip.h
@@ -320,6 +320,7 @@
                       int n_slots, ss_vocoder** out);
 void ss_vocoder_destroy(ss_vocoder* v);
 int ss_vocoder_set_bf16x3(ss_vocoder* v, int on);
+int ss_vocoder_declare_upconv_taps(ss_vocoder* v, unsigned mask);
 int ss_vocoder_set_f16(ss_vocoder* v, int on);
 int ss_vocoder_forward(ss_vocoder* v, void* stream, const int32_t* d_codes, int K, int dur_prediction,
                        const int32_t* d_forced_dur, float* d_wav, int64_t wav_capacity,
@@ -496,6 +497,11 @@
 } ss_op_conv_args;
 int ss_op_conv_gemm_ex(void* stream, const ss_op_conv_args* a);
 int ss_op_conv_gemm_rows(void* stream, const ss_op_conv_args* a, int m_begin, const int32_t* seg_mb, const float* const* seg_A, int canon);
+int ss_op_conv_gemm_up(void* stream, const ss_op_conv_args* a, int up_stride, int up_kernel);
+int ss_debug_upconv_taps(int on);
+int ss_debug_upconv_slots(int k, int s, int32_t* lo, int32_t* cnt);
+int64_t ss_debug_sk2_last_units(void);
+int ss_debug_c64_last_products(void);
 int ss_op_conv_pair(void* stream, const float* dA, int lda, const float* dW1, const float* db1, const float* dW2, const float* db2,
                     float* dC, int ldc, const float* dR2, int ldr2, float div, float* dC2, int ldc2, float c2_slope, int C, int taps,
                     int dil, int M, int in_len, float slope, const int32_t* d_segs, int nseg);
diff --git a/streamspeech_amd/csrc/conv_c64.hip b/streamspeech_amd/csrc/conv_c64.hip
--- a/streamspeech_amd/csrc/conv_c64.hip
+++ b/streamspeech_amd/csrc/conv_c64.hip
@@ -24,7 +24,7 @@
 [[maybe_unused]] constexpr int C6_NP = ((C6_BM_MAX + C6_MAXHALO) * (C6_C / 4) + 255) / 256;
 }
 
-template <bool LRELU, int WM>
+template <bool LRELU, int WM, bool UP>
 __global__ __launch_bounds__(256, 2) void conv_c64_kernel(const GemmArgs p, const int slab_rows) {
 #if __HIP_DEVICE_COMPILE__
   constexpr int C = C6_C, BM = 64 * WM, LDA = C6_LDA, NP = C6_NP;
@@ -44,8 +44,10 @@
 
   const __amdgpu_buffer_rsrc_t rsW = __builtin_amdgcn_make_buffer_rsrc((void*)p.W, 0, C6_NUM_RECORDS, 0x00020000);
   const int vo = (r * K + 4 * g) * 4;
+  const int ntaps = UP ? p.taps - 1 : p.taps;
   auto wload = [&](int tap, int f) -> f32x4 {
-    const int so = __builtin_amdgcn_readfirstlane((((f & 3) * 16) * K + tap * C + (f >> 2) * 16) * 4);
+    const int tj = tap + (UP && (f & 3) >= 2 ? 1 : 0);
+    const int so = __builtin_amdgcn_readfirstlane((((f & 3) * 16) * K + tj * C + (f >> 2) * 16) * 4);
     const u32x4 v = __builtin_amdgcn_raw_buffer_load_b128(rsW, vo, so, 0);
     return f32x4{__uint_as_float(v[0]), __uint_as_float(v[1]), __uint_as_float(v[2]), __uint_as_float(v[3])};
   };
@@ -98,19 +100,29 @@
 
     const float* pa = sA + (wave * 16 * WM + r) * LDA + 4 * g;
     const int a_step = p.dil * LDA;
-    f32x4 xa[WM];
+    constexpr int WH = UP ? WM : 1;
+    f32x4 xa[WM], xah[WH];
 #pragma unroll
     for (int i = 0; i < WM; ++i) xa[i] = *reinterpret_cast<const f32x4*>(pa + i * 16 * LDA);
+    if constexpr (UP) {
+#pragma unroll
+      for (int i = 0; i < WM; ++i) xah[i] = *reinterpret_cast<const f32x4*>(pa + a_step + i * 16 * LDA);
+    }
 #pragma unroll 1
-    for (int tap = 0; tap < p.taps; ++tap) {
-      const int tap_next = tap + 1 < p.taps ? tap + 1 : 0;
-      const float* pa_next = tap + 1 < p.taps ? pa + a_step : pa;
+    for (int tap = 0; tap < ntaps; ++tap) {
+      const int tap_next = tap + 1 < ntaps ? tap + 1 : 0;
+      const float* pa_next = tap + 1 < ntaps ? pa + a_step : pa;
 #pragma unroll
       for (int cc = 0; cc < 4; ++cc) {
-        f32x4 xb[WM];
+        f32x4 xb[WM], xbh[WH];
 #pragma unroll
         for (int i = 0; i < WM; ++i)
           xb[i] = *reinterpret_cast<const f32x4*>((cc < 3 ? pa : pa_next) + i * 16 * LDA + (cc < 3 ? (cc + 1) * 16 : 0));
+        if constexpr (UP) {
+#pragma unroll
+          for (int i = 0; i < WM; ++i)
+            xbh[i] = *reinterpret_cast<const f32x4*>((cc < 3 ? pa : pa_next) + a_step + i * 16 * LDA + (cc < 3 ? (cc + 1) * 16 : 0));
+        }
         f32x4 wf[4];
 #pragma unroll
         for (int j = 0; j < 4; ++j) {
@@ -124,9 +136,13 @@
           for (int i = 0; i < WM; ++i)
 #pragma unroll
             for (int j = 0; j < 4; ++j)
-              acc[i][j] = __builtin_amdgcn_mfma_f32_16x16x4f32(wf[j][e], xa[i][e], acc[i][j], 0, 0, 0);
+              acc[i][j] = __builtin_amdgcn_mfma_f32_16x16x4f32(wf[j][e], (UP && j >= 2) ? xah[UP ? i : 0][e] : xa[i][e], acc[i][j], 0, 0, 0);
 #pragma unroll
         for (int i = 0; i < WM; ++i) xa[i] = xb[i];
+        if constexpr (UP) {
+#pragma unroll
+          for (int i = 0; i < WM; ++i) xah[i] = xbh[i];
+        }
         C64_STEP_FENCE;
       }
       pa = pa_next;
@@ -172,12 +188,21 @@
 }
 
 static size_t c64_lds(int bm, const GemmArgs& a) { return slab_lds_bytes(bm + (a.taps - 1) * a.dil, C6_LDA, C6_MAXSEG); }
-template <bool LRELU, int WM>
+static std::atomic<int> g_c64_last_products{0};
+int conv_c64_last_products() { return g_c64_last_products.load(std::memory_order_relaxed); }
+
+static bool c64_up_form(const GemmArgs& a) {
+  if (a.up_stride <= 0 || !disp().upconv_live_taps || a.taps != 3 || a.dil != 1) return false;
+  int lo0 = 0, c0 = 0, lo1 = 0, c1 = 0;
+  return upconv_tile_slots(a, 0, 32, lo0, c0) && upconv_tile_slots(a, 32, 32, lo1, c1) && lo0 == 0 && c0 == 2 && lo1 == 1 && c1 == 2;
+}
+
+template <bool LRELU, int WM, bool UP = false>
 static int launch_c64_t(const GemmArgs& a, hipStream_t stream) {
   constexpr int BM = 64 * WM;
   const int slab_rows = BM + (a.taps - 1) * a.dil;
   const size_t lds = c64_lds(BM, a);
-  SS_MAX_LDS_ONCE((&conv_c64_kernel<LRELU, WM>), 96 * 1024);
+  SS_MAX_LDS_ONCE((&conv_c64_kernel<LRELU, WM, UP>), 96 * 1024);
   SkWorkspace* st = nullptr;
   int rc = sk_workspace_acquire(stream, &st);
   if (rc != SS_OK) return rc;
@@ -186,7 +211,8 @@
   ProfRec rec{}; bool prof = false;
   rc = prof_begin(a, stream, PROF_CONV_C64, rec, prof);
   if (rc != SS_OK) return rc;
-  hipLaunchKernelGGL((conv_c64_kernel<LRELU, WM>), dim3(grid), dim3(256), lds, stream, a, slab_rows);
+  g_c64_last_products.store(UP ? 8 : 4 * a.taps, std::memory_order_relaxed);
+  hipLaunchKernelGGL((conv_c64_kernel<LRELU, WM, UP>), dim3(grid), dim3(256), lds, stream, a, slab_rows);
   SS_LAUNCH_CHECK();
   return prof_end(stream, rec, prof);
 }
@@ -194,6 +220,7 @@
 int launch_conv_c64(const GemmArgs& a, hipStream_t stream) {
   if (!conv_c64_eligible(a)) return SS_ERR_ARG;
   const bool wm4 = 2 * c64_lds(256, a) <= 158 * 1024;
+  if (wm4 && c64_up_form(a)) return a.in_act == ACT_LRELU ? launch_c64_t<true, 4, true>(a, stream) : launch_c64_t<false, 4, true>(a, stream);
   if (a.in_act == ACT_LRELU) return wm4 ? launch_c64_t<true, 4>(a, stream) : launch_c64_t<true, 3>(a, stream);
   return wm4 ? launch_c64_t<false, 4>(a, stream) : launch_c64_t<false, 3>(a, stream);
 }
diff --git a/streamspeech_amd/csrc/conv_sk2.hip b/streamspeech_amd/csrc/conv_sk2.hip
--- a/streamspeech_amd/csrc/conv_sk2.hip
+++ b/streamspeech_amd/csrc/conv_sk2.hip
@@ -28,6 +28,8 @@
   unsigned epoch;
   int G;
   unsigned long long* dbg;
+  unsigned long long tap_lo, tap_cnt;
+  int tap_sum;
 };
 
 #define K2_WAIT_VMCNT(n) asm volatile("s_waitcnt vmcnt(" #n ")" ::: "memory")
@@ -105,10 +107,36 @@
   const int Ktot = p.taps * p.Cin;
   const int tiles_n = p.N / BN;
   const int tiles_m = (p.M + BM - 1) / BM;
-  const long long U = (long long)tiles_m * tiles_n * nk;
+  const bool ranged = q.tap_sum > 0;
+  const int S = ranged ? q.tap_sum * kpt : tiles_n * nk;
+  const long long U = (long long)tiles_m * S;
   const long long u0 = (long long)w * U / q.G, u1 = (long long)(w + 1) * U / q.G;
   if (u1 <= u0) return;
-  const int t_first = (int)(u0 / nk), t_last = (int)((u1 - 1) / nk);
+  struct Tile { long long ut0; int nk, lo, cnt; };
+  auto tile_at = [&](int tile) {
+    Tile T;
+    if (!ranged) { T.ut0 = (long long)tile * nk; T.nk = nk; T.lo = 0; T.cnt = p.taps; return T; }
+    const int tm = tile / tiles_n, tn = tile - tm * tiles_n;
+    int pre = 0;
+    for (int j = 0; j < tn; ++j) pre += (int)((q.tap_cnt >> (2 * j)) & 3);
+    T.lo = (int)((q.tap_lo >> (2 * tn)) & 3);
+    T.cnt = (int)((q.tap_cnt >> (2 * tn)) & 3);
+    T.nk = T.cnt * kpt;
+    T.ut0 = (long long)tm * S + (long long)pre * kpt;
+    return T;
+  };
+  auto tile_of = [&](long long u) {
+    if (!ranged) return (int)(u / nk);
+    const int tm = (int)(u / S);
+    int rem = (int)(u - (long long)tm * S), tn = 0;
+    while (tn + 1 < tiles_n) {
+      const int c = (int)((q.tap_cnt >> (2 * tn)) & 3) * kpt;
+      if (rem < c) break;
+      rem -= c; ++tn;
+    }
+    return tm * tiles_n + tn;
+  };
+  const int t_first = tile_of(u0), t_last = tile_of(u1 - 1);
 
   const float slope = p.in_slope;
   const __amdgpu_buffer_rsrc_t rsA = __builtin_amdgcn_make_buffer_rsrc(
@@ -122,14 +150,16 @@
   const int rdW1 = BM * BK + (wcol + r) * BK + (((4 + g) ^ swz) << 2);
   const int st_row = lane >> 3, st_pos = lane & 7;
 
-  struct Part { int ka, kb, n, m0, n0, tm; };
+  struct Part { int ka, kb, n, m0, n0, tm, nk, lo, cnt; };
   const int nparts = t_last - t_first + 1;
   auto part_of = [&](int ip) {
     const int tile = t_last - ip;
-    const long long ut0 = (long long)tile * nk;
+    const Tile T = tile_at(tile);
+    const long long ut0 = T.ut0;
     Part P;
+    P.nk = T.nk; P.lo = T.lo; P.cnt = T.cnt;
     P.ka = (int)(max(u0, ut0) - ut0);
-    P.kb = (int)(min(u1, ut0 + nk) - ut0);
+    P.kb = (int)(min(u1, ut0 + T.nk) - ut0);
     P.n = P.kb - P.ka;
     P.tm = tile / tiles_n;
     P.m0 = P.tm * BM;
@@ -139,6 +169,7 @@
   int a_base[8], a_len[8];
   unsigned a_off[8], w_off[NWP];
   int nci = 0, ntap = 0;
+  int tap_lo = 0, tap_end = p.taps;
   int soffA = 0, soffW = 0, shift = 0;
   int cur_tm = -1;
   auto lds_barrier = [&]() {
@@ -180,8 +211,9 @@
       const int nrow = wave * (BN / 4) + j * 8 + st_row;
       w_off[j] = (unsigned)(((P.n0 + nrow) * Ktot + ((st_pos ^ ((nrow >> 1) & 7)) << 2)) * 4);
     }
-    nci = (P.ka / p.taps) * BK;
-    ntap = P.ka - (P.ka / p.taps) * p.taps;
+    tap_lo = P.lo; tap_end = P.lo + P.cnt;
+    nci = (P.ka / P.cnt) * BK;
+    ntap = P.lo + P.ka - (P.ka / P.cnt) * P.cnt;
   };
   int shift_l = 0;
   auto step_begin = [&](bool live) {
@@ -194,8 +226,8 @@
   };
   auto step_advance = [&](bool adv = true) {
     const int nt = ntap + (adv ? 1 : 0);
-    const bool wrap = nt >= p.taps;
-    ntap = wrap ? 0 : nt;
+    const bool wrap = nt >= tap_end;
+    ntap = wrap ? tap_lo : nt;
     nci += wrap ? BK : 0;
   };
   [[maybe_unused]] bool in_loop = false;
@@ -289,7 +321,7 @@
 #if K2_RPREF
     constexpr int PT = BN == 128 ? 2 : TM;
     f32x4 rall[PT][TN];
-    const bool want_r = p.R != nullptr && cur.kb == nk;
+    const bool want_r = p.R != nullptr && cur.kb == cur.nk;
 #endif
     in_loop = true;
     K2_STAMP(1);
@@ -336,7 +368,7 @@
     }
     in_loop = false;
     K2_STAMP(2);
-    const bool has_begin = cur.ka == 0, has_end = cur.kb == nk;
+    const bool has_begin = cur.ka == 0, has_end = cur.kb == cur.nk;
     if (K2D_SKIP_TAIL && acc[0][0][0] != 12345.f) continue;
 
     int le = lane;
@@ -360,7 +392,7 @@
       continue;
     }
     if (!K2D_SKIP_HANDOFF && !has_begin) {
-      const long long ut0 = (long long)(t_last - ip) * nk;
+      const long long ut0 = tile_at(t_last - ip).ut0;
       const int wf = (int)(((ut0 + 1) * q.G - 1) / U);
       if (t == 0) {
         for (int ww = wf; ww < w; ++ww) {
@@ -530,6 +562,27 @@
 
 int conv_sk2_error_count() { return 0; }
 
+static std::atomic<long long> g_k2_last_units{0};
+long long conv_sk2_last_units() { return g_k2_last_units.load(std::memory_order_relaxed); }
+static bool sk2_tap_ranges(const GemmArgs& a, int BN, Sk2Args& q) {
+  q.tap_lo = q.tap_cnt = 0; q.tap_sum = 0;
+  if (a.up_stride <= 0 || !disp().upconv_live_taps) return false;
+  const int tiles_n = a.N / BN;
+  if (tiles_n > 32) return false;
+  unsigned long long lo_w = 0, cnt_w = 0;
+  int sum = 0;
+  for (int tn = 0; tn < tiles_n; ++tn) {
+    int lo = 0, cnt = 0;
+    if (!upconv_tile_slots(a, tn * BN, BN, lo, cnt)) return false;
+    lo_w |= (unsigned long long)lo << (2 * tn);
+    cnt_w |= (unsigned long long)cnt << (2 * tn);
+    sum += cnt;
+  }
+  if (sum == tiles_n * a.taps) return false;
+  q.tap_lo = lo_w; q.tap_cnt = cnt_w; q.tap_sum = sum;
+  return true;
+}
+
 template <int BN, bool LRELU, bool X3>
 static int launch_sk2(const GemmArgs& a, hipStream_t stream, int g_force) {
   constexpr size_t kLds = k2_lds_bytes(BN);
@@ -539,13 +592,15 @@
   if (rc != SS_OK) return rc;
   int cus = st->cus > K2_MAXG ? K2_MAXG : st->cus;
   if (const int spare = disp().sk2_spare_cus; spare > 0 && spare < cus) cus -= spare;
-  const long long nk = (long long)a.taps * (a.Cin / K2_BK);
-  const long long U = (long long)cdiv(a.M, K2_BM) * (a.N / BN) * nk;
+  Sk2Args q;
+  const bool ranged = sk2_tap_ranges(a, BN, q);
+  const long long S = (long long)(ranged ? q.tap_sum : (a.N / BN) * a.taps) * (a.Cin / K2_BK);
+  const long long U = (long long)cdiv(a.M, K2_BM) * S;
+  g_k2_last_units.store(U, std::memory_order_relaxed);
   long long G = g_force > 0 ? g_force : cus;
   if (G > cus) G = cus;
   if (G > U / 4) G = U / 4;
   if (G < 1) G = 1;
-  Sk2Args q;
   q.ws = st->ws; q.sync = st->sync2; q.G = (int)G; q.dbg = nullptr;
 #if K2D_TIMING
   if (!st->dbg) SS_HIP_CHECK(hipMalloc(&st->dbg, (size_t)K2_MAXG * 8 * sizeof(unsigned long long)));
diff --git a/streamspeech_amd/csrc/debug_ops.hip b/streamspeech_amd/csrc/debug_ops.hip
--- a/streamspeech_amd/csrc/debug_ops.hip
+++ b/streamspeech_amd/csrc/debug_ops.hip
@@ -54,6 +54,29 @@
   if (a.W && a.N > 0 && a.taps > 0) RET(op_bind_wino(a, stream));
   return launch_conv_gemm(a, (hipStream_t)stream);
 }
+extern "C" int ss_op_conv_gemm_up(void* stream, const ss_op_conv_args* x, int up_stride, int up_kernel) {
+  if (!x || up_stride < 0 || up_kernel < 0) return SS_ERR_ARG;
+  GemmArgs a;
+  op_fill_conv(a, x);
+  a.up_stride = up_stride; a.up_kernel = up_kernel;
+  if (a.W && a.N > 0 && a.taps > 0) RET(op_bind_wino(a, stream));
+  return launch_conv_gemm(a, (hipStream_t)stream);
+}
+extern "C" int ss_debug_upconv_taps(int on) {
+  if (on >= 0) dispatch_edit([on](Dispatch& d) { d.upconv_live_taps = on ? 1 : 0; });
+  return SS_OK;
+}
+extern "C" int ss_debug_upconv_slots(int k, int s, int32_t* lo, int32_t* cnt) {
+  if (!lo || !cnt || s < 1) return SS_ERR_ARG;
+  for (int r = 0; r < s; ++r) {
+    int l = 0, c = 0;
+    if (!upconv_live_slots(k, s, r, l, c)) return SS_ERR_ARG;
+    lo[r] = l; cnt[r] = c;
+  }
+  return SS_OK;
+}
+extern "C" int64_t ss_debug_sk2_last_units(void) { return conv_sk2_last_units(); }
+extern "C" int ss_debug_c64_last_products(void) { return conv_c64_last_products(); }
 extern "C" int ss_op_conv_pair(void* stream, const float* dA, int lda, const float* dW1, const float* db1, const float* dW2,
                                const float* db2, float* dC, int ldc, const float* dR2, int ldr2, float div, float* dC2, int ldc2,
                                float c2_slope, int Cch, int taps, int dil, int M, int in_len, float slope, const int32_t* d_segs,
diff --git a/streamspeech_amd/csrc/dispatch.hip b/streamspeech_amd/csrc/dispatch.hip
--- a/streamspeech_amd/csrc/dispatch.hip
+++ b/streamspeech_amd/csrc/dispatch.hip
@@ -32,6 +32,7 @@
   d.rt_kb_min_units = L("SS_RTLIN_KB_MIN_UNITS", d.rt_kb_min_units); d.rt_kb_uw = I("SS_RTLIN_KB_UW", d.rt_kb_uw); d.rt_kb_xmap = I("SS_RTLIN_KB_XMAP", d.rt_kb_xmap);
   d.smallm_max_rows = I("SS_SMALLM_MAX_ROWS", d.smallm_max_rows); d.sk_min_units = L("SS_SK_MIN_UNITS", d.sk_min_units);
   d.no_sk2 = I("SS_NO_SK2", 0) ? 1 : 0; d.sk2_min_k64 = I("SS_SK2_MINK64", d.sk2_min_k64); d.sk2_spare_cus = I("SS_SK2_SPARE_CUS", 0);
+  d.upconv_live_taps = I("SS_UPCONV_LIVE_TAPS", 1) ? 1 : 0;
   d.rt_wg_per_cu = I("SS_RTLIN_WG_PER_CU", 0); d.c32_min_k = I("SS_CONV_C32_MIN_K", d.c32_min_k); d.c16_min_k = I("SS_CONV_C16_MIN_K", d.c16_min_k);
   return d;
 }
diff --git a/streamspeech_amd/csrc/dispatch.hpp b/streamspeech_amd/csrc/dispatch.hpp
--- a/streamspeech_amd/csrc/dispatch.hpp
+++ b/streamspeech_amd/csrc/dispatch.hpp
@@ -17,6 +17,7 @@
   int slab_grid_cap = 0;
   int sk_groups = 0;
   int sk2_spare_cus = 0;
+  int upconv_live_taps = 1;
   int ffn_force_g = 0;
   int ffn_wm = 3, ffn_wm_forced = 0;
   int ffn_wm_env = 0;
diff --git a/streamspeech_amd/csrc/gemm.hpp b/streamspeech_amd/csrc/gemm.hpp
--- a/streamspeech_amd/csrc/gemm.hpp
+++ b/streamspeech_amd/csrc/gemm.hpp
@@ -43,7 +43,33 @@
   int same_rows = 0;
   int x3 = 0;
   int canon = 0;
-};
+  int up_stride = 0, up_kernel = 0;
+};
+inline bool upconv_live_slots(int k, int s, int r, int& lo, int& cnt) {
+  lo = 0; cnt = 0;
+  if (s < 1 || k < s || k > 3 * s || ((k - s) & 1) || r < 0 || r >= s) return false;
+  int first = 3, last = -1;
+  for (int jj = 0; jj < 3; ++jj) {
+    const int j = (1 - jj) * s + r + (k - s) / 2;
+    if (j >= 0 && j < k) { first = std::min(first, jj); last = std::max(last, jj); }
+  }
+  if (last < first) return false;
+  lo = first; cnt = last - first + 1;
+  return true;
+}
+inline bool upconv_tile_slots(const GemmArgs& a, int n0, int bn, int& lo, int& cnt) {
+  lo = 0; cnt = 0;
+  if (a.taps != 3 || a.up_stride < 1 || a.N % a.up_stride || n0 < 0 || n0 + bn > a.N) return false;
+  const int cout = a.N / a.up_stride;
+  int first = 3, last = -1;
+  for (int r = n0 / cout; r <= (n0 + bn - 1) / cout; ++r) {
+    int l = 0, c = 0;
+    if (!upconv_live_slots(a.up_kernel, a.up_stride, r, l, c)) return false;
+    first = std::min(first, l); last = std::max(last, l + c - 1);
+  }
+  lo = first; cnt = last - first + 1;
+  return true;
+}
 constexpr int CANON_NONE = 0, CANON_SEQ = 1, CANON_SMALLM = 2;
 constexpr int CANON_KBLOCK = 64;
 struct CanonScope {
@@ -84,6 +110,7 @@
 bool conv_sk2_eligible(const GemmArgs& a);
 int launch_conv_sk2(const GemmArgs& a, hipStream_t stream, int g_force = 0);
 int conv_sk2_error_count();
+long long conv_sk2_last_units();
 
 inline bool slab_rows_ok(long long rows) { return rows > 0 && rows < (1ll << 30); }
 
@@ -117,6 +144,7 @@
 bool conv_c64_eligible(const GemmArgs& a);
 bool conv_c64_enabled();
 int launch_conv_c64(const GemmArgs& a, hipStream_t stream);
+int conv_c64_last_products();
 bool conv_c64w_eligible(const GemmArgs& a);
 int launch_conv_c64w(const GemmArgs& a, hipStream_t stream);
 int launch_wino_pack(const float* W, float* WW, int C, int taps, hipStream_t stream);
diff --git a/streamspeech_amd/csrc/model_internal.hpp b/streamspeech_amd/csrc/model_internal.hpp
--- a/streamspeech_amd/csrc/model_internal.hpp
+++ b/streamspeech_amd/csrc/model_internal.hpp
@@ -420,6 +420,7 @@
   void* f16w = nullptr;
   const float* spk_table = nullptr;
   int n_spk = 0;
+  unsigned up_live = 0;
 };
 
 namespace {
diff --git a/streamspeech_amd/csrc/vocoder.hip b/streamspeech_amd/csrc/vocoder.hip
--- a/streamspeech_amd/csrc/vocoder.hip
+++ b/streamspeech_amd/csrc/vocoder.hip
@@ -129,6 +129,12 @@
 extern "C" int ss_vocoder_set_bf16x3(ss_vocoder* v, int on) {
   if (!v) return SS_ERR_ARG;
   v->x3 = on ? 1 : 0;
+  return SS_OK;
+}
+
+extern "C" int ss_vocoder_declare_upconv_taps(ss_vocoder* v, unsigned mask) {
+  if (!v || (v->cfg.n_up < 32 && (mask >> v->cfg.n_up))) return SS_ERR_ARG;
+  v->up_live = mask;
   return SS_OK;
 }
 
@@ -306,6 +312,7 @@
       if (!pa_in) { a.in_act = ACT_LRELU; a.in_slope = 0.1f; }
       if (pa) a.C2 = b.bsa;
       a.algo_flops = 2.0 * Ft * scale * C * Co * c.upsample_kernel_sizes[i];
+      if (v->up_live & (1u << i)) { a.up_stride = st; a.up_kernel = c.upsample_kernel_sizes[i]; }
       if (f16 && Co >= 64) a.canon = CANON_SEQ;
       RET(conv(a, scale));
     }
diff --git a/streamspeech_amd/engine.py b/streamspeech_amd/engine.py
--- a/streamspeech_amd/engine.py
+++ b/streamspeech_amd/engine.py
@@ -7,7 +7,7 @@
 
 from . import lib as L
 from .config import ModelConfig, VocoderConfig
-from .weights import pack_model, pack_vocoder
+from .weights import pack_model, pack_vocoder, upconv_dead_slots_are_zero
 
 
 def _ptr(t: Optional[torch.Tensor]):
@@ -1078,13 +1078,20 @@
         self.lib = L.load()
         self.cfg = cfg or VocoderConfig()
         self.device = _require_gpu(device)
+        c = self.cfg
         if _share is not None:
-            names, offsets, numels, self.blob = _share
+            names, offsets, numels, self.blob = _share[:4]
+            self._up_live = int(_share[4]) if len(_share) > 4 else 0
         else:
             names, offsets, numels, blob = pack_vocoder(generator_state_dict, self.cfg)
+            self._up_live = 0
+            for i, (u, k) in enumerate(zip(c.upsample_rates, c.upsample_kernel_sizes)):
+                j = names.index(f"voc.up{i}.w")
+                w, cin = blob[offsets[j]:offsets[j] + numels[j]], c.upsample_initial_channel >> i
+                if cin > 0 and numels[j] % (3 * cin) == 0 and upconv_dead_slots_are_zero(w.view(-1, 3 * cin), k, u):
+                    self._up_live |= 1 << i
             self.blob = blob.to(self.device)
         self._packed = (names, offsets, numels, self.blob)
-        c = self.cfg
         cc = L.SSVocoderConfig()
         c.validate()
         cc.num_embeddings, cc.embedding_dim, cc.model_in_dim = c.num_embeddings, c.embedding_dim, c.embedding_dim
@@ -1106,6 +1113,7 @@
             L.check(self.lib.ss_vocoder_create(C.byref(cc), _ptr(self.blob), self.blob.numel(), cn, co, cm, n,
                                                C.byref(h)), "ss_vocoder_create")
         self.h = h
+        L.check(self.lib.ss_vocoder_declare_upconv_taps(self.h, self._up_live), "ss_vocoder_declare_upconv_taps")
         self.num_speakers = int(self.lib.ss_vocoder_num_speakers(self.h))
         self.scratch = None
         if scratch is not None:
@@ -1118,7 +1126,7 @@
         self.scratch = scratch
 
     def new_context(self, scratch: "Scratch" = None) -> "HipVocoder":
-        v = HipVocoder(None, self.cfg, device=str(self.device), _share=self._packed, scratch=scratch)
+        v = HipVocoder(None, self.cfg, device=str(self.device), _share=self._packed + (self._up_live,), scratch=scratch)
         if getattr(self, "bf16x3", False):
             v.set_bf16x3(True)
         if getattr(self, "fp16", False):
diff --git a/streamspeech_amd/lib.py b/streamspeech_amd/lib.py
--- a/streamspeech_amd/lib.py
+++ b/streamspeech_amd/lib.py
@@ -212,6 +212,7 @@
                                C.POINTER(_i64), C.POINTER(_i64), _i, C.POINTER(_vp)]),
     "ss_vocoder_destroy": (None, [_vp]),
     "ss_vocoder_set_bf16x3": (_i, [_vp, _i]),
+    "ss_vocoder_declare_upconv_taps": (_i, [_vp, C.c_uint]),
     "ss_vocoder_set_f16": (_i, [_vp, _i]),
     "ss_vocoder_forward": (_i, [_vp, _vp, _vp, _i, _i, _vp, _vp, _i64, _vp, C.POINTER(_i64)]),
     "ss_vocoder_num_speakers": (_i, [_vp]),
@@ -312,6 +313,11 @@
                              _i, _f, _i, _f, _f, _i]),
     "ss_op_conv_gemm_ex": (_i, [_vp, C.POINTER(SSOpConvArgs)]),
     "ss_op_conv_gemm_rows": (_i, [_vp, C.POINTER(SSOpConvArgs), _i, _vp, _vp, _i]),
+    "ss_op_conv_gemm_up": (_i, [_vp, C.POINTER(SSOpConvArgs), _i, _i]),
+    "ss_debug_upconv_taps": (_i, [_i]),
+    "ss_debug_upconv_slots": (_i, [_i, _i, C.POINTER(C.c_int32), C.POINTER(C.c_int32)]),
+    "ss_debug_sk2_last_units": (_i64, []),
+    "ss_debug_c64_last_products": (_i, []),
     "ss_op_conv_pair": (_i, [_vp, _vp, _i, _vp, _vp, _vp, _vp, _vp, _i, _vp, _i, _f, _vp, _i, _f, _i, _i, _i, _i, _i, _f, _vp, _i]),
     "ss_op_resblock_fused": (_i, [_vp, _vp, _i, _vp, _vp, _vp, _vp, _vp, _vp, _i, _vp, _i, _f, _i, _i, _i, _f, _vp, _i]),
     "ss_debug_slab": (_i, [_i, C.c_longlong]),
diff --git a/streamspeech_amd/weights.py b/streamspeech_amd/weights.py
--- a/streamspeech_amd/weights.py
+++ b/streamspeech_amd/weights.py
@@ -36,6 +36,32 @@
             if 0 <= j < k:
                 out[r, :, jj, :] = w[:, :, j].t()
     return out.reshape(stride * cout, 3 * cin).contiguous(), b.repeat(stride).contiguous()
+
+
+def upconv_live_slots(k: int, stride: int) -> List[Tuple[int, int]]:
+    if stride < 1 or k < stride or k > 3 * stride or (k - stride) % 2:
+        raise ValueError(f"ConvTranspose1d(k={k}, stride={stride}) has no 3-tap polyphase form")
+    p = (k - stride) // 2
+    out = []
+    for r in range(stride):
+        live = [jj for jj in range(3) if 0 <= (1 - jj) * stride + r + p < k]
+        out.append((live[0], live[-1] - live[0] + 1))
+    return out
+
+
+def upconv_dead_slots_are_zero(wp: torch.Tensor, k: int, stride: int) -> bool:
+    try:
+        slots = upconv_live_slots(k, stride)
+    except ValueError:
+        return False
+    if wp.dim() != 2 or wp.shape[0] % stride or wp.shape[1] % 3:
+        return False
+    w = wp.reshape(stride, wp.shape[0] // stride, 3, wp.shape[1] // 3)
+    for r, (lo, cnt) in enumerate(slots):
+        for jj in range(3):
+            if not lo <= jj < lo + cnt and bool((w[r, :, jj, :] != 0).any()):
+                return False
+    return True
 
 
 def rel_pos_table(tmax: int, d: int) -> torch.Tensor:
```

Result: no change. 6510 (median of 6 runs) (+0.9%).
